# scomup/EasyGaussianSplatting

Measured on AMD Instinct MI355X. Metric: rendered Mpix/s fwd+bwd at 1920x1080, 1M Gaussians, higher is better.
Workload: dtype f32; 1 GPU; 1 MI355X per view: 1000000 synthetic Gaussians, 1920x1080, SH degree 3, forward+backward (GSFunction, mode=fused); gaussians=1000000, width=1920, height=1080, sh_dim=48, views_per_rank=1, view_streams=1, policy=gsplatcu, mode=fused, validation=deferred (commit per step), preconditioning=400 untimed steps before the warm-up steps (clock ramp), lists=footprint-culled (fused path)

## Files before the change

### easygaussiansplatting_amd/_ahead.py

```python
from __future__ import annotations

import collections
import ctypes as C
import threading

import torch

from . import _lib
from ._host import _ptr

MAILBOX_SLOTS = 64
HINT_SLOTS = 16
SIZE_TABLE_MAX = 1024


class _Ticket:
    __slots__ = ("ctx", "slot", "key", "cap", "hint", "state", "status", "patches", "need", "collected")
    PENDING, OK, FAILED = 0, 1, 2


class _DeviceCtx:

    def __init__(self, lib, index):
        self.index = index
        self.lib = lib
        self.mb = lib.egs_mailbox_create(MAILBOX_SLOTS)
        if not self.mb:
            raise RuntimeError("egs_mailbox_create failed (page-locked host memory)")
        self.free = list(range(MAILBOX_SLOTS))
        self.pending = collections.deque()
        self.failed = []
        self.capacity = {}
        self.tile_work = {}
        self.seg_hint = {}
        self.walk_word = {}
        self.long_walks_expected = 0
        self.lock = threading.RLock()


_contexts = {}
_tls = threading.local()


def _ctx(dev) -> _DeviceCtx:
    c = _contexts.get(dev.index)
    if c is None:
        c = _contexts.setdefault(dev.index, _DeviceCtx(_lib.load(), dev.index))
    return c


def _grow(p):
    return p + p // 16 + 4096


def _learn_capacity(ctx, key, patches):
    cap = ctx.capacity
    val = max(cap.pop(key, 0), _grow(min(patches, 2**31 - 1)))
    cap[key] = val
    while len(cap) > SIZE_TABLE_MAX:
        cap.pop(next(iter(cap)), None)


_key_bits = {}
_key_low = {}
KEY_BITS_DECAY = 32


def _get_key_bits(dev_index, key=None) -> int:
    return _key_bits.get((dev_index, key), 32)


def _set_key_bits(dev_index, key, bits) -> None:
    _key_bits[(dev_index, key)] = int(bits)
    _key_low.pop((dev_index, key), None)


def _learn_key_bits(dev_index, key, need, missed=False) -> None:
    k = (dev_index, key)
    target = min(32, int(need) + 1)
    while len(_key_bits) > 1024:
        old = next(iter(_key_bits))
        _key_bits.pop(old, None)
        _key_low.pop(old, None)
    if missed:
        _key_bits[k] = 32
        _key_low.pop(k, None)
        return
    hint = _key_bits.get(k, 32)
    if hint >= 32 or target >= hint:
        _key_bits[k] = target
        _key_low.pop(k, None)
        return
    low = _key_low.setdefault(k, [0, 0])
    low[0] += 1
    low[1] = max(low[1], target)
    if low[0] >= KEY_BITS_DECAY:
        _key_bits[k] = low[1]
        _key_low.pop(k, None)


def _bin_stage(enqueue, device, key=None):
    total = torch.empty(2, dtype=torch.int32, device=device)
    hint = _get_key_bits(device.index, key)
    enqueue(hint, total, None)
    p, mk = (int(v) & 0xFFFFFFFF for v in total.tolist())
    need = mk.bit_length()
    if hint < 32 and need > hint:
        enqueue(32, total, None)
        p, mk = (int(v) & 0xFFFFFFFF for v in total.tolist())
    _learn_key_bits(device.index, key, need)
    if p >= 2**31:
        raise RuntimeError("splat: %d tile patches overflow int32 indexing" % p)
    return p


def _settle(t: _Ticket, blocking: bool) -> bool:
    ctx = t.ctx
    with ctx.lock:
        if t.status != _Ticket.PENDING:
            return True
        out = (C.c_uint32 * 2)()
    rc = ctx.lib.egs_mailbox_fetch(ctx.mb, t.slot, 1 if blocking else 0, out)
    if rc == 0:
        return False
    if rc < 0:
        with ctx.lock:
            if t.status == _Ticket.PENDING:
                t.status, t.patches, t.need = _Ticket.FAILED, 0, 0
                ctx.free.append(t.slot)
                try:
                    ctx.pending.remove(t)
                except ValueError:
                    pass
                if t.state is not None:
                    t.state.ticket = None
                    t.state._patches = 0
        _lib.check(-rc)
    with ctx.lock:
        if t.status != _Ticket.PENDING:
            return True
        t.patches, mk = int(out[0]), int(out[1])
        t.need = mk.bit_length()
        ctx.free.append(t.slot)
        try:
            ctx.pending.remove(t)
        except ValueError:
            pass
        ok = t.patches <= t.cap and not (t.hint < 32 and t.need > t.hint) and t.patches < 2**31
        _learn_key_bits(ctx.index, t.key, t.need, missed=(t.hint < 32 and t.need > t.hint))
        _learn_capacity(ctx, t.key, t.patches)
        t.status = _Ticket.OK if ok else _Ticket.FAILED
        S = t.state
        if S is not None:
            S._patches = t.patches
            S.ticket = None
            if ok:
                S.gsid = S.gsid[:t.patches]
        if not ok and not t.collected:
            ctx.failed.append(t)
    return True


class deferred:

    def __enter__(self):
        self._prev = getattr(_tls, "deferred", False)
        _tls.deferred = True
        return self

    def commit(self):
        return commit()

    def __exit__(self, et, ev, tb):
        _tls.deferred = self._prev
        if et is None and not self._prev:
            bad = commit()
            if bad:
                raise RuntimeError("%d enqueue-ahead render(s) were incomplete (patch capacity or depth-key hint "
                                   "exceeded) and nobody collected them with commit(): their results must not be used"
                                   % len(bad))
        return False


def commit(device=None):
    index = torch.cuda.current_device() if device is None else torch.device(device).index
    ctx = _contexts.get(index)
    if ctx is None:
        return []
    while True:
        with ctx.lock:
            t = ctx.pending[0] if ctx.pending else None
        if t is None:
            break
        _settle(t, True)
    with ctx.lock:
        bad, ctx.failed = ctx.failed, []
    for t in bad:
        t.collected = True
    return [t.state for t in bad]


def expect_long_walks(device=None, renders=4):
    index = torch.cuda.current_device() if device is None else torch.device(device).index
    if index is None:
        return
    ctx = _contexts.get(index)
    if ctx is None:
        ctx = _ctx(torch.device("cuda", index))
    with ctx.lock:
        ctx.long_walks_expected = max(ctx.long_walks_expected, int(renders))


def _seg_decision(ctx, lib, key, pol_, segments, speculate):
    if segments == "0" or pol_.footprint != 0 or not (pol_.alpha_skip > 0) or not (pol_.tau_stop > 0):
        return False, None, speculate == "1"
    with ctx.lock:
        slot = ctx.seg_hint.pop(key, None)
        if slot is None:
            if len(ctx.seg_hint) >= HINT_SLOTS:
                slot = ctx.seg_hint.pop(next(iter(ctx.seg_hint)))
            elif len(ctx.free) > MAILBOX_SLOTS // 2:
                slot = ctx.free.pop()
            else:
                return segments == "1", None, speculate == "1"
            _lib.check(lib.egs_mailbox_clear(ctx.mb, slot))
        ctx.seg_hint[key] = slot
    out = (C.c_uint32 * 4)()
    _lib.check(lib.egs_mailbox_peek(ctx.mb, slot, out))
    cfg = (C.c_int * 2)()
    _lib.check(lib.egs_seg_config(0, 0, cfg))
    longest, walk = int(out[0]), int(out[1])
    known = walk != 0xFFFFFFFF and longest != 0xFFFFFFFF
    unknown = walk == 0xFFFFFFFF and (longest == 0xFFFFFFFF or longest > cfg[1])
    use = segments == "1" or unknown or (walk != 0xFFFFFFFF and walk > cfg[1])
    with ctx.lock:
        announced = ctx.long_walks_expected > 0
        if announced:
            ctx.long_walks_expected -= 1
    hint = C.c_void_p(lib.egs_mailbox_slot(ctx.mb, slot))
    if announced and segments != "0":
        return True, hint, speculate != "0"
    return use, hint, speculate == "1" or (speculate == "auto" and known and 2 * walk >= longest)


def _walk_word(ctx, key, dev, st, have_hint):
    if not have_hint:
        return None
    k = (key, int(st.value or 0))
    with ctx.lock:
        w = ctx.walk_word.get(k)
        if w is None:
# ... 96 lines not shown
```

### easygaussiansplatting_amd/csrc/egs_bin.hip

```cpp
#include "egs_raster.h"

#include <stdlib.h>

#include <algorithm>

namespace egs {

__global__ __launch_bounds__(256) void k_bin_count(int n, BinParams p, const float* __restrict__ us,
                                                   int32_t* __restrict__ areas, float* __restrict__ depths,
                                                   uint4* __restrict__ cr,
                                                   uint32_t* __restrict__ dkeys, uint32_t* __restrict__ ids,
                                                   uint32_t* __restrict__ maxkey, uint32_t* __restrict__ sort_sup,
                                                   uint32_t sort_sup_words) {
  const int i = blockIdx.x * 256 + threadIdx.x;
  for (uint32_t z = (uint32_t)i; z < sort_sup_words; z += gridDim.x * 256u) sort_sup[z] = 0u;
  uint32_t key = 0u;
  if (i < n) {
    uint4 rect;
    bool cull;
    const uint32_t cnt = bin_count_one(p, us[2 * (size_t)i], us[2 * (size_t)i + 1], (float)areas[2 * (size_t)i],
                                       (float)areas[2 * (size_t)i + 1], depths[i], rect, key, cull);
    if (cull) {
      depths[i] = EGS_BAD_MARKER;
      areas[2 * (size_t)i] = 0;
      areas[2 * (size_t)i + 1] = 0;
    }
    ids[i] = (uint32_t)i;
    uint4 c = make_uint4(0u, 0u, 0u, 0u);
    if (cnt) {
      const uint32_t w = rect.z - rect.x, h = rect.w - rect.y;
      c.x = rect.x | (rect.y << 16);
      c.y = w | (h << 16);
      if (w <= 4u && h <= 4u) {
        const unsigned long long row = (1ull << (2 * w)) - 1ull;
        unsigned long long bits = 0ull;
        for (uint32_t r = 0; r < 2 * h; ++r) bits |= row << (8 * r);
        c.z = (uint32_t)bits; c.w = (uint32_t)(bits >> 32);
      } else {
        c.y |= EGS_CR_BIG; c.z = cnt; c.w = 0u;
      }
    }
    cr[i] = c;
    dkeys[i] = key;
  }
  __shared__ uint32_t wm[4];
  block_max_key(key, maxkey, wm);
}

__device__ __forceinline__ uint32_t row_stamp(float ux, float uy, float c0, float c1, float c2, float al) {
  uint32_t h = __float_as_uint(ux) * 0x9E3779B1u;
  h = (h ^ (h >> 15)) + __float_as_uint(uy) * 0x85EBCA77u;
  h = (h ^ (h >> 13)) + __float_as_uint(c0) * 0xC2B2AE3Du;
  h = (h ^ (h >> 16)) + __float_as_uint(c1) * 0x27D4EB2Fu;
  h = (h ^ (h >> 15)) + __float_as_uint(c2) * 0x165667B1u;
  h = (h ^ (h >> 13)) + __float_as_uint(al) * 0x9E3779B1u;
  return h ^ (h >> 16);
}
__device__ __forceinline__ void block_stamp(uint32_t h, uint32_t* __restrict__ stamp, uint32_t* red,
                                            const uint32_t* __restrict__ ref = nullptr,
                                            uint8_t* __restrict__ same = nullptr) {
  uint32_t s1 = h, s2 = h * (2u * threadIdx.x + 1u);
#pragma unroll
  for (int d = 32; d >= 1; d >>= 1) { s1 += (uint32_t)__shfl_xor((int)s1, d, 64); s2 += (uint32_t)__shfl_xor((int)s2, d, 64); }
  if ((threadIdx.x & 63) == 0) { red[threadIdx.x >> 6] = s1; red[4 + (threadIdx.x >> 6)] = s2; }
  __syncthreads();
  if (threadIdx.x == 0) {
    const uint32_t a = red[0] + red[1] + red[2] + red[3], b = red[4] + 3u * red[5] + 5u * red[6] + 7u * red[7];
    stamp[2 * (size_t)blockIdx.x] = a;
    stamp[2 * (size_t)blockIdx.x + 1] = b;
    if (ref && same) same[blockIdx.x] = (ref[2 * (size_t)blockIdx.x] == a && ref[2 * (size_t)blockIdx.x + 1] == b) ? 1 : 0;
  }
}
__global__ __launch_bounds__(256) void k_pack_bin(int n, BinParams p, float alpha_skip, const float* __restrict__ us,
                                                  const float* __restrict__ cinv, const float* __restrict__ alphas,
                                                  const float* __restrict__ colors, int32_t* __restrict__ areas,
                                                  float* __restrict__ depths, float4* __restrict__ rec,
                                                  uint4* __restrict__ cr, BinRec* __restrict__ br,
                                                  uint32_t* __restrict__ dkeys, uint32_t* __restrict__ ids,
                                                  uint32_t* __restrict__ maxkey, uint32_t* __restrict__ sort_sup,
                                                  uint32_t sort_sup_words, uint32_t* __restrict__ stamp,
                                                  uint8_t* __restrict__ visible) {
  const int i = blockIdx.x * 256 + threadIdx.x;
  for (uint32_t z = (uint32_t)i; z < sort_sup_words; z += gridDim.x * 256u) sort_sup[z] = 0u;
  uint32_t key = 0u, hst = 0u;
  __shared__ float4 st[256 * 5];
  float4 r3[3] = {make_float4(0.f, 0.f, 0.f, 0.f), make_float4(0.f, 0.f, 0.f, 0.f), make_float4(0.f, 0.f, 0.f, 0.f)};
  if (i < n) {
    const float ux = us[2 * (size_t)i], uy = us[2 * (size_t)i + 1];
    const float c0 = cinv[3 * (size_t)i], c1 = cinv[3 * (size_t)i + 1], c2 = cinv[3 * (size_t)i + 2];
    const float al = alphas[i];
    make_record(ux, uy, c0, c1, c2, al, colors[3 * (size_t)i], colors[3 * (size_t)i + 1], colors[3 * (size_t)i + 2],
                0, 0, p.W, p.H, 0, alpha_skip, r3);
    hst = row_stamp(ux, uy, c0, c1, c2, al);
    uint4 rect;
    bool cull;
    const uint32_t cnt = bin_count_one(p, ux, uy, (float)areas[2 * (size_t)i], (float)areas[2 * (size_t)i + 1],
                                       depths[i], rect, key, cull);
    const float depth_in = depths[i];
    if (cull) {
      depths[i] = EGS_BAD_MARKER;
      areas[2 * (size_t)i] = 0;
      areas[2 * (size_t)i + 1] = 0;
    }
    if (visible) visible[i] = (cull ? EGS_BAD_MARKER : depth_in) > 0.2f;
    ids[i] = (uint32_t)i;
    uint4 c = make_uint4(0u, 0u, 0u, 0u);
    if (cnt) {
      const BinRec b = make_binrec(ux, uy, c0, c1, c2, al, alpha_skip, true, rect, cnt);
      const uint32_t w = b.wh & 0xFFFFu, h = b.wh >> 16;
      if (w <= 4u && h <= 4u) {
        const unsigned long long bits = foot_bitmap(b);
        c = make_uint4(b.xy, b.wh | EGS_CR_ALLTILES, (uint32_t)bits, (uint32_t)(bits >> 32));
      } else {
        const bool walk = b.m < __int_as_float(0x7f800000);
        c = make_uint4(b.xy, b.wh | EGS_CR_BIG, cnt, walk ? 2u : 0u);
        if (walk) {
          float4* o = reinterpret_cast<float4*>(br + i);
          o[0] = make_float4(b.ux, b.uy, b.A, b.Bh);
          o[1] = make_float4(b.C, b.m, __uint_as_float(b.xy), __uint_as_float(b.wh));
        }
      }
    }
    cr[i] = c;
    dkeys[i] = key;
  }
#pragma unroll
  for (int j = 0; j < 3; ++j) st[threadIdx.x * 5 + j] = r3[j];
  __shared__ uint32_t wm[4];
  block_max_key(key, maxkey, wm);
  if (stamp) {
    __shared__ uint32_t red[8];
    block_stamp(hst, stamp, red);
  }
  {
    const int base = blockIdx.x * 256, rows = min(256, n - base);
    float4* __restrict__ d4 = rec + 3 * (size_t)base;
#pragma unroll
    for (int j = 0; j < 3; ++j) {
      const int f = (int)threadIdx.x + 256 * j;
      if (f < 3 * rows) { const int rr = f / 3; d4[f] = st[rr * 5 + (f - 3 * rr)]; }
    }
  }
}

__global__ __launch_bounds__(256) void k_bin_scan_partials(const uint32_t* __restrict__ cnt_sorted, int64_t n,
                                                           uint32_t* __restrict__ partials) {
  __shared__ uint32_t sm[4];
  const int64_t base = (int64_t)blockIdx.x * SC_TILE + (int64_t)threadIdx.x * SC_IPT;
  uint32_t s = 0;
  if (base + SC_IPT <= n) {
    const uint4 a = *reinterpret_cast<const uint4*>(cnt_sorted + base), b = *reinterpret_cast<const uint4*>(cnt_sorted + base + 4);
    s = a.x + a.y + a.z + a.w + b.x + b.y + b.z + b.w;
  } else {
#pragma unroll
    for (int k = 0; k < SC_IPT; ++k)
      if (base + k < n) s += cnt_sorted[base + k];
  }
  s = wave_inclusive_scan(s);
  if ((threadIdx.x & 63) == 63) sm[threadIdx.x >> 6] = s;
  __syncthreads();
  if (threadIdx.x == 0) partials[blockIdx.x] = sm[0] + sm[1] + sm[2] + sm[3];
}

__global__ __launch_bounds__(256) void k_bin_scan_apply(const uint32_t* __restrict__ cnt_sorted, int64_t n,
                                                        const uint32_t* __restrict__ partials,
                                                        uint32_t* __restrict__ out, uint32_t* __restrict__ total,
                                                        uint32_t* __restrict__ total_host) {
  __shared__ uint32_t sm[4];
  __shared__ uint32_t s_prefix;
  uint32_t pre = 0;
  for (int i = threadIdx.x; i < (int)blockIdx.x; i += 256) pre += partials[i];
  pre = wave_inclusive_scan(pre);
  if ((threadIdx.x & 63) == 63) sm[threadIdx.x >> 6] = pre;
  __syncthreads();
  if (threadIdx.x == 0) s_prefix = sm[0] + sm[1] + sm[2] + sm[3];
  __syncthreads();
  const uint32_t prefix = s_prefix;
  const int64_t base = (int64_t)blockIdx.x * SC_TILE + (int64_t)threadIdx.x * SC_IPT;
  uint32_t v[SC_IPT];
  uint32_t s = 0;
  if (base + SC_IPT <= n) {
    const uint4 a = *reinterpret_cast<const uint4*>(cnt_sorted + base), b = *reinterpret_cast<const uint4*>(cnt_sorted + base + 4);
    v[0] = a.x; v[1] = a.y; v[2] = a.z; v[3] = a.w; v[4] = b.x; v[5] = b.y; v[6] = b.z; v[7] = b.w;
  } else {
#pragma unroll
    for (int k = 0; k < SC_IPT; ++k) v[k] = (base + k < n) ? cnt_sorted[base + k] : 0u;
  }
#pragma unroll
  for (int k = 0; k < SC_IPT; ++k) s += v[k];
  uint32_t blocksum;
  uint32_t ex = block256_exclusive_scan(s, sm, &blocksum) + prefix;
  if (total && blockIdx.x == gridDim.x - 1 && threadIdx.x == 0) {
    *total = prefix + blocksum;
    if (total_host) *total_host = prefix + blocksum;
  }
  if (base + SC_IPT <= n) {
    uint4 a, b;
    a.x = ex; a.y = a.x + v[0]; a.z = a.y + v[1]; a.w = a.z + v[2];
    b.x = a.w + v[3]; b.y = b.x + v[4]; b.z = b.y + v[5]; b.w = b.z + v[6];
    *reinterpret_cast<uint4*>(out + base) = a;
    *reinterpret_cast<uint4*>(out + base + 4) = b;
  } else {
#pragma unroll
    for (int k = 0; k < SC_IPT; ++k) {
      const int64_t i = base + k;
      if (i < n) out[i] = ex;
      ex += v[k];
    }
  }
}

__global__ __launch_bounds__(256) void k_bin_emit(int n, int gx, const uint32_t* __restrict__ ids,
                                                  const uint32_t* __restrict__ offsets,
                                                  const uint4* __restrict__ cr_sorted,
                                                  const BinRec* __restrict__ br,
                                                  uint32_t* __restrict__ tkeys, uint32_t* __restrict__ gsid,
                                                  uint32_t cap, int32_t* __restrict__ ranges, int n_ranges,
                                                  int with_masks, uint32_t* __restrict__ sort_sup,
                                                  uint32_t sort_sup_words) {
  __shared__ uint32_t s_off[257];
  __shared__ uint32_t s_g[256];
  __shared__ uint4 s_cr[256];
  const int tid = threadIdx.x;
  const int j = blockIdx.x * 256 + tid;
  for (int i = j; i < n_ranges; i += gridDim.x * 256) ranges[i] = 0;
  for (uint32_t z = (uint32_t)j; z < sort_sup_words; z += gridDim.x * 256u) sort_sup[z] = 0u;
  uint32_t off = 0, g = 0;
  uint4 c = make_uint4(0u, 0u, 0u, 0u);
  if (j < n) {
    g = ids[j];
    c = cr_sorted[j];
    off = offsets[j];
  }
  __shared__ uint32_t s_first, s_last;
  if (tid == 0) s_first = off;
  const int last = min(255, n - 1 - blockIdx.x * 256);
  if (tid == last) s_last = off + cr_count(c);
  __syncthreads();
  const uint32_t first = s_first;
  s_off[tid] = (j < n) ? off - first : 0xFFFFFFFFu;
  s_g[tid] = g;
  s_cr[tid] = c;
  const uint32_t span = s_last - first;
  __syncthreads();
  for (uint32_t s0 = tid; s0 < span; s0 += 256) {
    int lo = 0;
#pragma unroll
    for (int step = 128; step >= 1; step >>= 1)
      if (s_off[lo + step] <= s0) lo += step;
    uint32_t r = s0 - s_off[lo];
    const uint4 cc = s_cr[lo];
    const int x0 = (int)(cc.x & 0xFFFFu), y0 = (int)(cc.x >> 16);
    const int w = (int)(cc.y & 0xFFFFu);
    uint32_t tile = 0u, mask = 0xFu;
    if (cc.y & EGS_CR_TILEMAP) {
      const unsigned long long tb = ((unsigned long long)cc.w << 32) | cc.z;
      int ty = 0, tx = 0;
      uint32_t rb = 0u;
      bool found = false;
#pragma unroll
      for (int q = 0; q < 8; ++q) {
        const uint32_t bq = (uint32_t)(tb >> (8 * q)) & 0xFFu;
        const uint32_t pc = (uint32_t)__popc(bq);
        if (!found) {
          if (r < pc) { rb = bq; ty = q; found = true; }
          else r -= pc;
        }
      }
      found = false;
#pragma unroll
      for (int q = 0; q < 8; ++q) {
        if (((rb >> q) & 1u) && !found) {
          if (r == 0u) { tx = q; found = true; }
          else --r;
        }
      }
      tile = (uint32_t)(y0 + ty) * (uint32_t)gx + (uint32_t)(x0 + tx);
      const BinRec b = br[s_g[lo]];
      const Foot f = foot_setup(b);
      const SlabPx sa = foot_slab(f, (y0 + ty) * EGS_TILE), sb = foot_slab(f, (y0 + ty) * EGS_TILE + 8);
      mask = foot_mask(sa, sb, x0 + tx);
    } else if (!(cc.y & EGS_CR_BIG)) {
      const unsigned long long blocks = ((unsigned long long)cc.w << 32) | cc.z;
      int ty = 0, tx = 0;
      if (cc.y & EGS_CR_ALLTILES) {
        ty = (int)(r / (uint32_t)w);
        tx = (int)(r - (uint32_t)ty * (uint32_t)w);
      } else {
      const unsigned long long tb = cr_tile_bits(blocks);
      uint32_t rb = 0u;
      bool found = false;
#pragma unroll
      for (int q = 0; q < 4; ++q) {
        const uint32_t bq = (uint32_t)(tb >> (16 * q)) & 0x55u;
        const uint32_t pc = (uint32_t)__popc(bq);
        if (!found) {
          if (r < pc) { rb = bq; ty = q; found = true; }
          else r -= pc;
        }
      }
      found = false;
#pragma unroll
      for (int q = 0; q < 4; ++q) {
        if (((rb >> (2 * q)) & 1u) && !found) {
          if (r == 0u) { tx = q; found = true; }
          else --r;
        }
      }
      }
      tile = (uint32_t)(y0 + ty) * (uint32_t)gx + (uint32_t)(x0 + tx);
      mask = ((uint32_t)(blocks >> (16 * ty + 2 * tx)) & 3u) | (((uint32_t)(blocks >> (16 * ty + 8 + 2 * tx)) & 3u) << 2);
    } else if (cc.w == 0u) {
      const uint32_t ry = r / (uint32_t)w, rx = r - ry * (uint32_t)w;
      tile = (uint32_t)(y0 + (int)ry) * (uint32_t)gx + (uint32_t)x0 + rx;
    } else if (cc.w == 2u) {
      const uint32_t ry = r / (uint32_t)w, rx = r - ry * (uint32_t)w;
      tile = (uint32_t)(y0 + (int)ry) * (uint32_t)gx + (uint32_t)x0 + rx;
      const BinRec b = br[s_g[lo]];
      mask = 0u;
      if (!(b.m < 0.f)) {
        const Foot f = foot_setup(b);
        SlabPx sa, sb;
        int tlo, thi;
        foot_row(f, y0 + (int)ry, sa, sb, tlo, thi);
        const int tx = x0 + (int)rx;
        if (tx >= tlo && tx <= thi) mask = foot_mask(sa, sb, tx);
      }
    } else {
      continue;
    }
    if (first + s0 >= cap) break;
    tkeys[first + s0] = tile;
    gsid[first + s0] = with_masks ? (s_g[lo] | (mask << EGS_GSID_BITS)) : s_g[lo];
  }
  {
    const int lane = tid & 63, wbase = tid & ~63;
    unsigned long long bigs = __ballot(j < n && (c.y & EGS_CR_BIG) && c.w == 1u && c.z != 0u);
    while (bigs != 0ull) {
      const int t = wbase + (int)__builtin_ctzll(bigs);
      bigs &= bigs - 1ull;
      const uint4 cc = s_cr[t];
      const uint32_t gg = s_g[t];
      const uint32_t obase = first + s_off[t];
      const int y0 = (int)(cc.x >> 16), h = (int)((cc.y & EGS_CR_WH_MASK) >> 16);
      const BinRec b = br[gg];
      const Foot f = foot_setup(b);
      uint32_t run = 0u;
      for (int rb = 0; rb < h; rb += 64) {
        SlabPx sa, sb;
        sa.pl = sb.pl = 0x7fffffff; sa.pr = sb.pr = (int)0x80000000;
        int tlo = 1, thi = 0;
        if (rb + lane < h) foot_row(f, y0 + rb + lane, sa, sb, tlo, thi);
        const uint32_t wd = thi >= tlo ? (uint32_t)(thi - tlo + 1) : 0u;
        const uint32_t inc = wave_inclusive_scan(wd);
        const uint32_t ex = run + inc - wd;
        const int rows = min(64, h - rb);
        for (int q = 0; q < rows; ++q) {
          const int qlo = __shfl(tlo, q, 64), qhi = __shfl(thi, q, 64);
          const uint32_t qoff = (uint32_t)__shfl((int)ex, q, 64);
          SlabPx qa, qb;
          qa.pl = __shfl(sa.pl, q, 64); qa.pr = __shfl(sa.pr, q, 64);
          qb.pl = __shfl(sb.pl, q, 64); qb.pr = __shfl(sb.pr, q, 64);
          for (int tx = qlo + lane; tx <= qhi; tx += 64) {
            const uint32_t o = obase + qoff + (uint32_t)(tx - qlo);
            if (o < cap) {
              tkeys[o] = (uint32_t)(y0 + rb + q) * (uint32_t)gx + (uint32_t)tx;
              gsid[o] = with_masks ? (gg | (foot_mask(qa, qb, tx) << EGS_GSID_BITS)) : gg;
            }
          }
        }
        run += (uint32_t)__shfl((int)inc, 63, 64);
      }
    }
  }
}

__global__ __launch_bounds__(256) void k_tile_ranges(int64_t P, const uint32_t* __restrict__ tkeys,
                                                     int32_t* __restrict__ ranges,
                                                     const uint32_t* __restrict__ n_dev,
                                                     const uint32_t* __restrict__ masked, int32_t* __restrict__ plain,
                                                     int32_t* __restrict__ zero, int zero_words,
                                                     int32_t* __restrict__ walk_word, uint32_t* __restrict__ walk_host) {
  for (int z = blockIdx.x * 256 + threadIdx.x; z < zero_words; z += gridDim.x * 256) zero[z] = 0;
  if (walk_word && blockIdx.x == 0 && threadIdx.x == 0) {
    const int w = walk_word[0], l = walk_word[1];
    if (w >= 0 && l >= 0 && walk_host) { walk_host[0] = (uint32_t)l; walk_host[1] = (uint32_t)w; }
    walk_word[0] = -1; walk_word[1] = -1;
  }
  if (n_dev) P = min(P, (int64_t)*n_dev);
  const int64_t p0 = ((int64_t)blockIdx.x * 256 + threadIdx.x) * 4;
  if (p0 >= P) return;
  if (plain) {
    if (p0 + 4 <= P) {
      uint4 v = *reinterpret_cast<const uint4*>(masked + p0);
      v.x &= EGS_GSID_MASK; v.y &= EGS_GSID_MASK; v.z &= EGS_GSID_MASK; v.w &= EGS_GSID_MASK;
      *reinterpret_cast<uint4*>(plain + p0) = v;
    } else {
      for (int64_t q = p0; q < P; ++q) plain[q] = (int32_t)(masked[q] & EGS_GSID_MASK);
    }
  }
  uint32_t k[5];
  k[0] = p0 > 0 ? tkeys[p0 - 1] : 0u;
  if (p0 + 4 <= P) {
    const uint4 v = *reinterpret_cast<const uint4*>(tkeys + p0);
    k[1] = v.x; k[2] = v.y; k[3] = v.z; k[4] = v.w;
  } else {
#pragma unroll
    for (int i = 0; i < 4; ++i) k[1 + i] = (p0 + i < P) ? tkeys[p0 + i] : 0u;
  }
#pragma unroll
  for (int i = 0; i < 4; ++i) {
    const int64_t p = p0 + i;
    if (p < P) {
      const uint32_t cur = k[1 + i];
      if (p == 0) ranges[2 * (size_t)cur] = 0;
      else if (k[i] != cur) {
        ranges[2 * (size_t)k[i] + 1] = (int32_t)p;
        ranges[2 * (size_t)cur] = (int32_t)p;
      }
      if (p == P - 1) ranges[2 * (size_t)cur + 1] = (int32_t)P;
    }
  }
}

__global__ __launch_bounds__(256) void k_pair_fix(int64_t P, uint32_t* __restrict__ kept,
                                                  const int32_t* __restrict__ plain,
                                                  const uint8_t* __restrict__ same, uint32_t n) {
  const int64_t p0 = 4 * ((int64_t)blockIdx.x * 256 + threadIdx.x);
  if (p0 >= P) return;
  uint32_t k[4], q[4];
  if (p0 + 4 <= P) {
    const uint4 kv = *reinterpret_cast<const uint4*>(kept + p0);
    const uint4 qv = *reinterpret_cast<const uint4*>(plain + p0);
    k[0] = kv.x; k[1] = kv.y; k[2] = kv.z; k[3] = kv.w;
    q[0] = qv.x; q[1] = qv.y; q[2] = qv.z; q[3] = qv.w;
  } else {
#pragma unroll
    for (int t = 0; t < 4; ++t) { k[t] = (p0 + t < P) ? kept[p0 + t] : 0u; q[t] = (p0 + t < P) ? (uint32_t)plain[p0 + t] : 0u; }
  }
  bool changed = false;
#pragma unroll
  for (int t = 0; t < 4; ++t) {
    const uint32_t gid = q[t] & EGS_GSID_MASK;
    const bool good = (k[t] & EGS_GSID_MASK) == q[t] && gid < n && same[gid >> 8] != 0;
    if (!good) { k[t] = (q[t] & EGS_GSID_MASK) | (0xFu << EGS_GSID_BITS); changed = true; }
  }
  if (changed) {
#pragma unroll
    for (int t = 0; t < 4; ++t)
      if (p0 + t < P) kept[p0 + t] = k[t];
  }
}

__global__ __launch_bounds__(256) void k_pack_records(int n, int W, int H, int footprint, float alpha_skip,
                                                      const float* __restrict__ us,
                                                      const float* __restrict__ cinv,
                                                      const float* __restrict__ alphas,
                                                      const float* __restrict__ colors,
                                                      const int32_t* __restrict__ areas,
                                                      float4* __restrict__ rec, uint32_t* __restrict__ stamp,
                                                      const uint32_t* __restrict__ stamp_ref, uint8_t* __restrict__ same) {
  const int i = blockIdx.x * 256 + threadIdx.x;
  uint32_t h = 0u;
  if (i < n) {
    const float ux = us[2 * (size_t)i], uy = us[2 * (size_t)i + 1];
    const float c0 = cinv[3 * (size_t)i], c1 = cinv[3 * (size_t)i + 1], c2 = cinv[3 * (size_t)i + 2];
    const float al = alphas[i];
    make_record(ux, uy, c0, c1, c2, al, colors[3 * (size_t)i], colors[3 * (size_t)i + 1],
                colors[3 * (size_t)i + 2], footprint == 1 ? areas[2 * (size_t)i] : 0,
                footprint == 1 ? areas[2 * (size_t)i + 1] : 0, W, H, footprint, alpha_skip, rec + 3 * (size_t)i);
    h = row_stamp(ux, uy, c0, c1, c2, al);
  }
  if (stamp) {
    __shared__ uint32_t red[8];
    block_stamp(h, stamp, red, stamp_ref, same);
  }
}

size_t bin_ws_bytes(int n) {
  const size_t N = (size_t)(n > 0 ? n : 1);
  return 2 * align_up(N * 16, 256) + align_up(N * 32, 256) + 6 * align_up(N * 4, 256) + scan_ws_bytes(n) +
         sort_ws_bytes(n) + align_up((64 + N / 256 + 1) * 4, 256) + 4096;
}
bool bin_carve(void* ws, size_t bytes, int n, BinLayout* L) {
  Carver cv(ws, bytes);
  const size_t N = (size_t)(n > 0 ? n : 1);
  L->cr = cv.take<uint4>(N);
  L->cr_sorted = cv.take<uint4>(N);
  L->br = cv.take<BinRec>(N);
  L->cnt_sorted = cv.take<uint32_t>(N);
  L->dkeys = cv.take<uint32_t>(N);
  L->dkeys_alt = cv.take<uint32_t>(N);
  L->ids = cv.take<uint32_t>(N);
  L->ids_alt = cv.take<uint32_t>(N);
  L->offsets = cv.take<uint32_t>(N);
  L->scan_partials = cv.take<uint32_t>(scan_ws_bytes(n) / 4);
  L->maxkey = cv.take<uint32_t>(64 + div_up(N, 256));
  return sort_ws_carve(cv, n, &L->sort) && cv.ok();
}


int bin_emit(int n, int gx, const BinLayout& B, uint32_t* tkeys, uint32_t* gsid, uint32_t cap, int32_t* ranges,
             int n_ranges, int with_masks, uint32_t* sort_sup, uint32_t sort_sup_words, hipStream_t s) {
  EGS_LAUNCH("k_bin_emit", k_bin_emit, dim3(div_up(n, 256)), dim3(256), s, n, gx, B.ids, B.offsets, B.cr_sorted, B.br,
             tkeys, gsid, cap, ranges, n_ranges, with_masks, sort_sup, sort_sup_words);
  EGS_LAUNCH_OK();
  return 0;
}

int tile_ranges(int64_t P, const uint32_t* tkeys, int32_t* ranges, const uint32_t* n_dev, const uint32_t* masked,
                int32_t* plain, hipStream_t s, int32_t* zero, int zero_words, int32_t* walk_word, uint32_t* walk_host) {
  EGS_LAUNCH("k_tile_ranges", k_tile_ranges, dim3(div_up(P, 1024)), dim3(256), s, P, tkeys, ranges, n_dev, masked, plain,
             zero, zero_words, walk_word, walk_host);
  EGS_LAUNCH_OK();
  return 0;
}

int pack_records(int n, int width, int height, int footprint, float alpha_skip, const float* us, const float* cinv2ds,
                 const float* alphas, const float* colors, const int32_t* areas, float4* rec, uint32_t* stamp,
                 const uint32_t* stamp_ref, uint8_t* same, hipStream_t s) {
  EGS_LAUNCH("k_pack_records", k_pack_records, dim3(div_up(n, 256)), dim3(256), s, n, width, height, footprint,
             alpha_skip, us, cinv2ds, alphas, colors, areas, rec, stamp, stamp_ref, same);
  EGS_LAUNCH_OK();
  return 0;
}

}

using namespace egs;

extern "C" size_t egs_splat_bin_ws_bytes(int n) { return bin_ws_bytes(n); }
static int splat_bin_impl(int n, int width, int height, const float* us, int32_t* areas, float* depths,
                          const EgsPolicy* pol, int key_bits_hint, void* ws_bin, size_t ws_bin_bytes,
                          uint32_t* total_patches, uint32_t* host_totals, void* stream);

extern "C" int egs_splat_bin(int n, int width, int height, const float* us, int32_t* areas, float* depths,
                             const EgsPolicy* pol, int key_bits_hint, void* ws_bin, size_t ws_bin_bytes,
                             uint32_t* total_patches, void* stream) {
  return splat_bin_impl(n, width, height, us, areas, depths, pol, key_bits_hint, ws_bin, ws_bin_bytes, total_patches,
                        nullptr, stream);
}

extern "C" int egs_splat_bin_mb(int n, int width, int height, const float* us, int32_t* areas, float* depths,
                                const EgsPolicy* pol, int key_bits_hint, void* ws_bin, size_t ws_bin_bytes,
                                uint32_t* total_patches, uint32_t* host_totals, void* stream) {
  return splat_bin_impl(n, width, height, us, areas, depths, pol, key_bits_hint, ws_bin, ws_bin_bytes, total_patches,
                        host_totals, stream);
}

extern "C" int egs_splat_bin_pack(int n, int width, int height, const float* us, const float* cinv2ds,
                                  const float* alphas, const float* colors, int32_t* areas, float* depths,
                                  const EgsPolicy* pol, int key_bits_hint, void* ws_bin, size_t ws_bin_bytes,
                                  uint32_t* total_patches, uint32_t* host_totals, void* rec, uint32_t* stamp,
                                  uint8_t* visible, void* stream) {
  EGS_CHECK_ARG(n >= 0 && width > 0 && height > 0 && pol && total_patches);
  EGS_CHECK_ARG(width < 32768 && height < 32768);
  EGS_CHECK_ARG(pol->footprint == 0 && pol->alpha_skip > 0.f && n < (1 << EGS_GSID_BITS));
  hipStream_t s = (hipStream_t)stream;
  if (n == 0) {
    EGS_HIP(hipMemsetAsync(total_patches, 0, 8, s));
    if (host_totals) EGS_HIP(hipMemcpyAsync(host_totals, total_patches, 8, hipMemcpyDeviceToHost, s));
    return 0;
  }
  EGS_CHECK_ARG(us && cinv2ds && alphas && colors && areas && depths && ws_bin && rec);
  EGS_CHECK_ARG(((uintptr_t)rec & 15) == 0);
  BinLayout L;
  if (!bin_carve(ws_bin, ws_bin_bytes, n, &L)) {
    set_error(EGS_ERR_WORKSPACE, "bin workspace too small", __FILE__, __LINE__);
    return EGS_ERR_WORKSPACE;
  }
  const BinParams p = make_bin_params(width, height, pol);
  EGS_LAUNCH("k_pack_bin", k_pack_bin, dim3(div_up(n, 256)), dim3(256), s, n, p, pol->alpha_skip, us, cinv2ds, alphas,
             colors, areas, depths, (float4*)rec, L.cr, L.br, L.dkeys, L.ids, L.maxkey, L.sort.sup,
             (uint32_t)L.sort.sup_words, stamp, visible);
  EGS_LAUNCH_OK();
  return splat_bin_after_count(n, key_bits_hint, ws_bin, ws_bin_bytes, total_patches, stream, host_totals);
}

static int splat_bin_impl(int n, int width, int height, const float* us, int32_t* areas, float* depths,
                          const EgsPolicy* pol, int key_bits_hint, void* ws_bin, size_t ws_bin_bytes,
                          uint32_t* total_patches, uint32_t* host_totals, void* stream) {
  EGS_CHECK_ARG(n >= 0 && width > 0 && height > 0 && pol && total_patches);
  EGS_CHECK_ARG(width < 32768 && height < 32768);
  hipStream_t s = (hipStream_t)stream;
  if (n == 0) {
    EGS_HIP(hipMemsetAsync(total_patches, 0, 8, s));
    if (host_totals) EGS_HIP(hipMemcpyAsync(host_totals, total_patches, 8, hipMemcpyDeviceToHost, s));
    return 0;
  }
  EGS_CHECK_ARG(us && areas && depths && ws_bin);
  BinLayout L;
  if (!bin_carve(ws_bin, ws_bin_bytes, n, &L)) {
    set_error(EGS_ERR_WORKSPACE, "bin workspace too small", __FILE__, __LINE__);
    return EGS_ERR_WORKSPACE;
  }
  const BinParams p = make_bin_params(width, height, pol);
  EGS_LAUNCH("k_bin_count", k_bin_count, dim3(div_up(n, 256)), dim3(256), s, n, p, us, areas, depths, L.cr,
             L.dkeys, L.ids, L.maxkey, L.sort.sup, (uint32_t)L.sort.sup_words);
  EGS_LAUNCH_OK();
  return splat_bin_after_count(n, key_bits_hint, ws_bin, ws_bin_bytes, total_patches, stream, host_totals);
}

namespace egs {
BinParams make_bin_params(int width, int height, const EgsPolicy* pol, bool cull_lists) {
  BinParams p;
  p.W = width; p.H = height;
  p.gx = div_up(width, EGS_TILE); p.gy = div_up(height, EGS_TILE);
  p.footprint = pol->footprint; p.far_cull = pol->far_cull; p.depth_key = pol->depth_key;
  p.mutate = (pol->footprint == 0);
  p.cull_lists = cull_lists && pol->footprint == 0 && pol->alpha_skip > 0.f;
  return p;
}

bool bin_count_outputs(void* ws_bin, size_t ws_bin_bytes, int n, BinCountOut* out) {
  BinLayout L;
  if (!bin_carve(ws_bin, ws_bin_bytes, n, &L)) return false;
  out->cr = L.cr; out->br = L.br; out->dkeys = L.dkeys; out->ids = L.ids; out->maxkey = L.maxkey;
  out->sort_sup = L.sort.sup; out->sort_sup_words = (uint32_t)L.sort.sup_words;
  return true;
}

int splat_bin_after_count(int n, int key_bits_hint, void* ws_bin, size_t ws_bin_bytes, uint32_t* total_patches,
                          void* stream, uint32_t* host_totals) {
  hipStream_t s = (hipStream_t)stream;
  BinLayout L;
  if (!bin_carve(ws_bin, ws_bin_bytes, n, &L)) {
    set_error(EGS_ERR_WORKSPACE, "bin workspace too small", __FILE__, __LINE__);
    return EGS_ERR_WORKSPACE;
  }
  const int end_bit = (key_bits_hint <= 0 || key_bits_hint > 32) ? 32 : key_bits_hint;
  int rc = radix_sort(n, L.dkeys, L.ids, L.dkeys_alt, L.ids_alt, 0, end_bit, L.sort, s, L.maxkey, nullptr, L.maxkey,
                      div_up(n, 256), total_patches + 1, host_totals ? host_totals + 1 : nullptr, L.cr, L.cr_sorted,
                      L.cnt_sorted);
  if (rc) return rc;
  if (sort_passes(0, end_bit) & 1) {
    EGS_HIP(hipMemcpyAsync(L.dkeys, L.dkeys_alt, (size_t)n * 4, hipMemcpyDeviceToDevice, s));
    EGS_HIP(hipMemcpyAsync(L.ids, L.ids_alt, (size_t)n * 4, hipMemcpyDeviceToDevice, s));
  }
  const int nb = div_up(n, SC_TILE);
  EGS_LAUNCH("k_bin_scan_partials", k_bin_scan_partials, dim3(nb), dim3(256), s, L.cnt_sorted, (int64_t)n,
             L.scan_partials);
  EGS_LAUNCH("k_bin_scan_apply", k_bin_scan_apply, dim3(nb), dim3(256), s, L.cnt_sorted, (int64_t)n, L.scan_partials,
             L.offsets, total_patches, host_totals);
  EGS_LAUNCH_OK();
  return 0;
}
}

extern "C" int egs_pack_records(int n, int width, int height, const float* us, const float* cinv2ds,
                                const float* alphas, const float* colors, const int32_t* areas, const EgsPolicy* pol,
                                void* rec, void* stream) {
  EGS_CHECK_ARG(n >= 0 && width > 0 && height > 0 && pol);
  if (n == 0) return 0;
  EGS_CHECK_ARG(us && cinv2ds && alphas && colors && rec && (areas || pol->footprint != 1));
  EGS_CHECK_ARG(((uintptr_t)rec & 15) == 0);
  return pack_records(n, width, height, pol->footprint, pol->alpha_skip, us, cinv2ds, alphas, colors, areas, (float4*)rec,
                      nullptr, nullptr, nullptr, (hipStream_t)stream);
}

extern "C" size_t egs_pair_stamp_words(int n) {
  const size_t nwg = (size_t)div_up(n > 0 ? n : 1, 256);
  return 2 * nwg + (nwg + 3) / 4 + 4;
}

extern "C" int egs_pack_records_validate(int n, int width, int height, const float* us, const float* cinv2ds,
                                         const float* alphas, const float* colors, const EgsPolicy* pol, void* rec,
                                         const uint32_t* stamp_a, uint32_t* stamp_b, int64_t patches, void* kept,
                                         const int32_t* plain, void* stream) {
  EGS_CHECK_ARG(n > 0 && width > 0 && height > 0 && pol && pol->footprint == 0 && n < (1 << EGS_GSID_BITS));
  EGS_CHECK_ARG(us && cinv2ds && alphas && colors && rec && stamp_a && stamp_b && patches >= 0);
  EGS_CHECK_ARG(patches == 0 || (kept && plain && (((uintptr_t)kept | (uintptr_t)plain) & 15) == 0));
  EGS_CHECK_ARG(((uintptr_t)rec & 15) == 0 && (((uintptr_t)stamp_a | (uintptr_t)stamp_b) & 7) == 0);
  hipStream_t s = (hipStream_t)stream;
  uint8_t* same = (uint8_t*)(stamp_b + 2 * (size_t)div_up(n, 256));
  EGS_LAUNCH("k_pack_records", k_pack_records, dim3(div_up(n, 256)), dim3(256), s, n, width, height, 0,
             pol->alpha_skip, us, cinv2ds, alphas, colors, (const int32_t*)nullptr, (float4*)rec, stamp_b, stamp_a, same);
  if (patches > 0)
    EGS_LAUNCH("k_pair_fix", k_pair_fix, dim3(div_up(patches, 1024)), dim3(256), s, patches, (uint32_t*)kept, plain,
               (const uint8_t*)same, (uint32_t)n);
  EGS_LAUNCH_OK();
  return 0;
}
```

### easygaussiansplatting_amd/csrc/egs_common.h

```cpp
#pragma once

#include <hip/hip_runtime.h>
#include <stdint.h>
#include <stddef.h>
#include <type_traits>

#include "../../include/egs_hip.h"

#define EGS_MIN_DEPTH 0.2f
#define EGS_BAD_MARKER (-1.f)
#define EGS_TILE 16
#define EGS_WAVE 64

namespace egs {

void set_error(int code, const char* what, const char* file, int line);

#define EGS_CHECK_ARG(cond)                                                      \
  do {                                                                           \
    if (!(cond)) {                                                               \
      ::egs::set_error(EGS_ERR_BAD_ARG, "bad argument: " #cond, __FILE__, __LINE__); \
      return EGS_ERR_BAD_ARG;                                                    \
    }                                                                            \
  } while (0)

#define EGS_HIP(expr)                                                            \
  do {                                                                           \
    hipError_t e__ = (expr);                                                     \
    if (e__ != hipSuccess) {                                                     \
      ::egs::set_error((int)e__, hipGetErrorString(e__), __FILE__, __LINE__);    \
      return (int)e__;                                                           \
    }                                                                            \
  } while (0)

#define EGS_LAUNCH_OK() EGS_HIP(hipGetLastError())

bool prof_on(const char* name);
void prof_begin(const char* name, hipStream_t s);
void prof_end(hipStream_t s);
struct ProfScope {
  hipStream_t s;
  bool on;
  ProfScope(const char* name, hipStream_t st) : s(st), on(prof_on(name)) {
    if (on) prof_begin(name, s);
  }
  ~ProfScope() {
    if (on) prof_end(s);
  }
};
#define EGS_LAUNCH(name, kern, grid, block, stream, ...)                 \
  do {                                                                   \
    ::egs::ProfScope ps__(name, stream);                                 \
    hipLaunchKernelGGL(kern, grid, block, 0, stream, __VA_ARGS__);       \
  } while (0)

template <typename F>
inline void with_bools(F&& f) { f(); }
template <typename F, typename... B>
inline void with_bools(F&& f, bool b0, B... rest) {
  if (b0) with_bools([&](auto... c) { f(std::true_type{}, c...); }, rest...);
  else with_bools([&](auto... c) { f(std::false_type{}, c...); }, rest...);
}
template <typename F>
inline void with_sh_dim(int sh_dim, F&& f) {
  switch (sh_dim) {
    case 3: f(std::integral_constant<int, 1>{}); break;
    case 12: f(std::integral_constant<int, 4>{}); break;
    case 27: f(std::integral_constant<int, 9>{}); break;
    default: f(std::integral_constant<int, 16>{}); break;
  }
}

static inline int div_up(int64_t a, int64_t b) { return (int)((a + b - 1) / b); }
static inline size_t align_up(size_t v, size_t a) { return (v + a - 1) / a * a; }

struct Carver {
  char* base;
  size_t off;
  size_t cap;
  Carver(void* p, size_t bytes) : base((char*)p), off(0), cap(bytes) {}
  template <typename T>
  T* take(size_t count) {
    size_t start = align_up(off, 256);
    off = start + count * sizeof(T);
    return (T*)(base + start);
  }
  bool ok() const { return off <= cap; }
};

struct BinParams {
  int W, H, gx, gy;
  int footprint, far_cull, depth_key, mutate;
  int cull_lists;
};
struct BinRec {
  float ux, uy, A, Bh;
  float C, m;
  uint32_t xy;
  uint32_t wh;
};
static_assert(sizeof(BinRec) == 32, "BinRec is two dwordx4");
#define EGS_CR_BIG 0x80000000u
#define EGS_CR_TILEMAP 0x40000000u
#define EGS_CR_ALLTILES 0x20000000u
#define EGS_CR_WH_MASK 0x1FFFFFFFu
struct BinCountOut {
  uint4* cr;
  BinRec* br;
  uint32_t *dkeys, *ids, *maxkey;
  uint32_t* sort_sup;
  uint32_t sort_sup_words;
};
#define EGS_GSID_BITS 28
#define EGS_GSID_MASK 0x0FFFFFFFu
BinParams make_bin_params(int width, int height, const EgsPolicy* pol, bool cull_lists = false);
bool bin_count_outputs(void* ws_bin, size_t ws_bin_bytes, int n, BinCountOut* out);
int splat_bin_after_count(int n, int key_bits_hint, void* ws_bin, size_t ws_bin_bytes, uint32_t* total_patches,
                          void* stream, uint32_t* host_totals);

struct SplatSource {
  const void* rec;
  const float *us, *cinv2ds, *alphas, *colors;
  const int32_t* areas;
};
struct SplatForward {
  const int32_t* contrib;
  const float* final_tau;
  const int32_t* ranges;
  const int32_t* gsid;
};
struct SplatCarry {
  const int32_t* tile_order;
  float* grad_records;
  bool keep_forward_order;
  bool masked_lists;
  void* seg_ws;
  size_t seg_ws_bytes;
  int rebuild;
  uint32_t* seg_hint;
  const EgsExtras* extras;
  bool absgrad;
};
int splat_bwd_packed(int n, int64_t patches, int width, int height, const EgsPolicy* pol, const SplatSource& src,
                     const SplatForward& fwd, const float* dloss_dgammas, void* ws, const SplatCarry& carry,
                     float** gpack, void* stream);

#ifdef __HIPCC__
__device__ __forceinline__ int lane_id() { return (int)(threadIdx.x & 63u); }

__device__ __forceinline__ uint32_t wave_inclusive_scan(uint32_t v) {
  const int lane = lane_id();
#pragma unroll
  for (int d = 1; d < 64; d <<= 1) {
    uint32_t t = __shfl_up(v, d, 64);
    if (lane >= d) v += t;
  }
  return v;
}

__device__ __forceinline__ uint32_t block256_exclusive_scan(uint32_t v, uint32_t* smem, uint32_t* total) {
  const int wave = threadIdx.x >> 6, lane = threadIdx.x & 63;
  uint32_t inc = wave_inclusive_scan(v);
  if (lane == 63) smem[wave] = inc;
  __syncthreads();
  uint32_t s0 = smem[0], s1 = smem[1], s2 = smem[2], s3 = smem[3];
  uint32_t off = (wave > 0 ? s0 : 0u) + (wave > 1 ? s1 : 0u) + (wave > 2 ? s2 : 0u);
  if (total) *total = s0 + s1 + s2 + s3;
  __syncthreads();
  return off + inc - v;
}

__device__ __forceinline__ float wave_sum(float v) {
#pragma unroll
  for (int d = 32; d >= 1; d >>= 1) v += __shfl_xor(v, d, 64);
  return v;
}
#endif

}
```

### easygaussiansplatting_amd/csrc/egs_gaussian_math.h

```cpp
#pragma once
#include "egs_common.h"

namespace egs {

struct f3 { float x, y, z; };
struct q4 { float w, x, y, z; };
__device__ __forceinline__ f3 ld3(const float* p) { return {p[0], p[1], p[2]}; }
__device__ __forceinline__ void st3(float* p, f3 v) { p[0] = v.x; p[1] = v.y; p[2] = v.z; }
__device__ __forceinline__ f3 operator*(float s, f3 a) { return {s * a.x, s * a.y, s * a.z}; }
__device__ __forceinline__ f3 operator+(f3 a, f3 b) { return {a.x + b.x, a.y + b.y, a.z + b.z}; }
__device__ __forceinline__ float dot(f3 a, f3 b) { return a.x * b.x + a.y * b.y + a.z * b.z; }
__device__ __forceinline__ f3 had(f3 a, f3 b) { return {a.x * b.x, a.y * b.y, a.z * b.z}; }
__device__ __forceinline__ q4 vm(f3 v, q4 r0, q4 r1, q4 r2) {
  return {v.x * r0.w + v.y * r1.w + v.z * r2.w, v.x * r0.x + v.y * r1.x + v.z * r2.x,
          v.x * r0.y + v.y * r1.y + v.z * r2.y, v.x * r0.z + v.y * r1.z + v.z * r2.z};
}
__device__ __forceinline__ q4 operator+(q4 a, q4 b) { return {a.w + b.w, a.x + b.x, a.y + b.y, a.z + b.z}; }
__device__ __forceinline__ q4 operator*(float s, q4 a) { return {s * a.w, s * a.x, s * a.y, s * a.z}; }
__device__ __forceinline__ void st4(float* p, q4 v) { p[0] = v.w; p[1] = v.x; p[2] = v.y; p[3] = v.z; }

struct Proj {
  f3 pc;
  float u0, u1, z_inv;
};
// ... 433 lines not shown
  }
  if (cnt != 0) key = (p.depth_key == 0) ? (uint32_t)(depth * 1000.f) : __float_as_uint(depth);
  return cnt;
}

struct Foot {
  float ux, uy, A, Bh, C, m;
  float det, rA, ymax, k, eps;
  int px_lo, px_hi;
  bool cull;
};
struct SlabPx { int pl, pr; };
#pragma clang fp contract(off)
__device__ __forceinline__ Foot foot_setup(const BinRec& b) {
  Foot f;
  f.ux = b.ux; f.uy = b.uy; f.A = b.A; f.Bh = b.Bh; f.C = b.C; f.m = b.m;
  f.cull = b.m < __int_as_float(0x7f800000);
  const int x0 = (int)(b.xy & 0xFFFFu), w = (int)(b.wh & 0xFFFFu);
  f.px_lo = x0 * EGS_TILE;
  f.px_hi = (x0 + w) * EGS_TILE - 1;
  f.det = f.A * f.C - f.Bh * f.Bh;
  const float rdet = __builtin_amdgcn_rcpf(f.det);
  f.rA = __builtin_amdgcn_rcpf(f.A);
  const float xext = __builtin_amdgcn_sqrtf(f.m * f.C * rdet);
  f.ymax = __builtin_amdgcn_sqrtf(f.m * f.A * rdet);
  f.k = f.Bh * __builtin_amdgcn_rcpf(f.C) * xext;
  f.eps = 0.05f + 0.01f * fmaxf(xext, f.ymax);
  return f;
}
__device__ __forceinline__ SlabPx foot_slab(const Foot& f, int Y0) {
  SlabPx o;
  o.pl = 0x7fffffff; o.pr = (int)0x80000000;
  const float ya = fmaxf((float)Y0 - f.uy - f.eps, -f.ymax);
  const float yb = fminf((float)(Y0 + 7) - f.uy + f.eps, f.ymax);
  if (!(ya <= yb)) return o;
  const float yr = fminf(fmaxf(-f.k, ya), yb), yl = fminf(fmaxf(f.k, ya), yb);
  const float Am = f.A * f.m;
  const float sr = __builtin_amdgcn_sqrtf(fmaxf(Am - f.det * yr * yr, 0.f));
  const float sl = __builtin_amdgcn_sqrtf(fmaxf(Am - f.det * yl * yl, 0.f));
  const float xr = f.ux + ((sr - f.Bh * yr) * f.rA + f.eps);
  const float xl = f.ux + ((-sl - f.Bh * yl) * f.rA - f.eps);
  if (!(xl <= xr)) return o;
  o.pl = max(f.px_lo, (int)ceilf(fmaxf(xl, -1.0e9f)));
  o.pr = min(f.px_hi, (int)floorf(fminf(xr, 1.0e9f)));
  if (o.pl > o.pr) { o.pl = 0x7fffffff; o.pr = (int)0x80000000; }
  return o;
}
__device__ __forceinline__ void foot_row(const Foot& f, int ty, SlabPx& s0, SlabPx& s1, int& lo, int& hi) {
  s0 = foot_slab(f, ty * EGS_TILE);
  s1 = foot_slab(f, ty * EGS_TILE + 8);
  lo = min(s0.pl, s1.pl) >> 4;
  hi = max(s0.pr, s1.pr) >> 4;
  if (s0.pl > s0.pr && s1.pl > s1.pr) { lo = 1; hi = 0; }
}
__device__ __forceinline__ uint32_t foot_mask(const SlabPx& s0, const SlabPx& s1, int tx) {
  const int X = tx * EGS_TILE;
  uint32_t m = 0u;
  if (s0.pl <= X + 7 && s0.pr >= X) m |= 1u;
  if (s0.pl <= X + 15 && s0.pr >= X + 8) m |= 2u;
  if (s1.pl <= X + 7 && s1.pr >= X) m |= 4u;
  if (s1.pl <= X + 15 && s1.pr >= X + 8) m |= 8u;
  return m;
}
__device__ __forceinline__ uint32_t foot_count(const BinRec& b) {
  const int w = (int)(b.wh & 0xFFFFu), h = (int)(b.wh >> 16), y0 = (int)(b.xy >> 16);
  if (b.m < 0.f) return 0u;
  const Foot f = foot_setup(b);
  if (!f.cull) return (uint32_t)(w * h);
  uint32_t c = 0u;
  for (int ry = 0; ry < h; ++ry) {
    SlabPx s0, s1;
    int lo, hi;
    foot_row(f, y0 + ry, s0, s1, lo, hi);
    if (hi >= lo) c += (uint32_t)(hi - lo + 1);
  }
  return c;
}
__device__ __forceinline__ unsigned long long foot_bitmap(const BinRec& b) {
  const int x0 = (int)(b.xy & 0xFFFFu), y0 = (int)(b.xy >> 16), w = (int)(b.wh & 0xFFFFu), h = (int)(b.wh >> 16);
  const uint32_t rowfull = (1u << (2 * w)) - 1u;
  unsigned long long bits = 0ull;
  if (b.m < 0.f) return 0ull;
  const Foot f = foot_setup(b);
  for (int s = 0; s < 2 * h; ++s) {
    uint32_t row = rowfull;
    if (f.cull) {
      const SlabPx sp = foot_slab(f, y0 * EGS_TILE + 8 * s);
      row = 0u;
      if (sp.pl <= sp.pr) {
        const int bl = (sp.pl >> 3) - 2 * x0, br = (sp.pr >> 3) - 2 * x0;
        row = ((2u << br) - 1u) & ~((1u << bl) - 1u);
      }
    }
    bits |= (unsigned long long)row << (8 * s);
  }
  return bits;
}
__device__ __forceinline__ unsigned long long foot_tilemap(const BinRec& b) {
  const int x0 = (int)(b.xy & 0xFFFFu), y0 = (int)(b.xy >> 16), h = (int)(b.wh >> 16);
  if (b.m < 0.f) return 0ull;
  const Foot f = foot_setup(b);
  unsigned long long bits = 0ull;
  for (int ry = 0; ry < h; ++ry) {
    SlabPx s0, s1;
    int lo, hi;
    foot_row(f, y0 + ry, s0, s1, lo, hi);
    if (hi >= lo) bits |= (unsigned long long)(((2u << (hi - x0)) - 1u) & ~((1u << (lo - x0)) - 1u)) << (8 * ry);
  }
  return bits;
}
#pragma clang fp contract(fast)
__device__ __forceinline__ unsigned long long cr_tile_bits(unsigned long long blocks) {
  unsigned long long t = blocks | (blocks >> 1);
  t |= t >> 8;
  return t & 0x0055005500550055ull;
}
__device__ __forceinline__ uint32_t cr_count(const uint4& c) {
  if (c.y & EGS_CR_BIG) return c.z;
  if (c.y & EGS_CR_ALLTILES) return (c.y & 0xFFFFu) * ((c.y & EGS_CR_WH_MASK) >> 16);
  const unsigned long long b = ((unsigned long long)c.w << 32) | c.z;
  return (uint32_t)__popcll((c.y & EGS_CR_TILEMAP) ? b : cr_tile_bits(b));
}
__device__ __forceinline__ BinRec make_binrec(float ux, float uy, float c0, float c1, float c2, float alpha,
                                              float alpha_skip, bool cull, const uint4& rect, uint32_t cnt_rect) {
  BinRec b;
  const float inf = __int_as_float(0x7f800000);
  b.ux = ux; b.uy = uy;
  b.A = -EGS_NHL2E * c0; b.Bh = -EGS_NHL2E * c1; b.C = -EGS_NHL2E * c2;
  b.m = inf;
  b.xy = cnt_rect ? (rect.x | (rect.y << 16)) : 0u;
  b.wh = cnt_rect ? ((rect.z - rect.x) | ((rect.w - rect.y) << 16)) : 0u;
  if (cull && alpha_skip > 0.f) {
    const float det = c0 * c2 - c1 * c1;
    if (det > 1e-4f * c0 * c2 && c0 > 0.f && c2 > 0.f && alpha == alpha) {
      if (alpha >= alpha_skip) {
        const float m = log2f(alpha / alpha_skip);
        if (m == m && m < inf) b.m = m;
      } else {
        b.m = -1.f;
      }
    }
  }
  return b;
}

__device__ __forceinline__ void block_max_key(uint32_t key, uint32_t* __restrict__ maxkey, uint32_t* wm) {
  uint32_t mk = key;
#pragma unroll
  for (int d = 32; d >= 1; d >>= 1) mk = max(mk, (uint32_t)__shfl_xor((int)mk, d, 64));
  if ((threadIdx.x & 63) == 0) wm[threadIdx.x >> 6] = mk;
  __syncthreads();
  if (threadIdx.x == 0) maxkey[1 + blockIdx.x] = max(max(wm[0], wm[1]), max(wm[2], wm[3]));
}

__device__ __forceinline__ void make_record(float ux, float uy, float c0, float c1, float c2, float alpha,
                                            float r, float g, float b, int area_x, int area_y, int W, int H,
                                            int footprint, float alpha_skip, float4* __restrict__ out) {
  const float inf = __int_as_float(0x7f800000);
  float e1, e2;
  if (footprint == 1) {
    int x0, x1, y0, y1;
    pixel_box(ux, uy, (float)area_x, (float)area_y, W, H, x0, x1, y0, y1);
    e1 = __uint_as_float((uint32_t)x0 | ((uint32_t)x1 << 16));
    e2 = __uint_as_float((uint32_t)y0 | ((uint32_t)y1 << 16));
  } else {
    e1 = inf; e2 = inf;
    const float det = c0 * c2 - c1 * c1;
    if (alpha_skip > 0.f && det > 1e-4f * c0 * c2 && c0 > 0.f && c2 > 0.f) {
      if (alpha > alpha_skip) {
        const float mstar = 2.f * logf(alpha / alpha_skip);
        const float sxx = c2 / det, syy = c0 / det;
        e1 = sqrtf(mstar * sxx) * 1.01f + 0.05f;
        e2 = sqrtf(mstar * syy) * 1.01f + 0.05f;
      } else if (alpha <= alpha_skip * 0.999f) {
        e1 = -inf; e2 = -inf;
      }
    }
    if (!(e1 == e1) || !(e2 == e2)) { e1 = inf; e2 = inf; }
  }
  float thr;
  if (alpha_skip > 0.f) thr = (alpha >= alpha_skip) ? log2f(alpha_skip / alpha) : inf;
  else thr = (alpha < 0.f) ? inf : -inf;
  out[0] = make_float4(ux, uy, EGS_NHL2E * c0, (2.f * EGS_NHL2E) * c1);
  out[1] = make_float4(EGS_NHL2E * c2, alpha, r, g);
  out[2] = make_float4(b, e1, e2, thr);
}

}
```

### easygaussiansplatting_amd/csrc/egs_preprocess.hip

```cpp
#include "egs_gaussian_math.h"

namespace egs {

template <int K>
struct RowStage {
  static constexpr bool V4 = (K % 4 == 0);
  static constexpr int Q = K / 4;
  static constexpr int STRIDE = V4 ? 4 * ((Q + 1) | 1) : (K | 1);
  static constexpr int LDS_FLOATS = 256 * STRIDE;
  static constexpr bool DIRECT = (K <= 2);
  static constexpr int OUT_LDS_FLOATS = DIRECT ? 1 : LDS_FLOATS;
};
constexpr int cmax(int a, int b) { return a > b ? a : b; }

template <int K>
__device__ __forceinline__ void rows_out(const float* row, float* __restrict__ dst, int n, int base, float* lds) {
  using RO = RowStage<K>;
  const int tid = threadIdx.x;
  const int rows = min(256, n - base);
  if constexpr (RO::DIRECT) {
    if (tid < rows) {
      if constexpr (K == 2) reinterpret_cast<float2*>(dst)[base + tid] = make_float2(row[0], row[1]);
      else dst[base + tid] = row[0];
    }
// ... 796 lines not shown
  if (i < n) sh_grad_row<NC>(ld3(pws + 3 * (size_t)i), rows, stride, views, n, i, scale, gsh);
  if constexpr (RAW) {
    if (i < n) {
#pragma unroll
      for (int k = 0; k < 3; ++k) dL_dsh[3 * (size_t)i + k] = gsh[k] + (accum ? dL_dsh[3 * (size_t)i + k] : 0.f);
    }
    if constexpr (KH > 0) {
      if constexpr (KH % 2 == 1) stage_span_out<KH>(gsh + 3, dL_dsh_high, n, blockIdx.x * 256, stage, accum != 0);
      else stage_rows_out<KH>(gsh + 3, dL_dsh_high, n, blockIdx.x * 256, stage, accum != 0);
    }
  } else {
    stage_rows_out<K>(gsh, dL_dsh, n, blockIdx.x * 256, stage, accum != 0);
  }
}

}

using namespace egs;

static void fov_limits(const EgsPolicy* pol, float fx, float fy, float width, float height, float* limx,
                       float* limy) {
  *limx = 0.f; *limy = 0.f;
  if (pol->fov_mode == 0) {
    *limx = 1.3f * (width / (2 * fx));
    *limy = 1.3f * (height / (2 * fy));
  } else if (pol->fov_mode == 1) {
    *limx = (float)(1.3 * (2 * atan((double)width / (2 * (double)fx))));
    *limy = (float)(1.3 * (2 * atan((double)height / (2 * (double)fy))));
  }
}

extern "C" int egs_project(int n, const float* pws, const float* Rcw, const float* tcw, float fx, float fy,
                           float cx, float cy, const EgsPolicy* pol, float* us, float* pcs, float* depths,
                           float* du_dpcs, void* stream) {
  EGS_CHECK_ARG(n >= 0 && pol);
  if (n == 0) return 0;
  EGS_CHECK_ARG(pws && Rcw && tcw && us && pcs && depths);
  EGS_CHECK_ARG((((uintptr_t)us | (uintptr_t)du_dpcs) & 7) == 0);
  EGS_LAUNCH("k_project", k_project, dim3(div_up(n, 256)), dim3(256), (hipStream_t)stream, n, pws, Rcw, tcw, fx,
                     fy, cx, cy, pol->near_cull, us, pcs, depths, du_dpcs);
  EGS_LAUNCH_OK();
  return 0;
}

extern "C" int egs_cov3d(int n, const float* rots, const float* scales, const float* depths,
                         const EgsPolicy* pol, float* cov3ds, float* dcov3d_drots, float* dcov3d_dscales,
                         void* stream) {
  EGS_CHECK_ARG(n >= 0 && pol);
  if (n == 0) return 0;
  EGS_CHECK_ARG(rots && scales && depths && cov3ds);
  EGS_CHECK_ARG((dcov3d_drots == nullptr) == (dcov3d_dscales == nullptr));
  EGS_CHECK_ARG(((uintptr_t)rots & 15) == 0);
  EGS_CHECK_ARG((((uintptr_t)cov3ds | (uintptr_t)dcov3d_drots | (uintptr_t)dcov3d_dscales) & 15) == 0);
  EGS_LAUNCH("k_cov3d", k_cov3d, dim3(div_up(n, 256)), dim3(256), (hipStream_t)stream, n, rots, scales, depths,
                     pol->near_cull, cov3ds, dcov3d_drots, dcov3d_dscales);
  EGS_LAUNCH_OK();
  return 0;
}

extern "C" int egs_cov2d(int n, const float* cov3ds, const float* pcs, const float* Rcw, const float* depths,
                         float fx, float fy, float width, float height, const EgsPolicy* pol, float* cov2ds,
                         float* dcov2d_dcov3ds, float* dcov2d_dpcs, void* stream) {
  EGS_CHECK_ARG(n >= 0 && pol);
  if (n == 0) return 0;
  EGS_CHECK_ARG(cov3ds && pcs && Rcw && depths && cov2ds);
  EGS_CHECK_ARG((dcov2d_dcov3ds == nullptr) == (dcov2d_dpcs == nullptr));
  EGS_CHECK_ARG((((uintptr_t)cov3ds & 7) | (((uintptr_t)cov2ds | (uintptr_t)dcov2d_dcov3ds | (uintptr_t)dcov2d_dpcs) & 15)) == 0);
  float limx, limy;
  fov_limits(pol, fx, fy, width, height, &limx, &limy);
  EGS_LAUNCH("k_cov2d", k_cov2d, dim3(div_up(n, 256)), dim3(256), (hipStream_t)stream, n, cov3ds, pcs, Rcw,
                     depths, fx, fy, limx, limy, pol->fov_mode != 2, pol->near_cull, cov2ds, dcov2d_dcov3ds,
                     dcov2d_dpcs);
  EGS_LAUNCH_OK();
  return 0;
}

extern "C" int egs_sh2color(int n, int sh_dim, const float* shs, const float* pws, const float* twc,
                            float* colors, float* dcolor_dshs, float* dcolor_dpws, void* stream) {
  EGS_CHECK_ARG(n >= 0);
  EGS_CHECK_ARG(sh_dim == 3 || sh_dim == 12 || sh_dim == 27 || sh_dim == 48);
  if (n == 0) return 0;
  EGS_CHECK_ARG(shs && pws && twc && colors);
  EGS_CHECK_ARG((dcolor_dshs == nullptr) == (dcolor_dpws == nullptr));
  EGS_CHECK_ARG(sh_dim % 4 != 0 || ((uintptr_t)shs & 15) == 0);
  EGS_CHECK_ARG((((uintptr_t)colors | (uintptr_t)dcolor_dshs | (uintptr_t)dcolor_dpws) & 15) == 0);
  dim3 g(div_up(n, 256)), b(256);
  hipStream_t s = (hipStream_t)stream;
  decltype(&k_sh2color<1>) kern = nullptr;
  with_sh_dim(sh_dim, [&](auto nc) { kern = k_sh2color<nc.value>; });
  EGS_LAUNCH("k_sh2color", kern, g, b, s, n, shs, pws, twc, colors, dcolor_dshs, dcolor_dpws);
  EGS_LAUNCH_OK();
  return 0;
}

extern "C" int egs_inv_cov2d(int n, const float* cov2ds, float* depths, const EgsPolicy* pol, float* cinv2ds,
                             int32_t* areas, float* dcinv2d_dcov2ds, void* stream) {
  EGS_CHECK_ARG(n >= 0 && pol);
  if (n == 0) return 0;
  EGS_CHECK_ARG(cov2ds && depths && cinv2ds && areas);
  EGS_CHECK_ARG((((uintptr_t)cinv2ds | (uintptr_t)areas | (uintptr_t)dcinv2d_dcov2ds) & 15) == 0);
  EGS_LAUNCH("k_inv_cov2d", k_inv_cov2d, dim3(div_up(n, 256)), dim3(256), (hipStream_t)stream, n, cov2ds, depths,
                     pol->det_eps, pol->near_cull, pol->nan_cull, pol->radius_mode, cinv2ds, areas,
                     dcinv2d_dcov2ds);
  EGS_LAUNCH_OK();
  return 0;
}

extern "C" int egs_chain_rule(int n, int sh_dim, const float* dloss_dus, const float* dloss_dcinv2ds,
                              const float* dloss_dcolors, const float* Rcw, const float* dcinv2d_dcov2ds,
                              const float* dcov2d_dcov3ds, const float* dcov3d_drots,
                              const float* dcov3d_dscales, const float* dcolor_dshs, const float* du_dpcs,
                              const float* dcov2d_dpcs, const float* dcolor_dpws, float* dloss_dpws,
                              float* dloss_dshs, float* dloss_dscales, float* dloss_drots, void* stream) {
  EGS_CHECK_ARG(n >= 0);
  EGS_CHECK_ARG(sh_dim == 3 || sh_dim == 12 || sh_dim == 27 || sh_dim == 48);
  if (n == 0) return 0;
  EGS_CHECK_ARG(dloss_dus && dloss_dcinv2ds && dloss_dcolors && Rcw && dcinv2d_dcov2ds && dcov2d_dcov3ds &&
                dcov3d_drots && dcov3d_dscales && dcolor_dshs && du_dpcs && dcov2d_dpcs && dcolor_dpws &&
                dloss_dpws && dloss_dshs && dloss_dscales && dloss_drots);
  EGS_CHECK_ARG((((uintptr_t)dloss_dpws | (uintptr_t)dloss_dshs | (uintptr_t)dloss_dscales | (uintptr_t)dloss_drots |
                  (uintptr_t)dcov3d_drots | (sh_dim % 12 == 0 ? (uintptr_t)dcolor_dshs : 0)) & 15) == 0);
  EGS_CHECK_ARG((((uintptr_t)dloss_dus | (uintptr_t)dcov2d_dcov3ds | (uintptr_t)dcov3d_dscales | (uintptr_t)du_dpcs) & 7) == 0);
  dim3 g(div_up(n, 256)), b(256);
  hipStream_t s = (hipStream_t)stream;
  decltype(&k_chain_rule<1>) kern = nullptr;
  with_sh_dim(sh_dim, [&](auto nc) { kern = k_chain_rule<nc.value>; });
  EGS_LAUNCH("k_chain_rule", kern, g, b, s, n, dloss_dus, dloss_dcinv2ds, dloss_dcolors, Rcw, dcinv2d_dcov2ds,
             dcov2d_dcov3ds, dcov3d_drots, dcov3d_dscales, dcolor_dshs, du_dpcs, dcov2d_dpcs, dcolor_dpws, dloss_dpws,
             dloss_dshs, dloss_dscales, dloss_drots);
  EGS_LAUNCH_OK();
  return 0;
}

static PreParams make_pre_params(const EgsPolicy* pol, float fx, float fy, float cx, float cy, int width,
                                 int height) {
  PreParams pp;
  pp.fx = fx; pp.fy = fy; pp.cx = cx; pp.cy = cy;
  fov_limits(pol, fx, fy, (float)width, (float)height, &pp.limx, &pp.limy);
  pp.det_eps = pol->det_eps; pp.alpha_skip = pol->alpha_skip;
  pp.footprint = pol->footprint; pp.W = width; pp.H = height;
  pp.clamp_fov = pol->fov_mode != 2; pp.near_cull = pol->near_cull; pp.nan_cull = pol->nan_cull;
  pp.radius_mode = pol->radius_mode;
  pp.stage_in = 0;
  return pp;
}

extern "C" int egs_fused_forward(int n, int sh_dim, const float* pws, const float* rots, const float* scales,
                                 const float* shs, const float* shs_high, const float* alphas, const float* Rcw,
                                 const float* tcw, const float* twc, float fx, float fy, float cx, float cy, int width,
                                 int height, const EgsPolicy* pol, float* us, float* depths, float* cinv2ds,
                                 float* colors, int32_t* areas, void* rec, uint8_t* visible, float* dcolor_dpws,
                                 int flags, int key_bits_hint, void* ws_bin, size_t ws_bin_bytes,
                                 uint32_t* total_patches, uint32_t* host_totals, void* stream) {
  EGS_CHECK_ARG((flags & ~(EGS_FUSED_CULLED_LISTS | EGS_FUSED_ANTIALIASED | EGS_FUSED_RAW)) == 0);
  const bool cull_lists = (flags & EGS_FUSED_CULLED_LISTS) != 0;
  const bool aa = (flags & EGS_FUSED_ANTIALIASED) != 0;
  const bool raw = (flags & EGS_FUSED_RAW) != 0;
  EGS_CHECK_ARG(!aa || rec);
  EGS_CHECK_ARG(!raw || n == 0 || (rec && alphas));
  EGS_CHECK_ARG(raw || !shs_high);
  EGS_CHECK_ARG(n >= 0 && pol && width > 0 && height > 0 && total_patches);
  EGS_CHECK_ARG(!cull_lists || (rec && n < (1 << EGS_GSID_BITS)));
  EGS_CHECK_ARG(((uintptr_t)dcolor_dpws & 15) == 0);
  EGS_CHECK_ARG(width < 32768 && height < 32768);
  EGS_CHECK_ARG(sh_dim == 3 || sh_dim == 12 || sh_dim == 27 || sh_dim == 48);
  hipStream_t s = (hipStream_t)stream;
  if (n == 0) {
    EGS_HIP(hipMemsetAsync(total_patches, 0, 8, s));
    if (host_totals) EGS_HIP(hipMemcpyAsync(host_totals, total_patches, 8, hipMemcpyDeviceToHost, s));
    return 0;
  }
  EGS_CHECK_ARG(pws && rots && scales && shs && Rcw && tcw && twc && depths);
  EGS_CHECK_ARG(rec || (us && cinv2ds && colors && areas));
  EGS_CHECK_ARG(!rec || alphas);
  EGS_CHECK_ARG(ws_bin);
  EGS_CHECK_ARG(((uintptr_t)rots & 15) == 0);
  if (raw) EGS_CHECK_ARG(sh_dim == 3 || (shs_high && ((uintptr_t)shs_high & 15) == 0));
  else EGS_CHECK_ARG(sh_dim % 4 != 0 || ((uintptr_t)shs & 15) == 0);
  BinCountOut bo;
  if (!bin_count_outputs(ws_bin, ws_bin_bytes, n, &bo)) {
    set_error(EGS_ERR_WORKSPACE, "bin workspace too small", __FILE__, __LINE__);
    return EGS_ERR_WORKSPACE;
  }
  const BinParams bp = make_bin_params(width, height, pol, cull_lists);
  const PreParams pp = make_pre_params(pol, fx, fy, cx, cy, width, height);
  dim3 g(div_up(n, 256)), b(256);
  decltype(&k_preprocess_fwd<1, false, false, false>) kern = nullptr;
  with_sh_dim(sh_dim, [&](auto nc) {
    with_bools([&](auto raw_c, auto jw, auto aa_c) { kern = k_preprocess_fwd<nc.value, raw_c.value, jw.value, aa_c.value>; },
               raw, dcolor_dpws != nullptr, aa);
  });
  EGS_LAUNCH(aa ? "k_preprocess_fwd_aa" : "k_preprocess_fwd", kern, g, b, s, n, pp, pws, rots, scales, shs, shs_high,
             alphas, Rcw, tcw, twc, us, depths, cinv2ds, colors, areas, (float4*)rec, bp, bo, visible, dcolor_dpws);
  EGS_LAUNCH_OK();
  return splat_bin_after_count(n, key_bits_hint, ws_bin, ws_bin_bytes, total_patches, stream, host_totals);
}

extern "C" size_t egs_fused_backward_ws_bytes(int n) { return egs_splat_bwd_ws_bytes(n); }

extern "C" size_t egs_pose_ws_bytes(int n) { return align_up((size_t)div_up(n > 0 ? n : 1, 256) * 16 * sizeof(float), 256); }

extern "C" int egs_fused_backward(int n, int sh_dim, int64_t patches, int width, int height, const float* pws,
                                  const float* rots, const float* scales, const float* shs, const float* shs_high,
                                  const float* alphas, const float* Rcw, const float* tcw, const float* twc, float fx,
                                  float fy, float cx, float cy, const EgsPolicy* pol, const float* us,
                                  const float* cinv2ds, const float* colors, const int32_t* areas, const void* rec,
                                  const float* depths, const int32_t* contrib, const float* final_tau,
                                  const int32_t* patch_range_per_tile, const int32_t* gsid_per_patch,
                                  const float* dloss_dgammas, void* ws, size_t ws_bytes, float* dloss_dpws,
                                  float* dloss_dshs, float* dloss_dshs_high, float* dloss_dalphas,
                                  float* dloss_dscales, float* dloss_drots, float* dloss_dus,
                                  const int32_t* tile_order, float* grad_records, const float* dcolor_dpws, int phase,
                                  int row_begin, int row_count, void* seg_ws, size_t seg_ws_bytes, void* stream,
                                  const EgsExtras* extras, const EgsPoseGrad* pose) {
  EGS_CHECK_ARG(n >= 0 && pol && width > 0 && height > 0 && patches >= 0);
  const bool keep_order = (phase & EGS_BWD_KEEP_FORWARD_ORDER) != 0;
  const bool masked = (phase & EGS_FUSED_CULLED_LISTS) != 0;
  const int accum = ((phase & EGS_BWD_ACCUMULATE) ? 1 : 0) | ((phase & EGS_BWD_FACTORED_SH) ? 2 : 0);
  const bool factored = (phase & EGS_BWD_FACTORED_SH) != 0;
  const bool aa = (phase & EGS_FUSED_ANTIALIASED) != 0;
  const bool raw = (phase & EGS_FUSED_RAW) != 0;
  const bool absgrad = (phase & EGS_BWD_ABSGRAD) != 0;
  const bool pose_only = (phase & EGS_BWD_POSE_ONLY) != 0;
  phase &= ~(EGS_BWD_KEEP_FORWARD_ORDER | EGS_BWD_ACCUMULATE | EGS_BWD_FACTORED_SH | EGS_FUSED_CULLED_LISTS |
             EGS_FUSED_ANTIALIASED | EGS_FUSED_RAW | EGS_BWD_ABSGRAD | EGS_BWD_POSE_ONLY);
  EGS_CHECK_ARG(phase >= 0 && phase <= 2);
  EGS_CHECK_ARG(!pose_only || (pose && phase == 0 && !accum && !absgrad));
  EGS_CHECK_ARG(!absgrad || ((grad_records || n == 0) && !extras));
  EGS_CHECK_ARG(raw || (!shs_high && !dloss_dshs_high));
  if (pose) {
    EGS_CHECK_ARG(phase == 0 && pose->dloss_dRcw && pose->dloss_dtcw);
    if (pose->ws_bytes < egs_pose_ws_bytes(n) || !pose->ws) {
      set_error(EGS_ERR_WORKSPACE, "fused_backward pose workspace too small", __FILE__, __LINE__);
      return EGS_ERR_WORKSPACE;
    }
    if (n == 0) {
      EGS_HIP(hipMemsetAsync(pose->dloss_dRcw, 0, 9 * sizeof(float), (hipStream_t)stream));
      EGS_HIP(hipMemsetAsync(pose->dloss_dtcw, 0, 3 * sizeof(float), (hipStream_t)stream));
    }
  }
  if (phase != 2) { row_begin = 0; row_count = n; }
  EGS_CHECK_ARG(row_begin >= 0 && row_count >= 0 && row_begin + (int64_t)row_count <= n && row_begin % 256 == 0);
  EGS_CHECK_ARG(sh_dim == 3 || sh_dim == 12 || sh_dim == 27 || sh_dim == 48);
  if (n == 0) return 0;
  EGS_CHECK_ARG(pws && rots && scales && shs && alphas && Rcw && tcw && twc && depths && ws &&
                (pose_only || (dloss_dpws && dloss_dshs && dloss_dalphas && dloss_dscales && dloss_drots && dloss_dus)));
  if (raw) EGS_CHECK_ARG(rec && (sh_dim == 3 || (shs_high && (dloss_dshs_high || factored || pose_only))));
  if (ws_bytes < egs_splat_bwd_ws_bytes(n)) {
    set_error(EGS_ERR_WORKSPACE, "fused_backward workspace too small", __FILE__, __LINE__);
    return EGS_ERR_WORKSPACE;
  }
  float* gpack = grad_records ? grad_records : (float*)((char*)ws + align_up((size_t)n * 48, 256));
  if (phase != 2) {
    int rc = splat_bwd_packed(
        n, patches, width, height, pol,
        {.rec = rec, .us = us, .cinv2ds = cinv2ds, .alphas = alphas, .colors = colors, .areas = areas},
        {.contrib = contrib, .final_tau = final_tau, .ranges = patch_range_per_tile, .gsid = gsid_per_patch},
        dloss_dgammas, ws,
        {.tile_order = tile_order, .grad_records = grad_records, .keep_forward_order = keep_order, .masked_lists = masked,
         .seg_ws = seg_ws, .seg_ws_bytes = seg_ws_bytes, .extras = extras, .absgrad = absgrad},
        &gpack, stream);
    if (rc) return rc;
    if (phase == 1) return 0;
  }
  if (row_count == 0) return 0;
  const PreParams pp = make_pre_params(pol, fx, fy, cx, cy, width, height);
  const int kh = sh_dim - 3;
  const size_t r0 = (size_t)row_begin;
  dim3 g(div_up(row_count, 256)), b(256);
  hipStream_t s = (hipStream_t)stream;
  float* pose_ws = pose ? (float*)pose->ws : nullptr;
  const char* label = pose_only ? "k_preprocess_bwd_pose_only"
                      : aa      ? "k_preprocess_bwd_aa"
                      : pose    ? "k_preprocess_bwd_pose"
                      : extras  ? "k_preprocess_bwd_extra"
                                : "k_preprocess_bwd";
  const int sh_in = raw ? 3 : sh_dim, sh_out = (factored || raw) ? 3 : sh_dim;
  decltype(&k_preprocess_bwd<1, false, false, false, false, false, false>) kern = nullptr;
  with_sh_dim(sh_dim, [&](auto nc) {
    if (pose_only)
      with_bools(
          [&](auto raw_c, auto jw, auto extra, auto aa_c) {
            kern = k_preprocess_bwd<nc.value, raw_c.value, jw.value, extra.value, true, aa_c.value, true>;
          },
          raw, dcolor_dpws != nullptr, extras != nullptr, aa);
    else
      with_bools(
          [&](auto raw_c, auto jw, auto extra, auto pose_c, auto aa_c) {
            kern = k_preprocess_bwd<nc.value, raw_c.value, jw.value, extra.value, pose_c.value, aa_c.value, false>;
          },
          raw, dcolor_dpws != nullptr, extras != nullptr, pose != nullptr, aa);
  });
  EGS_LAUNCH(label, kern, g, b, s, row_count, pp, pws + 3 * r0, rots + 4 * r0, scales + 3 * r0, shs + sh_in * r0,
             (raw && shs_high) ? shs_high + kh * r0 : shs_high, alphas + r0, Rcw, tcw, twc, depths + r0,
             (const float4*)gpack + 3 * r0, dloss_dpws + 3 * r0, dloss_dshs + sh_out * r0,
             factored ? (row_begin == 0 ? dloss_dshs + 3 * (size_t)n : nullptr)
                      : ((raw && dloss_dshs_high) ? dloss_dshs_high + kh * r0 : dloss_dshs_high),
             dloss_dalphas + r0, dloss_dscales + 3 * r0, dloss_drots + 4 * r0, dloss_dus + 2 * r0,
             dcolor_dpws ? dcolor_dpws + 9 * r0 : dcolor_dpws, accum, pose_ws);
  EGS_LAUNCH_OK();
  if (pose) {
    EGS_LAUNCH("k_pose_reduce", k_pose_reduce, dim3(1), dim3(1024), s, (int)g.x, pose_ws, Rcw, tcw, pose->dloss_dRcw,
               pose->dloss_dtcw);
    EGS_LAUNCH_OK();
  }
  return 0;
}

extern "C" int egs_sh_grad_views(int n, int sh_dim, int views, const float* pws, const float* rows,
                                 int64_t row_stride, float scale, float* dloss_dshs, float* dloss_dhigh_shs,
                                 int accumulate, void* stream) {
  EGS_CHECK_ARG(n >= 0 && views >= 0);
  EGS_CHECK_ARG(sh_dim == 3 || sh_dim == 12 || sh_dim == 27 || sh_dim == 48);
  if (n == 0) return 0;
  EGS_CHECK_ARG(pws && dloss_dshs && (views == 0 || rows) && row_stride >= 3 * (int64_t)n + 3);
  const bool raw = dloss_dhigh_shs != nullptr;
  EGS_CHECK_ARG((((uintptr_t)dloss_dshs | (uintptr_t)dloss_dhigh_shs) & 15) == 0);
  dim3 g(div_up(n, 256)), b(256);
  hipStream_t s = (hipStream_t)stream;
  decltype(&k_sh_grad_views<1, false>) kern = nullptr;
  with_sh_dim(sh_dim, [&](auto nc) {
    with_bools([&](auto raw_c) { kern = k_sh_grad_views<nc.value, raw_c.value && nc.value != 1>; }, raw);
  });
  EGS_LAUNCH("k_sh_grad_views", kern, g, b, s, n, views, pws, rows, row_stride, scale, dloss_dshs, dloss_dhigh_shs,
             accumulate ? 1 : 0);
  EGS_LAUNCH_OK();
  return 0;
}
```

### easygaussiansplatting_amd/csrc/egs_raster.h

```cpp
#pragma once
#include "egs_gaussian_math.h"

namespace egs {

struct SortWs {
  uint32_t* hist;
  uint32_t* sup;
  size_t sup_words;
  int nblocks;
};
size_t sort_ws_bytes(int64_t n);
bool sort_ws_carve(Carver& cv, int64_t n, SortWs* w);
int sort_passes(int begin_bit, int end_bit);
int radix_sort(int64_t n, uint32_t* keys, uint32_t* vals, uint32_t* keys_alt, uint32_t* vals_alt, int begin_bit,
               int end_bit, const SortWs& w, hipStream_t s, const uint32_t* maxkey = nullptr,
               const uint32_t* n_dev = nullptr, uint32_t* mk_parts = nullptr, int nparts = 0,
               uint32_t* mk_out = nullptr, uint32_t* mk_host = nullptr, const uint4* gsrc = nullptr,
               uint4* gdst = nullptr, uint32_t* cdst = nullptr);
constexpr int SC_IPT = 8;
constexpr int SC_TILE = 256 * SC_IPT;
size_t scan_ws_bytes(int64_t n);

struct BinLayout {
  uint4 *cr, *cr_sorted;
  uint32_t* cnt_sorted;
  BinRec* br;
  uint32_t *dkeys, *dkeys_alt, *ids, *ids_alt, *offsets, *scan_partials, *maxkey;
  SortWs sort;
};
size_t bin_ws_bytes(int n);
bool bin_carve(void* ws, size_t bytes, int n, BinLayout* L);
int bin_emit(int n, int gx, const BinLayout& B, uint32_t* tkeys, uint32_t* gsid, uint32_t cap, int32_t* ranges,
             int n_ranges, int with_masks, uint32_t* sort_sup, uint32_t sort_sup_words, hipStream_t s);
int tile_ranges(int64_t P, const uint32_t* tkeys, int32_t* ranges, const uint32_t* n_dev, const uint32_t* masked,
                int32_t* plain, hipStream_t s, int32_t* zero = nullptr, int zero_words = 0, int32_t* walk_word = nullptr,
                uint32_t* walk_host = nullptr);
int pack_records(int n, int width, int height, int footprint, float alpha_skip, const float* us, const float* cinv2ds,
                 const float* alphas, const float* colors, const int32_t* areas, float4* rec, uint32_t* stamp,
                 const uint32_t* stamp_ref, uint8_t* same, hipStream_t s);

struct DrawParams {
  int W, H, gx, gy, T;
  float alpha_skip, tau_stop;
  float lskip;
  int maha_floor, alpha_clamp;
  int nan_blend;
  int map_mode;
  const int32_t* order;
  int ngrid;
  float4* zero_buf;
  uint32_t zero_n4, zero_per;
  int32_t* work_out;
  int32_t* walk_out;
  int32_t* walk_max;
  int masked;
};
DrawParams make_draw_params(int W, int H, const EgsPolicy* pol, bool backward = false);
struct DrawExtras {
  const float* depths;
  float* depth_out;
  float* alpha_out;
  const float* dl_depth;
  const float* dl_alpha;
  float bg[3];
};
int draw_grid(const DrawParams& p);
constexpr int TILE_ORDER_MAX_T = (16 + 24) * 1024;
int tile_order_enqueue(DrawParams& p, int32_t* buf, size_t buf_len, const int32_t* ranges, hipStream_t s,
                       const int32_t* work = nullptr, const int32_t* walk = nullptr, uint32_t* hint = nullptr);
int tile_work_from_contrib(const DrawParams& p, const int32_t* contrib, int32_t* work, int32_t* walk, hipStream_t s);
int launch_draw(const DrawParams& dp, const EgsPolicy* pol, int32_t* ranges, const int32_t* gsid, const float4* rec,
                float* image, int32_t* contrib, float* final_tau, const DrawExtras* ex, hipStream_t s);

constexpr int SEG_HDR = 16;
constexpr int SEG_SLOT_FLOATS = 256 * 6;
constexpr uint32_t SEG_TILE_MASK = 0x7FFFFu, SEG_SEG_MASK = 0x7FFu;
constexpr int SEG_SPEC = 1, SEG_COMPOSE = 2;
enum { SH_ITEMS1 = 0, SH_ITEMS3 = 1, SH_SLOTS = 2, SH_MAXLEN = 3, SH_SPLIT = 4, SH_L = 6, SH_MIN = 7,
       SH_MAXWALK = 8 ,
       SH_P_SLOTS = 10, SH_P_N3 = 11 ,
       SH_P_MAXLEN = 12, SH_P_MAXWALK = 13 };
constexpr int SEG_PLAN_BINS = 4096;
constexpr int SEG_PLAN_WORDS = SEG_HDR + 48 + SEG_PLAN_BINS;
struct SegArgs {
  int32_t* hdr;
  int32_t* seg_base;
  int32_t* walk;
  int32_t* items1;
  int32_t* items3;
  int32_t* tmp;
  int32_t* tmp2;
  float4* st4;
  float* st1;
  float* st2;
  int slot_cap, item_cap;
  int32_t* hist_walk;
  int rebuild;
  int32_t* walk_max;
};
struct SegConfig { int L, split_min; };
SegConfig seg_config();
size_t seg_ws_bytes_for(int64_t slots, int T);
bool seg_carve(void* ws, size_t bytes, int T, SegArgs* a);
int64_t seg_item_bound(int T, int64_t patches, const SegConfig& c);
int draw_segments_forward(DrawParams& dp, const EgsPolicy* pol, SegArgs& sga, const SegConfig& cfg, int64_t patches,
                          const int32_t* hist, int speculate, bool fix_pass, int32_t* walk_word, uint32_t* seg_hint,
                          bool plan_zeroed,
                          int32_t* ranges, const int32_t* gsid, const float4* rec, float* image, int32_t* contrib,
                          float* final_tau, hipStream_t s);
template <bool EXTRA> struct DrawBwdFlavour { SegArgs sg; };
template <> struct DrawBwdFlavour<true> { DrawExtras ex; };
int launch_draw_bwd(const DrawParams& dp, const EgsPolicy* pol, const int32_t* ranges, const int32_t* gsid,
                    const float4* rec, const float* final_tau, const int32_t* contrib, const float* dLdg, float* gpack,
                    const DrawExtras* ex, hipStream_t s, bool absgrad = false);
int launch_draw_bwd_seg(const DrawParams& dp, const EgsPolicy* pol, const int32_t* ranges, const int32_t* gsid,
                        const float4* rec, const float* final_tau, const int32_t* contrib, const float* dLdg,
                        float* gpack, const SegArgs& sga, int grid, hipStream_t s, bool absgrad = false);
int unpack_grads(int n, const float* gpack, float* dus, float* dcinv, float* dalpha, float* dcolor, hipStream_t s);

}
```

### easygaussiansplatting_amd/csrc/egs_sort.hip

```cpp
#include "egs_raster.h"

#include <algorithm>

namespace egs {

constexpr int RS_THREADS = 256;
constexpr int64_t RS_SHORT = 5 << 19;
static int rs_ipt(int64_t n) { return n <= RS_SHORT ? 8 : 16; }

constexpr int RS_SB = 32;
template <int RS_IPT>
__global__ __launch_bounds__(RS_THREADS) void k_radix_hist(const uint32_t* __restrict__ keys, int64_t n,
                                                           int shift, uint32_t dmask, int nblocks,
                                                           uint32_t* __restrict__ hist, uint32_t* __restrict__ sup,
                                                           const uint32_t* __restrict__ maxkey,
                                                           const uint32_t* __restrict__ n_dev,
                                                           uint32_t* __restrict__ mk_parts, int nparts,
                                                           uint32_t* __restrict__ mk_out,
                                                           uint32_t* __restrict__ mk_host) {
  constexpr int RS_TILE = RS_THREADS * RS_IPT;
  __shared__ uint32_t h[256];
  __shared__ uint32_t sm[4];
  const int tid = threadIdx.x;
  const int blk = mk_parts ? (int)blockIdx.x - 1 : (int)blockIdx.x;
  if (mk_parts && blockIdx.x == 0) {
    uint32_t mk = 0u;
    for (int i = tid; i < nparts; i += 256) mk = max(mk, mk_parts[1 + i]);
#pragma unroll
    for (int d = 32; d >= 1; d >>= 1) mk = max(mk, (uint32_t)__shfl_xor((int)mk, d, 64));
    if ((tid & 63) == 0) sm[tid >> 6] = mk;
    __syncthreads();
    if (tid == 0) {
      const uint32_t m = max(max(sm[0], sm[1]), max(sm[2], sm[3]));
      mk_parts[0] = m;
      if (mk_out) *mk_out = m;
      if (mk_host) *mk_host = m;
    }
    return;
  }
  if (!mk_parts && maxkey && ((*maxkey >> shift) == 0u)) return;
  if (n_dev) n = min(n, (int64_t)*n_dev);
  h[tid] = 0;
  __syncthreads();
  const int64_t base = (int64_t)blk * RS_TILE;
  if (base < n) {
    const uint32_t* kb = keys + base;
    const uint32_t rlast = (uint32_t)min(n - base, (int64_t)RS_TILE) - 1u;
    uint32_t k[RS_IPT];
#pragma unroll
    for (int r = 0; r < RS_IPT; ++r) k[r] = kb[min((uint32_t)(r * RS_THREADS + tid), rlast)];
#pragma unroll
    for (int r = 0; r < RS_IPT; ++r)
      if ((uint32_t)(r * RS_THREADS + tid) <= rlast) atomicAdd(&h[(k[r] >> shift) & dmask], 1u);
  }
  __syncthreads();
  const uint32_t c = h[tid];
  hist[(size_t)blk * 256 + tid] = c;
  if (c) atomicAdd(&sup[(size_t)(blk / RS_SB) * 256 + tid], c);
}

template <int RS_IPT, int EXTRA>
__global__ __launch_bounds__(RS_THREADS) __attribute__((amdgpu_waves_per_eu(4, 8))) void k_radix_scatter(
    const uint32_t* __restrict__ keys_in, const uint32_t* __restrict__ vals_in,
    uint32_t* __restrict__ keys_out, uint32_t* __restrict__ vals_out, int64_t n, int shift, uint32_t dmask,
    int nblocks, const uint32_t* __restrict__ hist, const uint32_t* __restrict__ sup,
    const uint32_t* __restrict__ maxkey, const uint32_t* __restrict__ n_dev,
    const uint4* __restrict__ gsrc, uint4* __restrict__ gdst, uint32_t* __restrict__ cdst) {
  if (n_dev) n = min(n, (int64_t)*n_dev);
  constexpr int RS_TILE = RS_THREADS * RS_IPT;
  constexpr int RS_WAVE_ITEMS = EGS_WAVE * RS_IPT;
  const int tid = threadIdx.x, wave = __builtin_amdgcn_readfirstlane(tid >> 6), lane = tid & 63;
  const int64_t blockbase = (int64_t)blockIdx.x * RS_TILE;
  if (blockbase >= n) return;
  if (maxkey && ((*maxkey >> shift) == 0u)) {
#pragma unroll
    for (int r = 0; r < RS_IPT; ++r) {
      const int64_t idx = blockbase + r * RS_THREADS + tid;
      if (idx < n) {
        const uint32_t v = vals_in[idx];
        keys_out[idx] = keys_in[idx];
        vals_out[idx] = v;
        if constexpr (EXTRA == 1) { const uint4 c = gsrc[v]; gdst[idx] = c; cdst[idx] = cr_count(c); }
      }
    }
    return;
  }
  __shared__ uint32_t wcount[4][256];
  __shared__ uint32_t dstart[256];
  __shared__ uint32_t gadj[256];
  __shared__ uint32_t sm[4];
  __shared__ uint32_t skey[RS_TILE], sval[RS_TILE];
#pragma unroll
  for (int w = 0; w < 4; ++w) wcount[w][tid] = 0;
  const int64_t base = blockbase + (int64_t)wave * RS_WAVE_ITEMS;
  uint32_t key[RS_IPT], val[RS_IPT], rank[RS_IPT];
  uint4 tot = make_uint4(0u, 0u, 0u, 0u), bef = tot;
  {
    const int sb = blockIdx.x / RS_SB, nsb = (nblocks + RS_SB - 1) / RS_SB;
    const uint4* sup4 = reinterpret_cast<const uint4*>(sup) + lane;
    const uint4* hist4 = reinterpret_cast<const uint4*>(hist) + lane;
    uint4 v[8], w[8];
    __builtin_amdgcn_sched_barrier(0);
#pragma unroll
    for (int r = 0; r < 8; ++r) v[r] = sup4[(size_t)min(wave + 4 * r, nsb - 1) * 64];
#pragma unroll
    for (int r = 0; r < 8; ++r) w[r] = hist4[(size_t)min(sb * RS_SB + wave + 4 * r, (int)blockIdx.x) * 64];
    const uint32_t* kb = keys_in + blockbase;
    const uint32_t* vb = vals_in + blockbase;
    const uint32_t rlast = (uint32_t)min(n - blockbase, (int64_t)RS_TILE) - 1u;
    uint32_t off[RS_IPT];
#pragma unroll
    for (int r = 0; r < RS_IPT; ++r) off[r] = min((uint32_t)(wave * RS_WAVE_ITEMS + r * EGS_WAVE + lane), rlast);
#pragma unroll
    for (int r = 0; r < RS_IPT; ++r) key[r] = kb[off[r]];
#pragma unroll
    for (int r = 0; r < RS_IPT; ++r) val[r] = vb[off[r]];
    __builtin_amdgcn_sched_barrier(0);
#pragma unroll
    for (int r = 0; r < 8; ++r) {
      const int q = wave + 4 * r;
      const uint32_t mt = q < nsb ? ~0u : 0u, mb = q < sb ? ~0u : 0u;
      tot.x += v[r].x & mt; tot.y += v[r].y & mt; tot.z += v[r].z & mt; tot.w += v[r].w & mt;
      bef.x += v[r].x & mb; bef.y += v[r].y & mb; bef.z += v[r].z & mb; bef.w += v[r].w & mb;
    }
#pragma unroll
    for (int r = 0; r < 8; ++r) {
      const uint32_t mb = (sb * RS_SB + wave + 4 * r < (int)blockIdx.x) ? ~0u : 0u;
      bef.x += w[r].x & mb; bef.y += w[r].y & mb; bef.z += w[r].z & mb; bef.w += w[r].w & mb;
    }
    for (int q0 = wave + 32; q0 < nsb; q0 += 32) {
#pragma unroll
      for (int r = 0; r < 8; ++r) v[r] = sup4[(size_t)min(q0 + 4 * r, nsb - 1) * 64];
#pragma unroll
      for (int r = 0; r < 8; ++r) {
        const int q = q0 + 4 * r;
        const uint32_t mt = q < nsb ? ~0u : 0u, mb = q < sb ? ~0u : 0u;
        tot.x += v[r].x & mt; tot.y += v[r].y & mt; tot.z += v[r].z & mt; tot.w += v[r].w & mt;
        bef.x += v[r].x & mb; bef.y += v[r].y & mb; bef.z += v[r].z & mb; bef.w += v[r].w & mb;
      }
    }
  }
  reinterpret_cast<uint4*>(skey)[wave * 64 + lane] = tot;
  reinterpret_cast<uint4*>(sval)[wave * 64 + lane] = bef;
  __syncthreads();
  const uint32_t dtotal = skey[tid] + skey[256 + tid] + skey[512 + tid] + skey[768 + tid];
  const uint32_t before = sval[tid] + sval[256 + tid] + sval[512 + tid] + sval[768 + tid];
  const uint32_t dig_ex = block256_exclusive_scan(dtotal, sm, nullptr);
  const uint32_t gbase = dig_ex + before;

  uint32_t* wc = wcount[wave];
  const int nbits = __popc(dmask);
#pragma unroll
  for (int r = 0; r < RS_IPT; ++r) {
    const int64_t idx = base + r * EGS_WAVE + lane;
    const bool valid = idx < n;
    const uint32_t d = (key[r] >> shift) & dmask;
    const uint64_t vb = __ballot(valid);
    uint32_t plo = (uint32_t)vb, phi = (uint32_t)(vb >> 32);
#pragma unroll
    for (int b = 0; b < 8; ++b) {
      if (b >= nbits) break;
      const uint32_t m = (uint32_t)((int32_t)(d << (31 - b)) >> 31);
      const uint64_t bal = __ballot(m != 0u);
      plo &= ~((uint32_t)bal ^ m);
      phi &= ~((uint32_t)(bal >> 32) ^ m);
    }
    const uint32_t below = __builtin_amdgcn_mbcnt_hi(phi, __builtin_amdgcn_mbcnt_lo(plo, 0u));
    uint32_t prev = 0;
    if (valid) prev = __hip_atomic_load(&wc[d], __ATOMIC_RELAXED, __HIP_MEMORY_SCOPE_WAVEFRONT);
    if (valid && below == 0)
      __hip_atomic_store(&wc[d], prev + (uint32_t)(__popc(plo) + __popc(phi)), __ATOMIC_RELAXED, __HIP_MEMORY_SCOPE_WAVEFRONT);
    __builtin_amdgcn_fence(__ATOMIC_ACQ_REL, "wavefront");
    rank[r] = prev + below;
  }
  __syncthreads();
  uint32_t cnt = 0;
  {
#pragma unroll
    for (int w = 0; w < 4; ++w) {
      const uint32_t c = wcount[w][tid];
      wcount[w][tid] = cnt;
      cnt += c;
    }
  }
  const uint32_t ds = block256_exclusive_scan(cnt, sm, nullptr);
  dstart[tid] = ds;
  gadj[tid] = gbase - ds;
  __syncthreads();
#pragma unroll
  for (int r = 0; r < RS_IPT; ++r) {
    const int64_t idx = base + r * EGS_WAVE + lane;
    if (idx < n) {
      const uint32_t d = (key[r] >> shift) & dmask;
      const uint32_t slot = dstart[d] + wcount[wave][d] + rank[r];
      skey[slot] = key[r];
      sval[slot] = val[r];
    }
  }
  __syncthreads();
  const int64_t rem = n - blockbase;
  const int nvalid = rem < RS_TILE ? (int)rem : RS_TILE;
  if constexpr (EXTRA == 1) {
    constexpr int G = 8;
#pragma unroll
    for (int r0 = 0; r0 < RS_IPT; r0 += G) {
      uint32_t ok[G], ov[G], op[G];
      uint4 oc[G];
#pragma unroll
      for (int r = 0; r < G; ++r) {
        const int slot = (r0 + r) * RS_THREADS + tid;
        ok[r] = 0u; ov[r] = 0u; op[r] = 0u; oc[r] = make_uint4(0u, 0u, 0u, 0u);
        if (slot < nvalid) {
          ok[r] = skey[slot];
          op[r] = gadj[(ok[r] >> shift) & dmask] + (uint32_t)slot;
          ov[r] = sval[slot];
          oc[r] = gsrc[ov[r]];
        }
      }
#pragma unroll
      for (int r = 0; r < G; ++r) asm volatile("" ::"v"(oc[r].x), "v"(oc[r].y), "v"(oc[r].z), "v"(oc[r].w));
#pragma unroll
      for (int r = 0; r < G; ++r) {
        const int slot = (r0 + r) * RS_THREADS + tid;
        if (slot < nvalid) {
          keys_out[op[r]] = ok[r];
          vals_out[op[r]] = ov[r];
          gdst[op[r]] = oc[r];
          cdst[op[r]] = cr_count(oc[r]);
        }
      }
    }
  } else {
#pragma unroll
    for (int r = 0; r < RS_IPT; ++r) {
      const int slot = r * RS_THREADS + tid;
      if (slot < nvalid) {
        const uint32_t k = skey[slot];
        const uint32_t pos = gadj[(k >> shift) & dmask] + (uint32_t)slot;
        keys_out[pos] = k;
        vals_out[pos] = sval[slot];
      }
    }
  }
}

static size_t sort_sup_words(int64_t n) {
  const int nb = n > 0 ? div_up(n, RS_THREADS * 8) : 1;
  return (size_t)4 * div_up(nb, RS_SB) * 256;
}
size_t sort_ws_bytes(int64_t n) {
  const int nb = n > 0 ? div_up(n, RS_THREADS * 8) : 1;
  return align_up((size_t)256 * nb * 4, 256) + align_up(sort_sup_words(n) * 4, 256) + 512;
}
bool sort_ws_carve(Carver& cv, int64_t n, SortWs* w) {
  w->nblocks = n > 0 ? div_up(n, RS_THREADS * rs_ipt(n)) : 1;
  w->hist = cv.take<uint32_t>((size_t)256 * w->nblocks);
  w->sup_words = sort_sup_words(n);
  w->sup = cv.take<uint32_t>(w->sup_words);
  return cv.ok();
}
int sort_passes(int begin_bit, int end_bit) { return (end_bit - begin_bit + 7) / 8; }

int radix_sort(int64_t n, uint32_t* keys, uint32_t* vals, uint32_t* keys_alt, uint32_t* vals_alt, int begin_bit,
               int end_bit, const SortWs& w, hipStream_t s, const uint32_t* maxkey, const uint32_t* n_dev,
               uint32_t* mk_parts, int nparts, uint32_t* mk_out, uint32_t* mk_host, const uint4* gsrc, uint4* gdst,
               uint32_t* cdst) {
  if (n <= 0) return 0;
  uint32_t *ki = keys, *vi = vals, *ko = keys_alt, *vo = vals_alt;
  const int passes = sort_passes(begin_bit, end_bit);
  const int width = (end_bit - begin_bit + passes - 1) / passes;
  int pass = 0;
  for (int shift = begin_bit; shift < end_bit; shift += width) {
    const int nb = end_bit - shift < width ? end_bit - shift : width;
    const uint32_t dmask = (1u << nb) - 1u;
    const bool first = shift == begin_bit && mk_parts != nullptr;
    const uint32_t* mk = first ? nullptr : maxkey;
    const bool last = shift + width >= end_bit;
    const uint4* gs = last ? gsrc : nullptr;
    uint32_t* sup = w.sup + (size_t)pass * div_up(w.nblocks, RS_SB) * 256;
    uint32_t* mkp = first ? mk_parts : (uint32_t*)nullptr;
    if (rs_ipt(n) == 8)
      EGS_LAUNCH("k_radix_hist", k_radix_hist<8>, dim3(w.nblocks + (mkp ? 1 : 0)), dim3(RS_THREADS), s, ki, n, shift, dmask,
                 w.nblocks, w.hist, sup, mk, n_dev, mkp, nparts, mk_out, mk_host);
    else
      EGS_LAUNCH("k_radix_hist", k_radix_hist<16>, dim3(w.nblocks + (mkp ? 1 : 0)), dim3(RS_THREADS), s, ki, n, shift, dmask,
                 w.nblocks, w.hist, sup, mk, n_dev, mkp, nparts, mk_out, mk_host);
    ++pass;
#define EGS_SCATTER(IPT, EXTRA)                                                                                     \
  EGS_LAUNCH("k_radix_scatter", (k_radix_scatter<IPT, EXTRA>), dim3(w.nblocks), dim3(RS_THREADS), s, ki, vi, ko, vo, n, \
             shift, dmask, w.nblocks, w.hist, sup, mk, n_dev, gs, gdst, cdst)
    if (rs_ipt(n) == 8) {
      if (gs) EGS_SCATTER(8, 1); else EGS_SCATTER(8, 0);
    } else {
      if (gs) EGS_SCATTER(16, 1); else EGS_SCATTER(16, 0);
    }
#undef EGS_SCATTER
    uint32_t* t = ki; ki = ko; ko = t;
    t = vi; vi = vo; vo = t;
  }
  EGS_LAUNCH_OK();
  return 0;
}


__global__ __launch_bounds__(256) void k_scan_partials(const uint32_t* __restrict__ in,
                                                       const uint32_t* __restrict__ gather, int64_t n,
                                                       uint32_t* __restrict__ partials) {
  __shared__ uint32_t sm[4];
  const int64_t base = (int64_t)blockIdx.x * SC_TILE + (int64_t)threadIdx.x * SC_IPT;
  uint32_t s = 0;
#pragma unroll
  for (int k = 0; k < SC_IPT; ++k) {
    const int64_t i = base + k;
    if (i < n) s += in[gather ? gather[i] : i];
  }
  s = wave_inclusive_scan(s);
  if ((threadIdx.x & 63) == 63) sm[threadIdx.x >> 6] = s;
  __syncthreads();
  if (threadIdx.x == 0) partials[blockIdx.x] = sm[0] + sm[1] + sm[2] + sm[3];
}

__global__ __launch_bounds__(256) void k_scan_apply(const uint32_t* __restrict__ in,
                                                    const uint32_t* __restrict__ gather, int64_t n,
                                                    const uint32_t* __restrict__ partials,
                                                    uint32_t* __restrict__ out, uint32_t* __restrict__ total) {
  __shared__ uint32_t sm[4];
  __shared__ uint32_t s_prefix;
  uint32_t pre = 0;
  for (int i = threadIdx.x; i < (int)blockIdx.x; i += 256) pre += partials[i];
  pre = wave_inclusive_scan(pre);
  if ((threadIdx.x & 63) == 63) sm[threadIdx.x >> 6] = pre;
  __syncthreads();
  if (threadIdx.x == 0) s_prefix = sm[0] + sm[1] + sm[2] + sm[3];
  __syncthreads();
  const uint32_t prefix = s_prefix;
  const int64_t base = (int64_t)blockIdx.x * SC_TILE + (int64_t)threadIdx.x * SC_IPT;
  uint32_t v[SC_IPT];
  uint32_t s = 0;
#pragma unroll
  for (int k = 0; k < SC_IPT; ++k) {
    const int64_t i = base + k;
    v[k] = (i < n) ? in[gather ? gather[i] : i] : 0u;
    s += v[k];
  }
  uint32_t blocksum;
  uint32_t ex = block256_exclusive_scan(s, sm, &blocksum) + prefix;
  if (total && blockIdx.x == gridDim.x - 1 && threadIdx.x == 0) *total = prefix + blocksum;
#pragma unroll
  for (int k = 0; k < SC_IPT; ++k) {
    const int64_t i = base + k;
    if (i < n) out[i] = ex;
    ex += v[k];
  }
}

size_t scan_ws_bytes(int64_t n) { return align_up((size_t)(n > 0 ? div_up(n, SC_TILE) : 1) * 4, 256) + 256; }

static int exclusive_scan(int64_t n, const uint32_t* in, const uint32_t* gather, uint32_t* out, uint32_t* total,
                          uint32_t* partials, hipStream_t s) {
  if (n <= 0) {
    if (total) EGS_HIP(hipMemsetAsync(total, 0, 4, s));
    return 0;
  }
  const int nb = div_up(n, SC_TILE);
  EGS_LAUNCH("k_scan_partials", k_scan_partials, dim3(nb), dim3(256), s, in, gather, n, partials);
  EGS_LAUNCH("k_scan_apply", k_scan_apply, dim3(nb), dim3(256), s, in, gather, n, partials, out, total);
  EGS_LAUNCH_OK();
  return 0;
}

}

using namespace egs;

extern "C" size_t egs_sort_pairs_ws_bytes(int64_t n) { return sort_ws_bytes(n); }

extern "C" int egs_sort_pairs(int64_t n, uint32_t* keys, uint32_t* vals, uint32_t* keys_alt, uint32_t* vals_alt,
                              int begin_bit, int end_bit, void* ws, size_t ws_bytes, int* result_in_alt_host,
                              void* stream) {
  EGS_CHECK_ARG(n >= 0 && begin_bit >= 0 && end_bit <= 32 && begin_bit <= end_bit);
  if (result_in_alt_host) *result_in_alt_host = (n > 0) ? (sort_passes(begin_bit, end_bit) & 1) : 0;
  if (n == 0 || begin_bit == end_bit) {
    if (result_in_alt_host) *result_in_alt_host = 0;
    return 0;
  }
  EGS_CHECK_ARG(keys && vals && keys_alt && vals_alt && ws);
  Carver cv(ws, ws_bytes);
  SortWs w;
  if (!sort_ws_carve(cv, n, &w)) {
    set_error(EGS_ERR_WORKSPACE, "sort workspace too small", __FILE__, __LINE__);
    return EGS_ERR_WORKSPACE;
  }
  EGS_HIP(hipMemsetAsync(w.sup, 0, w.sup_words * 4, (hipStream_t)stream));
  return radix_sort(n, keys, vals, keys_alt, vals_alt, begin_bit, end_bit, w, (hipStream_t)stream);
}

extern "C" size_t egs_scan_ws_bytes(int64_t n) { return scan_ws_bytes(n); }

extern "C" int egs_exclusive_scan_u32(int64_t n, const uint32_t* in, const uint32_t* gather, uint32_t* out,
                                      uint32_t* total, void* ws, size_t ws_bytes, void* stream) {
  EGS_CHECK_ARG(n >= 0);
  EGS_CHECK_ARG(n == 0 || (in && out && ws));
  if (ws_bytes < scan_ws_bytes(n)) {
    set_error(EGS_ERR_WORKSPACE, "scan workspace too small", __FILE__, __LINE__);
    return EGS_ERR_WORKSPACE;
  }
  return exclusive_scan(n, in, gather, out, total, (uint32_t*)ws, (hipStream_t)stream);
}
```

### easygaussiansplatting_amd/csrc/egs_splat.hip

```cpp
#include "egs_raster.h"

#include <algorithm>
#include <cstring>

namespace egs {

static int tile_bits(int T) {
  int b = 1;
  while ((1 << b) < T) ++b;
  return b;
}

struct DrawLayout {
  uint32_t *tkeys, *tkeys_alt, *gsid_alt;
  float4* rec;
  int32_t* order;
  SortWs sort;
};
static size_t draw_ws_bytes(int n, int64_t P, int width, int height) {
  const size_t N = (size_t)(n > 0 ? n : 1), PP = (size_t)(P > 0 ? P : 1);
  const size_t ord = (size_t)div_up(width, EGS_TILE) * div_up(height, EGS_TILE);
  return 3 * align_up(PP * 4, 256) + align_up(N * 48, 256) + align_up(ord * 4, 256) + sort_ws_bytes(P) + 4096;
}
static bool draw_carve(void* ws, size_t bytes, int n, int64_t P, int width, int height, DrawLayout* L) {
// ... 21 lines not shown
  return ex;
}

int splat_bwd_packed(int n, int64_t patches, int width, int height, const EgsPolicy* pol, const SplatSource& src,
                     const SplatForward& fwd, const float* dloss_dgammas, void* ws, const SplatCarry& carry,
                     float** gpack_out, void* stream) {
  hipStream_t s = (hipStream_t)stream;
  const float4* rec = src.rec ? (const float4*)src.rec : (const float4*)ws;
  float* gpack = carry.grad_records ? carry.grad_records : (float*)((char*)ws + align_up((size_t)n * 48, 256));
  *gpack_out = gpack;
  if (!carry.grad_records) EGS_HIP(hipMemsetAsync(gpack, 0, (size_t)n * 48, s));
  if (patches == 0) return 0;
  EGS_CHECK_ARG(fwd.contrib && fwd.final_tau && fwd.ranges && fwd.gsid && dloss_dgammas);
  EGS_CHECK_ARG(!carry.extras || (carry.extras->depths && !carry.seg_ws));
  EGS_CHECK_ARG(!(carry.absgrad && carry.extras));
  EGS_CHECK_ARG(src.rec || (src.us && src.cinv2ds && src.alphas && src.colors && (src.areas || pol->footprint == 0)));
  DrawParams dp = make_draw_params(width, height, pol, true);
  dp.masked = (carry.masked_lists && pol->footprint == 0 && pol->alpha_skip > 0.f) ? 1 : 0;
  if (!src.rec) {
    const int rc = pack_records(n, width, height, pol->footprint, pol->alpha_skip, src.us, src.cinv2ds, src.alphas,
                                src.colors, src.areas, (float4*)ws, nullptr, nullptr, nullptr, s);
    if (rc) return rc;
  }
  if (carry.seg_ws) {
    SegArgs sga;
    const size_t hw = (size_t)width * height;
    const size_t scratch = carry.rebuild ? align_up(20 * hw, 256) + 256 : 0;
    if (pol->footprint != 0 || !(pol->alpha_skip > 0.f) || !(pol->tau_stop > 0.f) || carry.seg_ws_bytes <= scratch ||
        !seg_carve(carry.seg_ws, carry.seg_ws_bytes - scratch, dp.T, &sga)) {
      set_error(EGS_ERR_WORKSPACE, "segment workspace too small (or a policy without a skip / stop threshold)", __FILE__, __LINE__);
      return EGS_ERR_WORKSPACE;
    }
    const int grid = sga.item_cap;
    if (carry.rebuild) {
      sga.rebuild = 1;
      char* sc = (char*)(((uintptr_t)carry.seg_ws + carry.seg_ws_bytes - scratch + 255) & ~(uintptr_t)255);
      float* simg = (float*)sc;
      int32_t* scont = (int32_t*)(sc + 12 * hw);
      float* stau = (float*)(sc + 16 * hw);
      DrawParams fp = make_draw_params(width, height, pol);
      fp.masked = dp.masked;
      int32_t* rg = const_cast<int32_t*>(fwd.ranges);
      int rc = tile_work_from_contrib(dp, fwd.contrib, nullptr, sga.walk, s);
      if (rc) return rc;
      rc = draw_segments_forward(fp, pol, sga, seg_config(), patches, (const int32_t*)sga.walk, 0, true, nullptr,
                                 carry.seg_hint, false, rg, fwd.gsid, rec, simg, scont, stau, s);
      if (rc) return rc;
    }
    return launch_draw_bwd_seg(dp, pol, fwd.ranges, fwd.gsid, rec, fwd.final_tau, fwd.contrib, dloss_dgammas,
                               gpack, sga, grid, s, carry.absgrad);
  }
  if (carry.tile_order && (carry.keep_forward_order || (size_t)dp.T > BWD_ORDER_CAP)) {
    dp.order = carry.tile_order;
    dp.ngrid = dp.T;
  } else if (carry.tile_order) {
    int32_t* order = (int32_t*)((char*)ws + 2 * align_up((size_t)n * 48, 256));
    const int32_t* wk = carry.tile_order + dp.T;
    const int rc = tile_order_enqueue(dp, order, BWD_ORDER_CAP, fwd.ranges, s, wk,
                                      carry.seg_hint ? wk + dp.T : nullptr, carry.seg_hint);
    if (rc) return rc;
  } else {
    int32_t* order = (int32_t*)((char*)ws + 2 * align_up((size_t)n * 48, 256));
    int32_t* work = nullptr;
    int32_t* walk = nullptr;
    if (2 * (size_t)dp.T <= BWD_ORDER_CAP) {
      work = order + dp.T;
      if (carry.seg_hint && 3 * (size_t)dp.T <= BWD_ORDER_CAP) walk = work + dp.T;
      const int rc = tile_work_from_contrib(dp, fwd.contrib, work, walk, s);
      if (rc) return rc;
    }
    const int rc = tile_order_enqueue(dp, order, BWD_ORDER_CAP, fwd.ranges, s, work, walk,
                                      walk ? carry.seg_hint : nullptr);
    if (rc) return rc;
  }
  const DrawExtras ex = draw_extras(carry.extras);
  return launch_draw_bwd(dp, pol, fwd.ranges, fwd.gsid, rec, fwd.final_tau, fwd.contrib, dloss_dgammas, gpack,
                         carry.extras ? &ex : nullptr, s, carry.absgrad);
}
}

using namespace egs;

extern "C" size_t egs_splat_draw_ws_bytes(int n, int64_t patches, int width, int height) {
  return draw_ws_bytes(n, patches, width, height);
}

struct DrawOptions {
  const uint32_t* patches_dev;
  int32_t* tile_order;
  float* grad_records;
  const int32_t* prev_tile_work;
  int order_ready;
  int flags;
  int32_t* gsid_plain;
  void* seg_ws;
  size_t seg_ws_bytes;
  uint32_t* seg_hint;
  int32_t* walk_word;
  const EgsExtras* extras;
};

static int splat_draw_impl(int n, int64_t patches, int width, int height, const EgsPolicy* pol, const SplatSource& src,
                           const void* ws_bin, void* ws_draw, size_t ws_draw_bytes, float* image, int32_t* contrib,
                           float* final_tau, int32_t* patch_range_per_tile, int32_t* gsid_per_patch,
                           const DrawOptions& o, void* stream) {
  EGS_CHECK_ARG(n >= 0 && patches >= 0 && patches < (int64_t)0x7FFFFFFF && width > 0 && height > 0 && pol);
  EGS_CHECK_ARG(image && contrib && final_tau && patch_range_per_tile);
  EGS_CHECK_ARG(!o.extras || ((o.extras->depths || n == 0) && !o.seg_ws));
  hipStream_t s = (hipStream_t)stream;
  DrawParams dp = make_draw_params(width, height, pol);
  const bool masked = (o.flags & (EGS_DRAW_CULLED_LISTS | EGS_DRAW_MASKED_LISTS)) && pol->footprint == 0 &&
                      pol->alpha_skip > 0.f;
  EGS_CHECK_ARG(!masked || n < (1 << EGS_GSID_BITS));
  dp.masked = masked ? 1 : 0;
  if (o.grad_records && n > 0 && (patches == 0)) EGS_HIP(hipMemsetAsync(o.grad_records, 0, (size_t)n * 48, s));
  if (n == 0 || patches == 0) {
    const size_t hw = (size_t)width * height;
    EGS_HIP(hipMemsetAsync(patch_range_per_tile, 0, (size_t)dp.T * 8, s));
    EGS_HIP(hipMemsetAsync(image, 0, 12 * hw, s));
    EGS_HIP(hipMemsetAsync(contrib, 0, 4 * hw, s));
    EGS_HIP(hipMemsetAsync(final_tau, 0, 4 * hw, s));
    if (o.extras) {
      for (int c = 0; c < 3; ++c) {
        uint32_t bits;
        memcpy(&bits, &o.extras->background[c], 4);
        EGS_HIP(hipMemsetD32Async((hipDeviceptr_t)(image + c * hw), (int)bits, hw, s));
      }
      if (o.extras->depth_out) EGS_HIP(hipMemsetAsync(o.extras->depth_out, 0, 4 * hw, s));
      if (o.extras->alpha_out) EGS_HIP(hipMemsetAsync(o.extras->alpha_out, 0, 4 * hw, s));
    }
    if (o.tile_order) {
      if (!o.order_ready) {
        const int rc = tile_order_enqueue(dp, o.tile_order, (size_t)dp.T, patch_range_per_tile, s, nullptr);
        if (rc) return rc;
      }
      EGS_HIP(hipMemsetAsync(o.tile_order + dp.T, 0, (size_t)dp.T * 8, s));
    }
    if (o.seg_ws) {
      SegArgs sa;
      if (seg_carve(o.seg_ws, o.seg_ws_bytes, dp.T, &sa)) EGS_HIP(hipMemsetAsync(sa.hdr, 0, SEG_HDR * 4, s));
    }
    return 0;
  }
  EGS_CHECK_ARG(ws_bin && ws_draw && gsid_per_patch);
  EGS_CHECK_ARG(src.rec || (src.us && src.cinv2ds && src.alphas && src.colors && src.areas));
  BinLayout B;
  if (!bin_carve(const_cast<void*>(ws_bin), bin_ws_bytes(n), n, &B)) return EGS_ERR_WORKSPACE;
  DrawLayout D;
  if (!draw_carve(ws_draw, ws_draw_bytes, n, patches, width, height, &D)) {
    set_error(EGS_ERR_WORKSPACE, "draw workspace too small", __FILE__, __LINE__);
    return EGS_ERR_WORKSPACE;
  }
  const int tb = tile_bits(dp.T);
  const int passes = sort_passes(0, tb);
  uint32_t* gs_primary = (uint32_t*)gsid_per_patch;
  uint32_t* k0 = (passes & 1) ? D.tkeys_alt : D.tkeys;
  uint32_t* k1 = (passes & 1) ? D.tkeys : D.tkeys_alt;
  uint32_t* v0 = (passes & 1) ? D.gsid_alt : gs_primary;
  uint32_t* v1 = (passes & 1) ? gs_primary : D.gsid_alt;
  int rc = bin_emit(n, dp.gx, B, k0, v0, (uint32_t)patches, patch_range_per_tile, 2 * dp.T, dp.masked, D.sort.sup,
                    (uint32_t)D.sort.sup_words, s);
  if (rc) return rc;
  const float4* rec = src.rec ? (const float4*)src.rec : D.rec;
  if (!src.rec) {
    rc = pack_records(n, width, height, pol->footprint, pol->alpha_skip, src.us, src.cinv2ds, src.alphas, src.colors,
                      src.areas, D.rec, nullptr, nullptr, nullptr, s);
    if (rc) return rc;
  }
  rc = radix_sort(patches, k0, v0, k1, v1, 0, tb, D.sort, s, nullptr, o.patches_dev);
  if (rc) return rc;
  SegArgs sga;
  const bool seg = o.seg_ws && pol->footprint == 0 && pol->alpha_skip > 0.f && pol->tau_stop > 0.f &&
                   dp.T <= (int)SEG_TILE_MASK && seg_carve(o.seg_ws, o.seg_ws_bytes, dp.T, &sga);
  rc = tile_ranges(patches, D.tkeys, patch_range_per_tile, o.patches_dev,
                   (const uint32_t*)(o.gsid_plain ? gsid_per_patch : nullptr), o.gsid_plain, s, seg ? sga.hdr : nullptr,
                   seg ? SEG_PLAN_WORDS : 0, o.walk_word, o.seg_hint);
  if (rc) return rc;
  if (o.seg_ws && !seg) {
    set_error(EGS_ERR_WORKSPACE, "segment workspace too small (or a policy without a skip / stop threshold)", __FILE__, __LINE__);
    return EGS_ERR_WORKSPACE;
  }
  if (seg) {
    const SegConfig cfg = seg_config();
    const int32_t* hist = (o.tile_order && (o.flags & EGS_DRAW_SEG_HISTORY)) ? o.tile_order + 2 * dp.T : nullptr;
    sga.hist_walk = o.tile_order ? o.tile_order + 2 * dp.T : nullptr;
    const int speculate = (o.flags & EGS_DRAW_SEG_SPECULATE) ? 1 : 0;
    if (o.tile_order) dp.work_out = o.tile_order + dp.T;
    if (o.grad_records) {
      dp.zero_buf = (float4*)o.grad_records;
      dp.zero_n4 = (uint32_t)(3 * (size_t)n);
    }
    return draw_segments_forward(dp, pol, sga, cfg, patches, hist, speculate, hist || speculate, o.walk_word,
                                 o.seg_hint, true, patch_range_per_tile, gsid_per_patch, rec, image, contrib, final_tau, s);
  }
  if (o.order_ready && o.tile_order && dp.T <= TILE_ORDER_MAX_T) {
    dp.order = o.tile_order;
    dp.ngrid = dp.T;
  } else {
    rc = tile_order_enqueue(dp, o.tile_order ? o.tile_order : D.order, (size_t)dp.T, patch_range_per_tile, s,
                            o.prev_tile_work, nullptr, o.walk_word ? nullptr : o.seg_hint);
    if (rc) return rc;
  }
  if (o.tile_order) { dp.work_out = o.tile_order + dp.T; dp.walk_out = dp.work_out + dp.T; }
  if (o.tile_order) dp.walk_max = o.walk_word;
  if (o.grad_records) {
    dp.zero_buf = (float4*)o.grad_records;
    dp.zero_n4 = (uint32_t)(3 * (size_t)n);
    dp.zero_per = (dp.zero_n4 + (uint32_t)draw_grid(dp) - 1) / (uint32_t)draw_grid(dp);
  }
  const DrawExtras ex = draw_extras(o.extras);
  return launch_draw(dp, pol, patch_range_per_tile, gsid_per_patch, rec, image, contrib, final_tau,
                     o.extras ? &ex : nullptr, s);
}

extern "C" int egs_splat_draw(int n, int64_t patches, int width, int height, const float* us,
                              const float* cinv2ds, const float* alphas, const float* colors,
                              const int32_t* areas, const EgsPolicy* pol, const void* ws_bin, void* ws_draw,
                              size_t ws_draw_bytes, float* image, int32_t* contrib, float* final_tau,
                              int32_t* patch_range_per_tile, int32_t* gsid_per_patch, void* stream) {
  return splat_draw_impl(n, patches, width, height, pol,
                         {.us = us, .cinv2ds = cinv2ds, .alphas = alphas, .colors = colors, .areas = areas}, ws_bin,
                         ws_draw, ws_draw_bytes, image, contrib, final_tau, patch_range_per_tile, gsid_per_patch,
                         DrawOptions{}, stream);
}

extern "C" int egs_splat_draw_rec_seg(int n, int64_t patches, const uint32_t* total_patches, int width, int height,
                                      const void* rec, const EgsPolicy* pol, const void* ws_bin, void* ws_draw,
                                      size_t ws_draw_bytes, float* image, int32_t* contrib, float* final_tau,
                                      int32_t* patch_range_per_tile, int32_t* gsid_per_patch, int32_t* tile_order,
                                      float* grad_records, const int32_t* prev_tile_work, int order_ready, int flags,
                                      void* seg_ws, size_t seg_ws_bytes, uint32_t* seg_hint, int32_t* walk_word,
                                      int32_t* gsid_plain, void* stream, const EgsExtras* extras) {
  EGS_CHECK_ARG((rec || n == 0) && (!total_patches || patches > 0));
  EGS_CHECK_ARG(!gsid_plain || ((((uintptr_t)gsid_plain | (uintptr_t)gsid_per_patch) & 15) == 0));
  return splat_draw_impl(n, patches, width, height, pol, {.rec = rec}, ws_bin, ws_draw, ws_draw_bytes, image, contrib,
                         final_tau, patch_range_per_tile, gsid_per_patch,
                         {.patches_dev = total_patches, .tile_order = tile_order, .grad_records = grad_records,
                          .prev_tile_work = prev_tile_work, .order_ready = order_ready, .flags = flags,
                          .gsid_plain = gsid_plain, .seg_ws = seg_ws, .seg_ws_bytes = seg_ws_bytes, .seg_hint = seg_hint,
                          .walk_word = walk_word, .extras = extras},
                         stream);
}

extern "C" size_t egs_splat_bwd_ws_bytes(int n) {
  return 2 * align_up((size_t)(n > 0 ? n : 1) * 48, 256) + BWD_ORDER_CAP * 4 + 256;
}
extern "C" size_t egs_seg_rebuild_ws_bytes(int64_t patch_capacity, int width, int height) {
  return egs_seg_ws_bytes(patch_capacity, width, height) + align_up((size_t)20 * width * height, 256) + 512;
}

static int splat_bwd_unpacked(int n, int64_t patches, int width, int height, const EgsPolicy* pol,
                              const SplatSource& src, const SplatForward& fwd, const float* dloss_dgammas, void* ws,
                              size_t ws_bytes, const SplatCarry& carry, float* dloss_dus, float* dloss_dcinv2ds,
                              float* dloss_dalphas, float* dloss_dcolors, void* stream) {
  EGS_CHECK_ARG(n >= 0 && patches >= 0 && width > 0 && height > 0 && pol);
  if (n == 0) return 0;
  EGS_CHECK_ARG(ws && dloss_dus && dloss_dcinv2ds && dloss_dalphas && dloss_dcolors);
  if (ws_bytes < egs_splat_bwd_ws_bytes(n)) {
    set_error(EGS_ERR_WORKSPACE, "splat_bwd workspace too small", __FILE__, __LINE__);
    return EGS_ERR_WORKSPACE;
  }
  float* gpack = nullptr;
  const int rc = splat_bwd_packed(n, patches, width, height, pol, src, fwd, dloss_dgammas, ws, carry, &gpack, stream);
  if (rc) return rc;
  return unpack_grads(n, gpack, dloss_dus, dloss_dcinv2ds, dloss_dalphas, dloss_dcolors, (hipStream_t)stream);
}

extern "C" int egs_splat_bwd_seg(int n, int64_t patches, int width, int height, const float* us, const float* cinv2ds,
                                 const float* alphas, const float* colors, const void* rec, const EgsPolicy* pol,
                                 const int32_t* contrib, const float* final_tau, const int32_t* patch_range_per_tile,
                                 const int32_t* gsid_per_patch, const float* dloss_dgammas, void* ws, size_t ws_bytes,
                                 const int32_t* tile_order, float* grad_records, float* dloss_dus,
                                 float* dloss_dcinv2ds, float* dloss_dalphas, float* dloss_dcolors, int flags,
                                 void* seg_ws, size_t seg_ws_bytes, int rebuild, uint32_t* seg_hint, void* stream) {
  EGS_CHECK_ARG(n <= 0 || !pol || rec || (us && cinv2ds && alphas && colors && pol->footprint != 1));
  return splat_bwd_unpacked(n, patches, width, height, pol,
                            {.rec = rec, .us = us, .cinv2ds = cinv2ds, .alphas = alphas, .colors = colors},
                            {.contrib = contrib, .final_tau = final_tau, .ranges = patch_range_per_tile,
                             .gsid = gsid_per_patch},
                            dloss_dgammas, ws, ws_bytes,
                            {.tile_order = tile_order, .grad_records = grad_records,
                             .masked_lists = (flags & (EGS_DRAW_CULLED_LISTS | EGS_DRAW_MASKED_LISTS)) != 0,
                             .seg_ws = seg_ws, .seg_ws_bytes = seg_ws_bytes, .rebuild = rebuild, .seg_hint = seg_hint},
                            dloss_dus, dloss_dcinv2ds, dloss_dalphas, dloss_dcolors, stream);
}

extern "C" int egs_splat_bwd(int n, int64_t patches, int width, int height, const float* us,
                             const float* cinv2ds, const float* alphas, const float* colors,
                             const int32_t* areas, const EgsPolicy* pol, const int32_t* contrib,
                             const float* final_tau, const int32_t* patch_range_per_tile,
                             const int32_t* gsid_per_patch, const float* dloss_dgammas, void* ws, size_t ws_bytes,
                             float* dloss_dus, float* dloss_dcinv2ds, float* dloss_dalphas, float* dloss_dcolors,
                             void* stream) {
  return splat_bwd_unpacked(n, patches, width, height, pol,
                            {.us = us, .cinv2ds = cinv2ds, .alphas = alphas, .colors = colors, .areas = areas},
                            {.contrib = contrib, .final_tau = final_tau, .ranges = patch_range_per_tile,
                             .gsid = gsid_per_patch},
                            dloss_dgammas, ws, ws_bytes, SplatCarry{}, dloss_dus, dloss_dcinv2ds, dloss_dalphas,
                            dloss_dcolors, stream);
}
```

### easygaussiansplatting_amd/fused.py

```python
from __future__ import annotations

import collections
import ctypes as C
import os
import weakref

import torch

from . import _ahead, _lib
from ._ahead import (_ctx, _seg_decision, _settle, _tls, _walk_word,
                     commit, deferred, expect_long_walks, seg_hint)
from ._host import _alphas, _chk, _lib_on, _pol, _ptr, _stream, _tiles
from .dist_views import flat_grad_buffer


ENQUEUE_AHEAD = os.environ.get("EGS_ENQUEUE_AHEAD", "1") != "0"
MAILBOX_COPY = os.environ.get("EGS_MAILBOX_COPY", "0") == "1"
REUSE_ORDER = os.environ.get("EGS_BWD_REUSE_ORDER", "1") != "0"
KEEP_FORWARD_ORDER = 16
ORDER_REFRESH = max(2, int(os.environ.get("EGS_TILE_ORDER_REFRESH", "4")))
TILE_WORK_CACHE = os.environ.get("EGS_TILE_WORK_CACHE", "1") != "0"
SAVE_DCOLOR = os.environ.get("EGS_SAVE_DCOLOR", "1") != "0"
CULL_LISTS = os.environ.get("EGS_CULL_LISTS", "1") != "0"
SEGMENTS = os.environ.get("EGS_SEGMENTS", "auto")
DRAW_CULLED_LISTS = 1
DRAW_MASKED_LISTS = 2
SEG_HISTORY = 4
SEG_SPECULATE_FLAG = 8
SEG_SPECULATE = os.environ.get("EGS_SEG_SPECULATE", "auto")
ACCUMULATE = 64
FACTORED_SH = 128
ABSGRAD = 1024
POSE_ONLY = 2048
CULLED_LISTS = 32
ANTIALIASED = 256
RAW = 512
GSID_MASK = 0x0FFFFFFF


class FusedState:
    __slots__ = ("us", "depths", "cinv2ds", "colors", "areas", "rec", "contrib", "final_tau", "ranges", "gsid",
                 "order", "order_by_work", "gpack", "dcw", "flags", "width", "height", "ticket", "_patches", "_keep",
                 "seg", "extras")

    @property
    def culled(self):
        return bool(self.flags & CULLED_LISTS)

    @property
    def antialiased(self):
        return bool(self.flags & ANTIALIASED)

    def patch_count(self) -> int:
        if self.ticket is not None:
            _settle(self.ticket, True)
        return self._patches

    def gaussian_ids(self):
        g = self.gsid[:self.patch_count()]
        return (g & GSID_MASK) if self.culled else g

    def block_masks(self):
        g = self.gsid[:self.patch_count()]
        return ((g >> 28) & 15) if self.culled else torch.full_like(g, 15)


class Extras(collections.namedtuple("Extras", ("depth", "alpha", "background"))):
    __slots__ = ()

    def background_rgb(self):
        return (0.0, 0.0, 0.0) if self.background is None else tuple(float(v) for v in self.background)


def _egs_extras(depths, bg, depth_out=None, alpha_out=None, dloss_ddepth=None, dloss_dalpha=None):
    ex = _lib.EgsExtras()
    ex.depths = depths.data_ptr() if depths is not None else None
    ex.depth_out = depth_out.data_ptr() if depth_out is not None else None
    ex.alpha_out = alpha_out.data_ptr() if alpha_out is not None else None
    ex.background[:] = bg
    ex.dloss_ddepth = dloss_ddepth.data_ptr() if dloss_ddepth is not None else None
    ex.dloss_dalpha = dloss_dalpha.data_ptr() if dloss_dalpha is not None else None
    return ex


def pose_tensors(Rcw, tcw, like):
    pair = ((Rcw, "Rcw", (3, 3)), (tcw, "tcw", (3,)))
    for t, name, shape in pair:
        if not isinstance(t, torch.Tensor):
            raise ValueError("pose %s must be a torch.Tensor, got %s" % (name, type(t).__name__))
        if tuple(t.shape) != shape:
            raise ValueError("pose %s must have shape %s, got %s" % (name, list(shape), list(t.shape)))
        if t.dtype != torch.float32:
            raise ValueError("pose %s must be torch.float32, got %s" % (name, t.dtype))
    for t, name, _ in pair:
        if not t.is_cuda or t.device != like.device:
            raise ValueError("pose %s must live on the device of the Gaussians (%s), got %s" % (name, like.device,
                                                                                                 t.device))
    return Rcw.contiguous(), tcw.contiguous()


_exchange_hook = None
_sh_sink = None


def _split_sh(low_shs, high_shs, n):
    low = _chk(low_shs, "low_shs", torch.float32, (n, 3))
    high = _chk(high_shs, "high_shs", torch.float32, (n, None))
    K = 3 + high.shape[1]
    if K not in (3, 12, 27, 48):
        raise ValueError("low_shs + high_shs must have 3, 12, 27 or 48 columns, got %d" % K)
    return low, high, K


def forward(pws, shs, alphas, scales, rots, cam, high_shs=None, need_grad=False, extras=None, antialiased=False):
    raw = high_shs is not None
    pws = _chk(pws, "pws", torch.float32, (None, 3))
    n = pws.shape[0]
    if raw:
        shs, high_shs, K = _split_sh(shs, high_shs, n)
    else:
        shs = _chk(shs, "shs", torch.float32, (n, None))
        K = shs.shape[1]
        if K not in (3, 12, 27, 48):
            raise ValueError("shs must have 3, 12, 27 or 48 columns, got %d" % K)
    alphas = _alphas(alphas, n)
    scales = _chk(scales, "scales", torch.float32, (n, 3))
    rots = _chk(rots, "rots", torch.float32, (n, 4))
    Rcw = _chk(cam.Rcw, "cam.Rcw", torch.float32, (3, 3))
    tcw = _chk(cam.tcw, "cam.tcw", torch.float32, (3,))
    twc = _chk(cam.twc, "cam.twc", torch.float32, (3,))
    W, H = int(cam.width), int(cam.height)
    lib = _lib_on(pws)
    dev = pws.device
    pol = C.byref(_pol())
    st = _stream()
    f32, i32 = torch.float32, torch.int32
    S = FusedState()
    S.width, S.height = W, H
    S.ticket, S._patches, S._keep, S.seg, S.extras = None, None, None, None, None
    S.us = S.cinv2ds = S.colors = S.areas = None
    pol_ = _pol()
    culled = CULL_LISTS and pol_.footprint == 0 and pol_.alpha_skip > 0 and n < (1 << 28)
    S.flags = (CULLED_LISTS if culled else 0) | (ANTIALIASED if antialiased else 0) | (RAW if raw else 0)
    S.depths = torch.empty((n,), dtype=f32, device=dev)
    S.rec = torch.empty((max(n, 1), 12), dtype=f32, device=dev)
    mask = torch.empty((n,), dtype=torch.bool, device=dev)
    ws_bin_bytes = lib.egs_splat_bin_ws_bytes(n)
    ws_bin = torch.empty(ws_bin_bytes, dtype=torch.uint8, device=dev)
    enqueue_bin = lambda hint, total, host_slot: _lib.check(lib.egs_fused_forward(
        n, K, _ptr(pws), _ptr(rots), _ptr(scales), _ptr(shs), _ptr(high_shs), _ptr(alphas), _ptr(Rcw), _ptr(tcw),
        _ptr(twc), float(cam.fx), float(cam.fy), float(cam.cx), float(cam.cy), W, H, pol, _ptr(S.us), _ptr(S.depths),
        _ptr(S.cinv2ds), _ptr(S.colors), _ptr(S.areas), _ptr(S.rec), _ptr(mask), _ptr(S.dcw), S.flags, hint,
        _ptr(ws_bin), ws_bin_bytes, _ptr(total), host_slot, st))
    image = torch.empty((3, H, W), dtype=f32, device=dev)
    depth_map = alpha_map = None
    ex = None
    if extras is not None:
        S.extras = extras
        if extras.depth:
            depth_map = torch.empty((1, H, W), dtype=f32, device=dev)
        if extras.alpha:
            alpha_map = torch.empty((1, H, W), dtype=f32, device=dev)
        ex = _egs_extras(S.depths, extras.background_rgb(), depth_map, alpha_map)
    done = (lambda: (image, mask, S)) if extras is None else (lambda: (image, mask, S, depth_map, alpha_map))
    S.contrib = torch.empty((H, W), dtype=i32, device=dev)
    S.final_tau = torch.empty((H, W), dtype=f32, device=dev)
    S.ranges = torch.empty((_tiles(W, H), 2), dtype=i32, device=dev)
    S.order = None
    S.gpack = torch.empty((max(n, 1), 12), dtype=f32, device=dev) if (need_grad and n > 0) else None
    S.dcw = torch.empty((n, 9), dtype=f32, device=dev) if (need_grad and n > 0 and SAVE_DCOLOR) else None

    def draw(rows, total, redo):
        S.gsid = torch.empty(rows, dtype=i32, device=dev)
        ws_draw = torch.empty(lib.egs_splat_draw_ws_bytes(n, rows, W, H), dtype=torch.uint8, device=dev)
        if use_seg:
            S.seg = torch.empty(lib.egs_seg_ws_bytes(max(rows, 1), W, H), dtype=torch.uint8, device=dev)
        _lib.check(lib.egs_splat_draw_rec_seg(
            n, rows, _ptr(total), W, H, _ptr(S.rec), pol, _ptr(ws_bin), _ptr(ws_draw), ws_draw.numel(), _ptr(image),
            _ptr(S.contrib), _ptr(S.final_tau), _ptr(S.ranges), _ptr(S.gsid), _ptr(S.order), _ptr(S.gpack), prev_work,
            order_ready, draw_flags, _ptr(S.seg), S.seg.numel() if S.seg is not None else 0,
            None if (redo and walk_word is not None) else seg_hint, _ptr(walk_word), None, st,
            None if ex is None else C.byref(ex)))
        remember_order()

    ctx = _ctx(dev)
    key = (n, W, H)
    S.ticket = None
    prev_work, order_ready = None, 0
    cache_entry = None
    use_seg, seg_hint, speculate = _seg_decision(ctx, lib, key, pol_, SEGMENTS, SEG_SPECULATE) if n > 0 \
        else (False, None, False)
    if extras is not None:
        use_seg = False
    walk_word = _walk_word(ctx, key, dev, st, seg_hint is not None)
    walk_known = False
    if TILE_WORK_CACHE and n > 0:
        ck = (id(cam), int(st.value or 0))
        olen = lib.egs_tile_order_len(W, H)
        with ctx.lock:
            hit = ctx.tile_work.get(ck)
            if hit is not None and hit[0]() is cam and hit[1].numel() == olen and hit[3] == (n, W, H):
                S.order = hit[1]
                renders = hit[2] + (0 if use_seg else 1)
                walk_known = True
                if not use_seg:
                    if renders <= 2 or renders % ORDER_REFRESH == 0:
                        prev_work = C.c_void_p(S.order.data_ptr() + 4 * (olen - 2 * _tiles(W, H)))
                    else:
                        order_ready = 1
            else:
                S.order = torch.empty(olen, dtype=i32, device=dev)
                renders = 0 if use_seg else 1
        cache_entry = (ck, renders)
    if S.order is None:
        S.order = torch.empty(lib.egs_tile_order_len(W, H), dtype=i32, device=dev)

    def remember_order():
        if cache_entry is None:
            return
        ck, renders = cache_entry
        tw = ctx.tile_work

        def drop(_ref, ck=ck, tw=tw, lock=ctx.lock):
            with lock:
                ent = tw.get(ck)
                if ent is not None and ent[0] is _ref:
                    del tw[ck]
        try:
            ref = weakref.ref(cam, drop)
        except TypeError:
            return
        with ctx.lock:
            tw[ck] = (ref, S.order, renders, (n, W, H))
    S.order_by_work = prev_work is not None or order_ready == 1
    draw_flags = (DRAW_CULLED_LISTS if culled else 0) | (SEG_HISTORY if (use_seg and walk_known) else 0) | \
        (SEG_SPECULATE_FLAG if (use_seg and speculate) else 0)
    cap = ctx.capacity.get(key, 0) if (ENQUEUE_AHEAD and n > 0) else 0
    patches = _ahead.render(ctx, dev, key, st, cap, _ahead.wait_slot, enqueue_bin, draw, S,
                            getattr(_tls, "deferred", False), MAILBOX_COPY)
    if patches is not None:
        S._patches = patches
    return done()


_pad_index = {}


class accumulate_in_kernel:

    def __enter__(self):
        self._prev = getattr(_acc_flag, "on", False)
        _acc_flag.on = True
        return self

    def __exit__(self, et, ev, tb):
        _acc_flag.on = self._prev
        return False


class _AccFlag:
    on = False


_acc_flag = _AccFlag()


def _engine_accumulates_into(node_ctx, count):
    try:
        nodes = [fn for fn, _ in node_ctx.next_functions[:count]]
        return all(fn is not None and torch._C._will_engine_execute_node(fn) for fn in nodes)
    except Exception:
        return False


DEFAULT = object()


def sh_sink_for(node_ctx, count, sh_tensors, explicit=None):
    sink, hook = (_sh_sink, _exchange_hook) if explicit is None else explicit
    if sink is None or not all(t.is_leaf and t.requires_grad for t in sh_tensors) or \
            not _engine_accumulates_into(node_ctx, count):
        return None
    if hook is not None:
        raise RuntimeError("FactoredShGrad and ChunkedExchange cannot be attached together (the overlapped exchange "
                           "all-reduces the SH rows the factored form never writes)")
    return sink


def accumulation_targets(leaves, node_ctx=None, count=None, explicit=None):
    on, hook = (getattr(_acc_flag, "on", False), _exchange_hook) if explicit is None else explicit
    if not on or hook is not None:
        return None
    if node_ctx is not None and not _engine_accumulates_into(node_ctx, len(leaves) if count is None else count):
        return None
    grads = []
    for t in leaves:
        g = t.grad if (t.is_leaf and t.requires_grad) else None
        if g is None or g.dtype != torch.float32 or not g.is_contiguous() or g.shape != t.shape or \
                (g.data_ptr() & 15) or g.device != t.device:
            return None
        grads.append(g)
    if flat_grad_buffer(leaves) is None:
        return None
    return grads


def backward(pws, shs, alphas, scales, rots, cam, S: FusedState, dloss_dgammas, high_shs=None, accumulate=None,
             sh_sink=None, exchange=DEFAULT, dloss_ddepth=None, dloss_dalpha=None, pose=None, absgrad=False,
             pose_only=False):
    raw = high_shs is not None
    pws = _chk(pws, "pws", torch.float32, (None, 3))
    n = pws.shape[0]
    if raw:
        shs, high_shs, K = _split_sh(shs, high_shs, n)
    else:
        shs = _chk(shs, "shs", torch.float32, (n, None))
        K = shs.shape[1]
    alphas = _alphas(alphas, n)
    scales = _chk(scales, "scales", torch.float32, (n, 3))
    rots = _chk(rots, "rots", torch.float32, (n, 4))
    if raw != bool(S.flags & RAW):
        raise ValueError("fused.backward: the inputs must have the layout of the forward call (raw tensors with "
                         "high_shs, or activated ones without)")
    W, H = S.width, S.height
    dl = _chk(dloss_dgammas, "dloss_dgammas", torch.float32, (3, H, W))
    rx = getattr(S, "extras", None)
    ex = None
    if rx is not None:
        dd = _chk(dloss_ddepth, "dloss_ddepth", torch.float32, (1, H, W)) if dloss_ddepth is not None else None
        da = _chk(dloss_dalpha, "dloss_dalpha", torch.float32, (1, H, W)) if dloss_dalpha is not None else None
        ex = _egs_extras(S.depths, rx.background_rgb(), dloss_ddepth=dd, dloss_dalpha=da)
    elif dloss_ddepth is not None or dloss_dalpha is not None:
        raise ValueError("fused.backward: depth / alpha gradients for a render without extras")
    if absgrad and rx is not None:
        raise ValueError("fused.backward: absgrad is not available for a render with extras (depth / alpha / background)")
    lib = _lib_on(pws)
    dev = pws.device
    f32 = torch.float32
    pg = None
    hook = _exchange_hook if exchange is DEFAULT else exchange
    if pose_only:
        if pose is None:
            raise ValueError("fused.backward: pose_only needs pose=(Rcw, tcw)")
        for v, name in ((accumulate, "accumulate"), (sh_sink, "sh_sink"), (absgrad or None, "absgrad"),
                        (hook, "a ChunkedExchange")):
            if v is not None:
                raise ValueError("fused.backward: pose_only writes no per-Gaussian gradient and does not combine with "
# ... 100 lines not shown
```

### include/egs_hip.h

```cpp
#ifndef EGS_HIP_H_
#define EGS_HIP_H_

#include <stddef.h>
#include <stdint.h>

#ifdef __cplusplus
extern "C" {
#endif

#define EGS_ABI_VERSION 12

#define EGS_ERR_BAD_ARG 10001
#define EGS_ERR_WORKSPACE 10002

typedef struct EgsPolicy {
  int32_t near_cull;
  int32_t fov_mode;
  float det_eps;
  int32_t nan_cull;
  int32_t radius_mode;
  int32_t footprint;
  int32_t far_cull;
  int32_t maha_floor;
  int32_t alpha_clamp;
  float alpha_skip;
  float tau_stop;
  int32_t depth_key;
  int32_t nan_maha;
} EgsPolicy;

void egs_policy_gsplatcu(EgsPolicy* p);
void egs_policy_forward_cpu(EgsPolicy* p);

int egs_abi_version(void);
const char* egs_last_error_string(void);


int egs_project(int n, const float* pws, const float* Rcw, const float* tcw, float fx, float fy,
                float cx, float cy, const EgsPolicy* pol, float* us, float* pcs, float* depths,
                float* du_dpcs, void* stream);

int egs_cov3d(int n, const float* rots, const float* scales, const float* depths, const EgsPolicy* pol,
              float* cov3ds, float* dcov3d_drots, float* dcov3d_dscales, void* stream);

int egs_cov2d(int n, const float* cov3ds, const float* pcs, const float* Rcw, const float* depths,
              float fx, float fy, float width, float height, const EgsPolicy* pol, float* cov2ds,
              float* dcov2d_dcov3ds, float* dcov2d_dpcs, void* stream);

int egs_sh2color(int n, int sh_dim, const float* shs, const float* pws, const float* twc,
                 float* colors, float* dcolor_dshs, float* dcolor_dpws, void* stream);

int egs_inv_cov2d(int n, const float* cov2ds, float* depths, const EgsPolicy* pol, float* cinv2ds,
                  int32_t* areas, float* dcinv2d_dcov2ds, void* stream);

size_t egs_splat_bin_ws_bytes(int n);
size_t egs_splat_draw_ws_bytes(int n, int64_t patches, int width, int height);

int egs_splat_bin(int n, int width, int height, const float* us, int32_t* areas, float* depths,
                  const EgsPolicy* pol, int key_bits_hint, void* ws_bin, size_t ws_bin_bytes,
                  uint32_t* total_patches, void* stream);

int egs_splat_draw(int n, int64_t patches, int width, int height, const float* us,
                   const float* cinv2ds, const float* alphas, const float* colors, const int32_t* areas,
                   const EgsPolicy* pol, const void* ws_bin, void* ws_draw, size_t ws_draw_bytes,
                   float* image, int32_t* contrib, float* final_tau, int32_t* patch_range_per_tile,
                   int32_t* gsid_per_patch, void* stream);

size_t egs_splat_bwd_ws_bytes(int n);
int egs_splat_bwd(int n, int64_t patches, int width, int height, const float* us, const float* cinv2ds,
                  const float* alphas, const float* colors, const int32_t* areas, const EgsPolicy* pol,
                  const int32_t* contrib, const float* final_tau, const int32_t* patch_range_per_tile,
                  const int32_t* gsid_per_patch, const float* dloss_dgammas, void* ws, size_t ws_bytes,
                  float* dloss_dus, float* dloss_dcinv2ds, float* dloss_dalphas, float* dloss_dcolors,
                  void* stream);

int egs_splat_bin_mb(int n, int width, int height, const float* us, int32_t* areas, float* depths,
                     const EgsPolicy* pol, int key_bits_hint, void* ws_bin, size_t ws_bin_bytes,
                     uint32_t* total_patches, uint32_t* host_totals , void* stream);

int egs_pack_records(int n, int width, int height, const float* us, const float* cinv2ds, const float* alphas,
                     const float* colors, const int32_t* areas , const EgsPolicy* pol,
                     void* rec, void* stream);
int egs_splat_bin_pack(int n, int width, int height, const float* us, const float* cinv2ds, const float* alphas,
                       const float* colors, int32_t* areas, float* depths, const EgsPolicy* pol, int key_bits_hint,
                       void* ws_bin, size_t ws_bin_bytes, uint32_t* total_patches, uint32_t* host_totals, void* rec,
                       uint32_t* stamp ,
                       uint8_t* visible ,
                       void* stream);
size_t egs_pair_stamp_words(int n);
int egs_pack_records_validate(int n, int width, int height, const float* us, const float* cinv2ds,
                              const float* alphas, const float* colors, const EgsPolicy* pol, void* rec,
                              const uint32_t* stamp_a, uint32_t* stamp_b, int64_t patches, void* kept,
                              const int32_t* plain, void* stream);
int egs_words_differ(const void* a, const void* b, int64_t n_words, int32_t* flag, void* stream);

#define EGS_DRAW_CULLED_LISTS 1
#define EGS_DRAW_MASKED_LISTS 2
#define EGS_DRAW_SEG_HISTORY 4
#define EGS_DRAW_SEG_SPECULATE 8
size_t egs_tile_order_len(int width, int height);
size_t egs_seg_ws_bytes(int64_t patch_capacity, int width, int height);
int egs_seg_config(int segment_len, int split_min, int* out2);
typedef struct EgsExtras {
  const float* depths;
  float* depth_out;
  float* alpha_out;
  float background[3];
  const float* dloss_ddepth;
  const float* dloss_dalpha;
} EgsExtras;
int egs_splat_draw_rec_seg(int n, int64_t patches, const uint32_t* total_patches, int width, int height,
                           const void* rec, const EgsPolicy* pol, const void* ws_bin, void* ws_draw,
                           size_t ws_draw_bytes, float* image, int32_t* contrib, float* final_tau,
                           int32_t* patch_range_per_tile, int32_t* gsid_per_patch, int32_t* tile_order,
                           float* grad_records, const int32_t* prev_tile_work, int order_ready, int flags, void* seg_ws,
                           size_t seg_ws_bytes, uint32_t* seg_hint, int32_t* walk_word, int32_t* gsid_plain,
                           void* stream, const EgsExtras* extras);
size_t egs_seg_rebuild_ws_bytes(int64_t patch_capacity, int width, int height);
int egs_splat_bwd_seg(int n, int64_t patches, int width, int height, const float* us, const float* cinv2ds,
                      const float* alphas, const float* colors, const void* rec, const EgsPolicy* pol,
                      const int32_t* contrib, const float* final_tau, const int32_t* patch_range_per_tile,
                      const int32_t* gsid_per_patch, const float* dloss_dgammas, void* ws, size_t ws_bytes,
                      const int32_t* tile_order, float* grad_records, float* dloss_dus, float* dloss_dcinv2ds,
                      float* dloss_dalphas, float* dloss_dcolors, int flags, void* seg_ws, size_t seg_ws_bytes,
                      int rebuild, uint32_t* seg_hint, void* stream);


size_t egs_sort_pairs_ws_bytes(int64_t n);
int egs_sort_pairs(int64_t n, uint32_t* keys, uint32_t* vals, uint32_t* keys_alt, uint32_t* vals_alt,
                   int begin_bit, int end_bit, void* ws, size_t ws_bytes, int* result_in_alt_host,
                   void* stream);

size_t egs_scan_ws_bytes(int64_t n);
int egs_exclusive_scan_u32(int64_t n, const uint32_t* in, const uint32_t* gather, uint32_t* out,
                           uint32_t* total, void* ws, size_t ws_bytes, void* stream);

int egs_chain_rule(int n, int sh_dim, const float* dloss_dus, const float* dloss_dcinv2ds,
                   const float* dloss_dcolors, const float* Rcw, const float* dcinv2d_dcov2ds,
                   const float* dcov2d_dcov3ds, const float* dcov3d_drots, const float* dcov3d_dscales,
                   const float* dcolor_dshs, const float* du_dpcs, const float* dcov2d_dpcs,
                   const float* dcolor_dpws, float* dloss_dpws, float* dloss_dshs, float* dloss_dscales,
                   float* dloss_drots, void* stream);

#define EGS_FUSED_CULLED_LISTS 32
#define EGS_FUSED_ANTIALIASED 256
#define EGS_FUSED_RAW 512
int egs_fused_forward(int n, int sh_dim, const float* pws, const float* rots, const float* scales,
                      const float* shs, const float* high_shs , const float* alphas,
                      const float* Rcw, const float* tcw, const float* twc, float fx, float fy, float cx, float cy,
                      int width, int height, const EgsPolicy* pol, float* us, float* depths, float* cinv2ds,
                      float* colors, int32_t* areas, void* rec, uint8_t* visible, float* dcolor_dpws ,
                      int flags , int key_bits_hint, void* ws_bin, size_t ws_bin_bytes,
                      uint32_t* total_patches, uint32_t* host_totals, void* stream);
int egs_hbm_copy_probe(void* dst, const void* src, size_t bytes, void* stream);
int egs_clock_probe(void* out8, int iters, void* stream);
void* egs_mailbox_create(int slots);
void egs_mailbox_destroy(void* mailbox);
int egs_mailbox_post(void* mailbox, int slot, const uint32_t* total_patches, void* stream);
uint32_t* egs_mailbox_slot(void* mailbox, int slot);
int egs_mailbox_arm(void* mailbox, int slot, void* stream);
int egs_mailbox_fetch(void* mailbox, int slot, int blocking, uint32_t* out2);
int egs_mailbox_peek(void* mailbox, int slot, uint32_t* out4);
int egs_mailbox_clear(void* mailbox, int slot);
size_t egs_fused_backward_ws_bytes(int n);
#define EGS_BWD_KEEP_FORWARD_ORDER 16
#define EGS_BWD_ACCUMULATE 64
#define EGS_BWD_FACTORED_SH 128
#define EGS_BWD_ABSGRAD 1024
int egs_grad_records_absgrad(int n, const float* grad_records, float* dloss_dus_abs , void* stream);
#define EGS_BWD_POSE_ONLY 2048
typedef struct EgsPoseGrad {
  float* dloss_dRcw;
  float* dloss_dtcw;
  void* ws;
  size_t ws_bytes;
} EgsPoseGrad;
size_t egs_pose_ws_bytes(int n);
int egs_fused_backward(int n, int sh_dim, int64_t patches, int width, int height, const float* pws,
                       const float* rots, const float* scales, const float* shs, const float* shs_high,
                       const float* alphas, const float* Rcw, const float* tcw, const float* twc, float fx, float fy,
                       float cx, float cy, const EgsPolicy* pol, const float* us, const float* cinv2ds,
                       const float* colors, const int32_t* areas, const void* rec , const float* depths,
                       const int32_t* contrib, const float* final_tau, const int32_t* patch_range_per_tile,
                       const int32_t* gsid_per_patch, const float* dloss_dgammas, void* ws, size_t ws_bytes,
                       float* dloss_dpws, float* dloss_dshs, float* dloss_dhigh_shs, float* dloss_dalphas,
                       float* dloss_dscales, float* dloss_drots, float* dloss_dus,
                       const int32_t* tile_order ,
                       float* grad_records ,
                       const float* dcolor_dpws , int phase, int row_begin,
                       int row_count, void* seg_ws ,
                       size_t seg_ws_bytes, void* stream, const EgsExtras* extras ,
                       const EgsPoseGrad* pose );
int egs_sh_grad_views(int n, int sh_dim, int views, const float* pws, const float* rows, int64_t row_stride,
                      float scale, float* dloss_dshs, float* dloss_dhigh_shs , int accumulate,
                      void* stream);


size_t egs_gau_loss_ws_bytes(int height, int width);
int egs_gau_loss(int height, int width, const float* image, const float* gt_image, float loss_lambda,
                 float grad_scale, void* ws, size_t ws_bytes, float* loss_out, float* dloss_dimage,
                 void* stream);

typedef struct EgsGaussianParams {
  float* pws;
  float* low_shs;
  float* high_shs;
  float* alphas_raw;
  float* scales_raw;
  float* rots_raw;
} EgsGaussianParams;

int egs_density_accumulate(int n, const float* dloss_dus, const uint8_t* visible, int first, float* grad_accum,
                           int32_t* count, void* stream);

size_t egs_densify_ws_bytes(int n);
int egs_densify_plan(int n, const float* alphas_raw, const float* scales_raw, const float* grad_accum,
                     const int32_t* count, float alpha_thr_raw, float big_thr_raw, float grad_thr, float scale_thr,
                     uint8_t* cls, void* ws, size_t ws_bytes, int32_t* totals, void* stream);
int egs_densify_apply(int n, int n_keep, int n_clone, int n_split, int high_sh_width, const uint8_t* cls,
                      const void* ws, const EgsGaussianParams* in, const EgsGaussianParams* in_exp_avg,
                      const EgsGaussianParams* in_exp_avg_sq, const EgsGaussianParams* out,
                      const EgsGaussianParams* out_exp_avg, const EgsGaussianParams* out_exp_avg_sq,
                      const float* unit_noise, uint64_t seed, uint64_t round, void* stream);

int egs_reset_alpha(int n, float raw_val, float* alphas_raw, float* exp_avg, float* exp_avg_sq, void* stream);

typedef struct EgsAdamGroup {
  float* param;
  const float* grad;
  float* exp_avg;
  float* exp_avg_sq;
  int64_t count;
  float lr;
  int32_t step;
} EgsAdamGroup;
int egs_adam_step(int n_groups, const EgsAdamGroup* groups, double beta1, double beta2, double eps, void* stream);
int egs_adam_sh_factored(int n, int sh_dim, int views, const float* pws, const float* rows, int64_t row_stride,
                         float scale, const EgsAdamGroup* low, const EgsAdamGroup* high , double beta1,
                         double beta2, double eps, void* stream);

size_t egs_nn_sqdist_ws_bytes(int n);
int egs_nn_sqdist(int n, const float* points, void* ws, size_t ws_bytes, float* out_sqdist, void* stream);

int egs_viewer_prep(int n, int sh_dim, const float* gs_data, const float* view_matrix,
                    const float* projection_matrix, float focal_x, float focal_y, float* gs_prep, float* depth,
                    int flags , void* stream);

int egs_prof_enable(int on);
void egs_prof_set_filter(const char* kernel_name);
void egs_prof_reset(void);
int egs_prof_report(char* buf, size_t cap);

#ifdef __cplusplus
}
#endif
#endif
```

Before: 2470 Mpix/s.

## Replace global depth radix sort with per-tile depth sort via composite tile-depth keys

Adds a tile-depth-sort path that skips the global radix sort of Gaussians by depth. Instead it emits patch keys as (tile << dbits | depth bits) in unsorted Gaussian order, computes offsets directly from the count records, and sorts each tile's short list by depth in a new per-tile LDS sort kernel. The goal is to remove the full-size depth sort and its copies from the binning stage. The path is enabled by default but falls back when tile plus depth bits exceed 32 or when the longest list exceeds the 2048 cap. In exchange it adds a per-tile sort kernel, wider keys, and extra host-side gating logic.

```diff
diff --git a/easygaussiansplatting_amd/_ahead.py b/easygaussiansplatting_amd/_ahead.py
--- a/easygaussiansplatting_amd/_ahead.py
+++ b/easygaussiansplatting_amd/_ahead.py
@@ -97,6 +97,26 @@
     if low[0] >= KEY_BITS_DECAY:
         _key_bits[k] = low[1]
         _key_low.pop(k, None)
+
+
+def tile_bits(tiles) -> int:
+    b = 1
+    while (1 << b) < tiles:
+        b += 1
+    return b
+
+
+def tile_depth_bits(enabled, tiles, hint, longest, cap) -> int:
+    dbits = 32 if (hint <= 0 or hint > 32) else int(hint)
+    if not enabled or tile_bits(tiles) + dbits > 32:
+        return 0
+    if longest is not None and longest > cap:
+        return 0
+    return dbits
+
+
+def draw_depth_flags(dbits, flag, shift) -> int:
+    return (flag | (dbits << shift)) if dbits else 0
 
 
 def _bin_stage(enqueue, device, key=None):
diff --git a/easygaussiansplatting_amd/_tilesortlib.py b/easygaussiansplatting_amd/_tilesortlib.py
--- /dev/null
+++ b/easygaussiansplatting_amd/_tilesortlib.py
@@ -0,0 +1,36 @@
+from __future__ import annotations
+
+import ctypes as C
+import os
+
+from ._lib import load_library
+
+_HERE = os.path.dirname(os.path.abspath(__file__))
+LIB_PATH = os.path.join(_HERE, "libegs_tilesort.so")
+ABI_VERSION = 1
+CAP = 2048
+
+_P = C.c_void_p
+_i = C.c_int
+
+SIGNATURES = {
+    "egs_tilesort_abi_version": (_i, []),
+    "egs_tilesort_last_error_string": (C.c_char_p, []),
+    "egs_tile_depth_sort_cap": (_i, []),
+    "egs_tile_depth_sort": (_i, [_i, _P, _P, _P, _P, _P, C.c_int64, _i, _P]),
+}
+
+_lib = None
+
+
+def load():
+    global _lib
+    if _lib is None:
+        _lib = load_library(LIB_PATH, SIGNATURES, "egs_tilesort_abi_version", ABI_VERSION)
+    return _lib
+
+
+def check(rc: int):
+    if rc != 0:
+        msg = load().egs_tilesort_last_error_string().decode("utf-8", "replace")
+        raise RuntimeError(msg)
diff --git a/easygaussiansplatting_amd/csrc/egs_bin.hip b/easygaussiansplatting_amd/csrc/egs_bin.hip
--- a/easygaussiansplatting_amd/csrc/egs_bin.hip
+++ b/easygaussiansplatting_amd/csrc/egs_bin.hip
@@ -143,35 +143,69 @@
   }
 }
 
-__global__ __launch_bounds__(256) void k_bin_scan_partials(const uint32_t* __restrict__ cnt_sorted, int64_t n,
-                                                           uint32_t* __restrict__ partials) {
+template <bool CR>
+__global__ __launch_bounds__(256) void k_bin_scan_partials(const uint32_t* __restrict__ cnt_sorted,
+                                                           const uint4* __restrict__ cr, int64_t n,
+                                                           uint32_t* __restrict__ partials,
+                                                           uint32_t* __restrict__ mk_parts, int nparts,
+                                                           uint32_t* __restrict__ mk_out,
+                                                           uint32_t* __restrict__ mk_host) {
   __shared__ uint32_t sm[4];
-  const int64_t base = (int64_t)blockIdx.x * SC_TILE + (int64_t)threadIdx.x * SC_IPT;
   uint32_t s = 0;
-  if (base + SC_IPT <= n) {
-    const uint4 a = *reinterpret_cast<const uint4*>(cnt_sorted + base), b = *reinterpret_cast<const uint4*>(cnt_sorted + base + 4);
-    s = a.x + a.y + a.z + a.w + b.x + b.y + b.z + b.w;
+  int blk = blockIdx.x;
+  if constexpr (CR) {
+    if (blockIdx.x == 0) {
+      fold_max_key(mk_parts, nparts, mk_out, mk_host, sm);
+      return;
+    }
+    blk = (int)blockIdx.x - 1;
+    const int64_t tb = (int64_t)blk * SC_TILE + threadIdx.x;
+#pragma unroll
+    for (int k = 0; k < SC_IPT; ++k) {
+      const uint4 c = cr[min(tb + k * 256, n - 1)];
+      if (tb + k * 256 < n) s += cr_count(c);
+    }
   } else {
-#pragma unroll
-    for (int k = 0; k < SC_IPT; ++k)
-      if (base + k < n) s += cnt_sorted[base + k];
+    const int64_t base = (int64_t)blockIdx.x * SC_TILE + (int64_t)threadIdx.x * SC_IPT;
+    if (base + SC_IPT <= n) {
+      const uint4 a = *reinterpret_cast<const uint4*>(cnt_sorted + base), b = *reinterpret_cast<const uint4*>(cnt_sorted + base + 4);
+      s = a.x + a.y + a.z + a.w + b.x + b.y + b.z + b.w;
+    } else {
+#pragma unroll
+      for (int k = 0; k < SC_IPT; ++k)
+        if (base + k < n) s += cnt_sorted[base + k];
+    }
   }
   s = wave_inclusive_scan(s);
   if ((threadIdx.x & 63) == 63) sm[threadIdx.x >> 6] = s;
   __syncthreads();
-  if (threadIdx.x == 0) partials[blockIdx.x] = sm[0] + sm[1] + sm[2] + sm[3];
-}
-
-__global__ __launch_bounds__(256) void k_bin_scan_apply(const uint32_t* __restrict__ cnt_sorted, int64_t n,
+  if (threadIdx.x == 0) partials[blk] = sm[0] + sm[1] + sm[2] + sm[3];
+}
+
+template <bool CR>
+__global__ __launch_bounds__(256) void k_bin_scan_apply(const uint32_t* __restrict__ cnt_sorted,
+                                                        const uint4* __restrict__ cr, int64_t n,
                                                         const uint32_t* __restrict__ partials,
                                                         uint32_t* __restrict__ out, uint32_t* __restrict__ total,
                                                         uint32_t* __restrict__ total_host) {
   __shared__ uint32_t sm[4];
   __shared__ uint32_t s_prefix;
+  __shared__ uint32_t s_cnt[CR ? SC_TILE : 1];
+  uint4 c8[CR ? SC_IPT : 1];
+  if constexpr (CR) {
+    const int64_t tb = (int64_t)blockIdx.x * SC_TILE + threadIdx.x;
+#pragma unroll
+    for (int k = 0; k < SC_IPT; ++k) c8[k] = cr[min(tb + k * 256, n - 1)];
+  }
   uint32_t pre = 0;
   for (int i = threadIdx.x; i < (int)blockIdx.x; i += 256) pre += partials[i];
   pre = wave_inclusive_scan(pre);
   if ((threadIdx.x & 63) == 63) sm[threadIdx.x >> 6] = pre;
+  if constexpr (CR) {
+    const int64_t tb = (int64_t)blockIdx.x * SC_TILE + threadIdx.x;
+#pragma unroll
+    for (int k = 0; k < SC_IPT; ++k) s_cnt[k * 256 + threadIdx.x] = (tb + k * 256 < n) ? cr_count(c8[k]) : 0u;
+  }
   __syncthreads();
   if (threadIdx.x == 0) s_prefix = sm[0] + sm[1] + sm[2] + sm[3];
   __syncthreads();
@@ -179,7 +213,11 @@
   const int64_t base = (int64_t)blockIdx.x * SC_TILE + (int64_t)threadIdx.x * SC_IPT;
   uint32_t v[SC_IPT];
   uint32_t s = 0;
-  if (base + SC_IPT <= n) {
+  if constexpr (CR) {
+    const uint4 a = *reinterpret_cast<const uint4*>(s_cnt + threadIdx.x * SC_IPT);
+    const uint4 b = *reinterpret_cast<const uint4*>(s_cnt + threadIdx.x * SC_IPT + 4);
+    v[0] = a.x; v[1] = a.y; v[2] = a.z; v[3] = a.w; v[4] = b.x; v[5] = b.y; v[6] = b.z; v[7] = b.w;
+  } else if (base + SC_IPT <= n) {
     const uint4 a = *reinterpret_cast<const uint4*>(cnt_sorted + base), b = *reinterpret_cast<const uint4*>(cnt_sorted + base + 4);
     v[0] = a.x; v[1] = a.y; v[2] = a.z; v[3] = a.w; v[4] = b.x; v[5] = b.y; v[6] = b.z; v[7] = b.w;
   } else {
@@ -210,6 +248,7 @@
   }
 }
 
+template <bool TDS>
 __global__ __launch_bounds__(256) void k_bin_emit(int n, int gx, const uint32_t* __restrict__ ids,
                                                   const uint32_t* __restrict__ offsets,
                                                   const uint4* __restrict__ cr_sorted,
@@ -217,10 +256,12 @@
                                                   uint32_t* __restrict__ tkeys, uint32_t* __restrict__ gsid,
                                                   uint32_t cap, int32_t* __restrict__ ranges, int n_ranges,
                                                   int with_masks, uint32_t* __restrict__ sort_sup,
-                                                  uint32_t sort_sup_words) {
+                                                  uint32_t sort_sup_words, const uint32_t* __restrict__ dkeys,
+                                                  int dbits) {
   __shared__ uint32_t s_off[257];
   __shared__ uint32_t s_g[256];
   __shared__ uint4 s_cr[256];
+  __shared__ uint32_t s_dk[TDS ? 256 : 1];
   const int tid = threadIdx.x;
   const int j = blockIdx.x * 256 + tid;
   for (int i = j; i < n_ranges; i += gridDim.x * 256) ranges[i] = 0;
@@ -228,7 +269,8 @@
   uint32_t off = 0, g = 0;
   uint4 c = make_uint4(0u, 0u, 0u, 0u);
   if (j < n) {
-    g = ids[j];
+    if constexpr (TDS) { g = (uint32_t)j; s_dk[tid] = dkeys[j] & ((1u << dbits) - 1u); }
+    else g = ids[j];
     c = cr_sorted[j];
     off = offsets[j];
   }
@@ -330,6 +372,7 @@
       continue;
     }
     if (first + s0 >= cap) break;
+    if constexpr (TDS) tile = (tile << dbits) | s_dk[lo];
     tkeys[first + s0] = tile;
     gsid[first + s0] = with_masks ? (s_g[lo] | (mask << EGS_GSID_BITS)) : s_g[lo];
   }
@@ -364,7 +407,9 @@
           for (int tx = qlo + lane; tx <= qhi; tx += 64) {
             const uint32_t o = obase + qoff + (uint32_t)(tx - qlo);
             if (o < cap) {
-              tkeys[o] = (uint32_t)(y0 + rb + q) * (uint32_t)gx + (uint32_t)tx;
+              const uint32_t tl = (uint32_t)(y0 + rb + q) * (uint32_t)gx + (uint32_t)tx;
+              if constexpr (TDS) tkeys[o] = (tl << dbits) | s_dk[t];
+              else tkeys[o] = tl;
               gsid[o] = with_masks ? (gg | (foot_mask(qa, qb, tx) << EGS_GSID_BITS)) : gg;
             }
           }
@@ -380,7 +425,8 @@
                                                      const uint32_t* __restrict__ n_dev,
                                                      const uint32_t* __restrict__ masked, int32_t* __restrict__ plain,
                                                      int32_t* __restrict__ zero, int zero_words,
-                                                     int32_t* __restrict__ walk_word, uint32_t* __restrict__ walk_host) {
+                                                     int32_t* __restrict__ walk_word, uint32_t* __restrict__ walk_host,
+                                                     int key_shift) {
   for (int z = blockIdx.x * 256 + threadIdx.x; z < zero_words; z += gridDim.x * 256) zero[z] = 0;
   if (walk_word && blockIdx.x == 0 && threadIdx.x == 0) {
     const int w = walk_word[0], l = walk_word[1];
@@ -408,6 +454,8 @@
 #pragma unroll
     for (int i = 0; i < 4; ++i) k[1 + i] = (p0 + i < P) ? tkeys[p0 + i] : 0u;
   }
+#pragma unroll
+  for (int i = 0; i < 5; ++i) k[i] >>= key_shift;
 #pragma unroll
   for (int i = 0; i < 4; ++i) {
     const int64_t p = p0 + i;
@@ -501,17 +549,23 @@
 
 
 int bin_emit(int n, int gx, const BinLayout& B, uint32_t* tkeys, uint32_t* gsid, uint32_t cap, int32_t* ranges,
-             int n_ranges, int with_masks, uint32_t* sort_sup, uint32_t sort_sup_words, hipStream_t s) {
-  EGS_LAUNCH("k_bin_emit", k_bin_emit, dim3(div_up(n, 256)), dim3(256), s, n, gx, B.ids, B.offsets, B.cr_sorted, B.br,
-             tkeys, gsid, cap, ranges, n_ranges, with_masks, sort_sup, sort_sup_words);
+             int n_ranges, int with_masks, uint32_t* sort_sup, uint32_t sort_sup_words, hipStream_t s, int dbits) {
+  if (dbits > 0)
+    EGS_LAUNCH("k_bin_emit", k_bin_emit<true>, dim3(div_up(n, 256)), dim3(256), s, n, gx, (const uint32_t*)nullptr,
+               B.offsets, B.cr, B.br, tkeys, gsid, cap, ranges, n_ranges, with_masks, sort_sup, sort_sup_words, B.dkeys,
+               dbits);
+  else
+    EGS_LAUNCH("k_bin_emit", k_bin_emit<false>, dim3(div_up(n, 256)), dim3(256), s, n, gx, B.ids, B.offsets, B.cr_sorted,
+               B.br, tkeys, gsid, cap, ranges, n_ranges, with_masks, sort_sup, sort_sup_words, (const uint32_t*)nullptr, 0);
   EGS_LAUNCH_OK();
   return 0;
 }
 
 int tile_ranges(int64_t P, const uint32_t* tkeys, int32_t* ranges, const uint32_t* n_dev, const uint32_t* masked,
-                int32_t* plain, hipStream_t s, int32_t* zero, int zero_words, int32_t* walk_word, uint32_t* walk_host) {
+                int32_t* plain, hipStream_t s, int32_t* zero, int zero_words, int32_t* walk_word, uint32_t* walk_host,
+                int key_shift) {
   EGS_LAUNCH("k_tile_ranges", k_tile_ranges, dim3(div_up(P, 1024)), dim3(256), s, P, tkeys, ranges, n_dev, masked, plain,
-             zero, zero_words, walk_word, walk_host);
+             zero, zero_words, walk_word, walk_host, key_shift);
   EGS_LAUNCH_OK();
   return 0;
 }
@@ -621,12 +675,22 @@
 }
 
 int splat_bin_after_count(int n, int key_bits_hint, void* ws_bin, size_t ws_bin_bytes, uint32_t* total_patches,
-                          void* stream, uint32_t* host_totals) {
+                          void* stream, uint32_t* host_totals, bool tile_depth_sort) {
   hipStream_t s = (hipStream_t)stream;
   BinLayout L;
   if (!bin_carve(ws_bin, ws_bin_bytes, n, &L)) {
     set_error(EGS_ERR_WORKSPACE, "bin workspace too small", __FILE__, __LINE__);
     return EGS_ERR_WORKSPACE;
+  }
+  if (tile_depth_sort) {
+    const int nb = div_up(n, SC_TILE);
+    EGS_LAUNCH("k_bin_scan_partials", k_bin_scan_partials<true>, dim3(nb + 1), dim3(256), s, (const uint32_t*)nullptr,
+               L.cr, (int64_t)n, L.scan_partials, L.maxkey, div_up(n, 256), total_patches + 1,
+               host_totals ? host_totals + 1 : (uint32_t*)nullptr);
+    EGS_LAUNCH("k_bin_scan_apply", k_bin_scan_apply<true>, dim3(nb), dim3(256), s, (const uint32_t*)nullptr, L.cr,
+               (int64_t)n, L.scan_partials, L.offsets, total_patches, host_totals);
+    EGS_LAUNCH_OK();
+    return 0;
   }
   const int end_bit = (key_bits_hint <= 0 || key_bits_hint > 32) ? 32 : key_bits_hint;
   int rc = radix_sort(n, L.dkeys, L.ids, L.dkeys_alt, L.ids_alt, 0, end_bit, L.sort, s, L.maxkey, nullptr, L.maxkey,
@@ -638,10 +702,11 @@
     EGS_HIP(hipMemcpyAsync(L.ids, L.ids_alt, (size_t)n * 4, hipMemcpyDeviceToDevice, s));
   }
   const int nb = div_up(n, SC_TILE);
-  EGS_LAUNCH("k_bin_scan_partials", k_bin_scan_partials, dim3(nb), dim3(256), s, L.cnt_sorted, (int64_t)n,
-             L.scan_partials);
-  EGS_LAUNCH("k_bin_scan_apply", k_bin_scan_apply, dim3(nb), dim3(256), s, L.cnt_sorted, (int64_t)n, L.scan_partials,
-             L.offsets, total_patches, host_totals);
+  EGS_LAUNCH("k_bin_scan_partials", k_bin_scan_partials<false>, dim3(nb), dim3(256), s, L.cnt_sorted,
+             (const uint4*)nullptr, (int64_t)n, L.scan_partials, (uint32_t*)nullptr, 0, (uint32_t*)nullptr,
+             (uint32_t*)nullptr);
+  EGS_LAUNCH("k_bin_scan_apply", k_bin_scan_apply<false>, dim3(nb), dim3(256), s, L.cnt_sorted, (const uint4*)nullptr,
+             (int64_t)n, L.scan_partials, L.offsets, total_patches, host_totals);
   EGS_LAUNCH_OK();
   return 0;
 }
diff --git a/easygaussiansplatting_amd/csrc/egs_common.h b/easygaussiansplatting_amd/csrc/egs_common.h
--- a/easygaussiansplatting_amd/csrc/egs_common.h
+++ b/easygaussiansplatting_amd/csrc/egs_common.h
@@ -116,7 +116,7 @@
 BinParams make_bin_params(int width, int height, const EgsPolicy* pol, bool cull_lists = false);
 bool bin_count_outputs(void* ws_bin, size_t ws_bin_bytes, int n, BinCountOut* out);
 int splat_bin_after_count(int n, int key_bits_hint, void* ws_bin, size_t ws_bin_bytes, uint32_t* total_patches,
-                          void* stream, uint32_t* host_totals);
+                          void* stream, uint32_t* host_totals, bool tile_depth_sort = false);
 
 struct SplatSource {
   const void* rec;
diff --git a/easygaussiansplatting_amd/csrc/egs_gaussian_math.h b/easygaussiansplatting_amd/csrc/egs_gaussian_math.h
--- a/easygaussiansplatting_amd/csrc/egs_gaussian_math.h
+++ b/easygaussiansplatting_amd/csrc/egs_gaussian_math.h
@@ -609,6 +609,22 @@
   __syncthreads();
   if (threadIdx.x == 0) maxkey[1 + blockIdx.x] = max(max(wm[0], wm[1]), max(wm[2], wm[3]));
 }
+__device__ __forceinline__ void fold_max_key(uint32_t* __restrict__ mk_parts, int nparts, uint32_t* __restrict__ mk_out,
+                                             uint32_t* __restrict__ mk_host, uint32_t* sm) {
+  const int tid = threadIdx.x;
+  uint32_t mk = 0u;
+  for (int i = tid; i < nparts; i += 256) mk = max(mk, mk_parts[1 + i]);
+#pragma unroll
+  for (int d = 32; d >= 1; d >>= 1) mk = max(mk, (uint32_t)__shfl_xor((int)mk, d, 64));
+  if ((tid & 63) == 0) sm[tid >> 6] = mk;
+  __syncthreads();
+  if (tid == 0) {
+    const uint32_t m = max(max(sm[0], sm[1]), max(sm[2], sm[3]));
+    mk_parts[0] = m;
+    if (mk_out) *mk_out = m;
+    if (mk_host) *mk_host = m;
+  }
+}
 
 __device__ __forceinline__ void make_record(float ux, float uy, float c0, float c1, float c2, float alpha,
                                             float r, float g, float b, int area_x, int area_y, int W, int H,
diff --git a/easygaussiansplatting_amd/csrc/egs_preprocess.hip b/easygaussiansplatting_amd/csrc/egs_preprocess.hip
--- a/easygaussiansplatting_amd/csrc/egs_preprocess.hip
+++ b/easygaussiansplatting_amd/csrc/egs_preprocess.hip
@@ -972,7 +972,7 @@
                                  float* colors, int32_t* areas, void* rec, uint8_t* visible, float* dcolor_dpws,
                                  int flags, int key_bits_hint, void* ws_bin, size_t ws_bin_bytes,
                                  uint32_t* total_patches, uint32_t* host_totals, void* stream) {
-  EGS_CHECK_ARG((flags & ~(EGS_FUSED_CULLED_LISTS | EGS_FUSED_ANTIALIASED | EGS_FUSED_RAW)) == 0);
+  EGS_CHECK_ARG((flags & ~(EGS_FUSED_CULLED_LISTS | EGS_FUSED_ANTIALIASED | EGS_FUSED_RAW | EGS_FUSED_TILE_DEPTH_SORT)) == 0);
   const bool cull_lists = (flags & EGS_FUSED_CULLED_LISTS) != 0;
   const bool aa = (flags & EGS_FUSED_ANTIALIASED) != 0;
   const bool raw = (flags & EGS_FUSED_RAW) != 0;
@@ -1013,7 +1013,8 @@
   EGS_LAUNCH(aa ? "k_preprocess_fwd_aa" : "k_preprocess_fwd", kern, g, b, s, n, pp, pws, rots, scales, shs, shs_high,
              alphas, Rcw, tcw, twc, us, depths, cinv2ds, colors, areas, (float4*)rec, bp, bo, visible, dcolor_dpws);
   EGS_LAUNCH_OK();
-  return splat_bin_after_count(n, key_bits_hint, ws_bin, ws_bin_bytes, total_patches, stream, host_totals);
+  return splat_bin_after_count(n, key_bits_hint, ws_bin, ws_bin_bytes, total_patches, stream, host_totals,
+                               (flags & EGS_FUSED_TILE_DEPTH_SORT) != 0);
 }
 
 extern "C" size_t egs_fused_backward_ws_bytes(int n) { return egs_splat_bwd_ws_bytes(n); }
diff --git a/easygaussiansplatting_amd/csrc/egs_raster.h b/easygaussiansplatting_amd/csrc/egs_raster.h
--- a/easygaussiansplatting_amd/csrc/egs_raster.h
+++ b/easygaussiansplatting_amd/csrc/egs_raster.h
@@ -17,6 +17,8 @@
                const uint32_t* n_dev = nullptr, uint32_t* mk_parts = nullptr, int nparts = 0,
                uint32_t* mk_out = nullptr, uint32_t* mk_host = nullptr, const uint4* gsrc = nullptr,
                uint4* gdst = nullptr, uint32_t* cdst = nullptr);
+int tile_depth_sort(int T, const int32_t* ranges, uint32_t* tkeys, uint32_t* gsid, uint32_t* tkeys_alt,
+                    uint32_t* gsid_alt, int64_t capacity, int dbits, hipStream_t s);
 constexpr int SC_IPT = 8;
 constexpr int SC_TILE = 256 * SC_IPT;
 size_t scan_ws_bytes(int64_t n);
@@ -31,10 +33,10 @@
 size_t bin_ws_bytes(int n);
 bool bin_carve(void* ws, size_t bytes, int n, BinLayout* L);
 int bin_emit(int n, int gx, const BinLayout& B, uint32_t* tkeys, uint32_t* gsid, uint32_t cap, int32_t* ranges,
-             int n_ranges, int with_masks, uint32_t* sort_sup, uint32_t sort_sup_words, hipStream_t s);
+             int n_ranges, int with_masks, uint32_t* sort_sup, uint32_t sort_sup_words, hipStream_t s, int dbits = 0);
 int tile_ranges(int64_t P, const uint32_t* tkeys, int32_t* ranges, const uint32_t* n_dev, const uint32_t* masked,
                 int32_t* plain, hipStream_t s, int32_t* zero = nullptr, int zero_words = 0, int32_t* walk_word = nullptr,
-                uint32_t* walk_host = nullptr);
+                uint32_t* walk_host = nullptr, int key_shift = 0);
 int pack_records(int n, int width, int height, int footprint, float alpha_skip, const float* us, const float* cinv2ds,
                  const float* alphas, const float* colors, const int32_t* areas, float4* rec, uint32_t* stamp,
                  const uint32_t* stamp_ref, uint8_t* same, hipStream_t s);
diff --git a/easygaussiansplatting_amd/csrc/egs_sort.hip b/easygaussiansplatting_amd/csrc/egs_sort.hip
--- a/easygaussiansplatting_amd/csrc/egs_sort.hip
+++ b/easygaussiansplatting_amd/csrc/egs_sort.hip
@@ -1,4 +1,5 @@
 #include "egs_raster.h"
+#include "egs_tile_depth_sort.h"
 
 #include <algorithm>
 
@@ -24,18 +25,7 @@
   const int tid = threadIdx.x;
   const int blk = mk_parts ? (int)blockIdx.x - 1 : (int)blockIdx.x;
   if (mk_parts && blockIdx.x == 0) {
-    uint32_t mk = 0u;
-    for (int i = tid; i < nparts; i += 256) mk = max(mk, mk_parts[1 + i]);
-#pragma unroll
-    for (int d = 32; d >= 1; d >>= 1) mk = max(mk, (uint32_t)__shfl_xor((int)mk, d, 64));
-    if ((tid & 63) == 0) sm[tid >> 6] = mk;
-    __syncthreads();
-    if (tid == 0) {
-      const uint32_t m = max(max(sm[0], sm[1]), max(sm[2], sm[3]));
-      mk_parts[0] = m;
-      if (mk_out) *mk_out = m;
-      if (mk_host) *mk_host = m;
-    }
+    fold_max_key(mk_parts, nparts, mk_out, mk_host, sm);
     return;
   }
   if (!mk_parts && maxkey && ((*maxkey >> shift) == 0u)) return;
@@ -155,23 +145,7 @@
     const int64_t idx = base + r * EGS_WAVE + lane;
     const bool valid = idx < n;
     const uint32_t d = (key[r] >> shift) & dmask;
-    const uint64_t vb = __ballot(valid);
-    uint32_t plo = (uint32_t)vb, phi = (uint32_t)(vb >> 32);
-#pragma unroll
-    for (int b = 0; b < 8; ++b) {
-      if (b >= nbits) break;
-      const uint32_t m = (uint32_t)((int32_t)(d << (31 - b)) >> 31);
-      const uint64_t bal = __ballot(m != 0u);
-      plo &= ~((uint32_t)bal ^ m);
-      phi &= ~((uint32_t)(bal >> 32) ^ m);
-    }
-    const uint32_t below = __builtin_amdgcn_mbcnt_hi(phi, __builtin_amdgcn_mbcnt_lo(plo, 0u));
-    uint32_t prev = 0;
-    if (valid) prev = __hip_atomic_load(&wc[d], __ATOMIC_RELAXED, __HIP_MEMORY_SCOPE_WAVEFRONT);
-    if (valid && below == 0)
-      __hip_atomic_store(&wc[d], prev + (uint32_t)(__popc(plo) + __popc(phi)), __ATOMIC_RELAXED, __HIP_MEMORY_SCOPE_WAVEFRONT);
-    __builtin_amdgcn_fence(__ATOMIC_ACQ_REL, "wavefront");
-    rank[r] = prev + below;
+    EGS_WAVE_DIGIT_RANK(rank[r], d, valid, nbits, wc)
   }
   __syncthreads();
   uint32_t cnt = 0;
@@ -302,6 +276,16 @@
   return 0;
 }
 
+int tile_depth_sort(int T, const int32_t* ranges, uint32_t* tkeys, uint32_t* gsid, uint32_t* tkeys_alt,
+                    uint32_t* gsid_alt, int64_t capacity, int dbits, hipStream_t s) {
+  if (T <= 0 || dbits <= 0 || capacity <= 0) return 0;
+  const int width = tile_depth_sort_width(dbits);
+  EGS_LAUNCH("k_tile_depth_sort", k_tile_depth_sort, dim3(T), dim3(256), s, T, ranges, tkeys, gsid, tkeys_alt, gsid_alt,
+             capacity, dbits, width);
+  EGS_LAUNCH_OK();
+  return 0;
+}
+
 
 __global__ __launch_bounds__(256) void k_scan_partials(const uint32_t* __restrict__ in,
                                                        const uint32_t* __restrict__ gather, int64_t n,
diff --git a/easygaussiansplatting_amd/csrc/egs_splat.hip b/easygaussiansplatting_amd/csrc/egs_splat.hip
--- a/easygaussiansplatting_amd/csrc/egs_splat.hip
+++ b/easygaussiansplatting_amd/csrc/egs_splat.hip
@@ -197,6 +197,8 @@
     return EGS_ERR_WORKSPACE;
   }
   const int tb = tile_bits(dp.T);
+  const int dbits = (o.flags & EGS_DRAW_TILE_DEPTH_SORT) ? ((o.flags >> EGS_DRAW_DEPTH_BITS_SHIFT) & 63) : 0;
+  EGS_CHECK_ARG(!(o.flags & EGS_DRAW_TILE_DEPTH_SORT) || (dbits >= 1 && tb + dbits <= 32 && !o.gsid_plain));
   const int passes = sort_passes(0, tb);
   uint32_t* gs_primary = (uint32_t*)gsid_per_patch;
   uint32_t* k0 = (passes & 1) ? D.tkeys_alt : D.tkeys;
@@ -204,7 +206,7 @@
   uint32_t* v0 = (passes & 1) ? D.gsid_alt : gs_primary;
   uint32_t* v1 = (passes & 1) ? gs_primary : D.gsid_alt;
   int rc = bin_emit(n, dp.gx, B, k0, v0, (uint32_t)patches, patch_range_per_tile, 2 * dp.T, dp.masked, D.sort.sup,
-                    (uint32_t)D.sort.sup_words, s);
+                    (uint32_t)D.sort.sup_words, s, dbits);
   if (rc) return rc;
   const float4* rec = src.rec ? (const float4*)src.rec : D.rec;
   if (!src.rec) {
@@ -212,15 +214,19 @@
                       src.areas, D.rec, nullptr, nullptr, nullptr, s);
     if (rc) return rc;
   }
-  rc = radix_sort(patches, k0, v0, k1, v1, 0, tb, D.sort, s, nullptr, o.patches_dev);
+  rc = radix_sort(patches, k0, v0, k1, v1, dbits, dbits + tb, D.sort, s, nullptr, o.patches_dev);
   if (rc) return rc;
   SegArgs sga;
   const bool seg = o.seg_ws && pol->footprint == 0 && pol->alpha_skip > 0.f && pol->tau_stop > 0.f &&
                    dp.T <= (int)SEG_TILE_MASK && seg_carve(o.seg_ws, o.seg_ws_bytes, dp.T, &sga);
   rc = tile_ranges(patches, D.tkeys, patch_range_per_tile, o.patches_dev,
                    (const uint32_t*)(o.gsid_plain ? gsid_per_patch : nullptr), o.gsid_plain, s, seg ? sga.hdr : nullptr,
-                   seg ? SEG_PLAN_WORDS : 0, o.walk_word, o.seg_hint);
+                   seg ? SEG_PLAN_WORDS : 0, o.walk_word, o.seg_hint, dbits);
   if (rc) return rc;
+  if (dbits > 0) {
+    rc = tile_depth_sort(dp.T, patch_range_per_tile, D.tkeys, gs_primary, D.tkeys_alt, D.gsid_alt, patches, dbits, s);
+    if (rc) return rc;
+  }
   if (o.seg_ws && !seg) {
     set_error(EGS_ERR_WORKSPACE, "segment workspace too small (or a policy without a skip / stop threshold)", __FILE__, __LINE__);
     return EGS_ERR_WORKSPACE;
diff --git a/easygaussiansplatting_amd/csrc/egs_tile_depth_sort.h b/easygaussiansplatting_amd/csrc/egs_tile_depth_sort.h
--- /dev/null
+++ b/easygaussiansplatting_amd/csrc/egs_tile_depth_sort.h
@@ -0,0 +1,173 @@
+#pragma once
+#include "egs_common.h"
+
+namespace egs {
+
+#define EGS_WAVE_DIGIT_RANK(out, d, valid, nbits, wc)                                                                  \
+  {                                                                                                                    \
+    const uint64_t vb_ = __ballot(valid);                                                                              \
+    uint32_t plo_ = (uint32_t)vb_, phi_ = (uint32_t)(vb_ >> 32);                                                       \
+    _Pragma("unroll") for (int b_ = 0; b_ < 8; ++b_) {                                                                 \
+      if (b_ >= (nbits)) break;                                                 \
+      const uint32_t m_ = (uint32_t)((int32_t)((d) << (31 - b_)) >> 31);               \
+      const uint64_t bal_ = __ballot(m_ != 0u);                                                                        \
+      plo_ &= ~((uint32_t)bal_ ^ m_);                      \
+      phi_ &= ~((uint32_t)(bal_ >> 32) ^ m_);                                                                          \
+    }                                                                                                                  \
+    const uint32_t below_ = __builtin_amdgcn_mbcnt_hi(phi_, __builtin_amdgcn_mbcnt_lo(plo_, 0u));                      \
+    uint32_t prev_ = 0;                                                                                                \
+    if (valid) prev_ = __hip_atomic_load(&(wc)[d], __ATOMIC_RELAXED, __HIP_MEMORY_SCOPE_WAVEFRONT);                    \
+    if ((valid) && below_ == 0)                                                               \
+      __hip_atomic_store(&(wc)[d], prev_ + (uint32_t)(__popc(plo_) + __popc(phi_)), __ATOMIC_RELAXED,                  \
+                         __HIP_MEMORY_SCOPE_WAVEFRONT);                                                                \
+    __builtin_amdgcn_fence(__ATOMIC_ACQ_REL, "wavefront");                                                             \
+    (out) = prev_ + below_;                                                                                            \
+  }
+
+constexpr int TDS_CAP = 2048;
+constexpr int TDS_IPT = TDS_CAP / 256;
+
+__global__ __launch_bounds__(256) void k_tile_depth_sort(int T, const int32_t* __restrict__ ranges, uint32_t* tkeys,
+                                                         uint32_t* gsid, uint32_t* tkeys_alt, uint32_t* gsid_alt,
+                                                         int64_t capacity, int dbits, int width) {
+  __shared__ uint32_t wcount[4][256];
+  __shared__ uint32_t dstart[256];
+  __shared__ uint32_t sm[4];
+  __shared__ uint32_t skey[TDS_CAP], sval[TDS_CAP];
+  const int tid = threadIdx.x, wave = __builtin_amdgcn_readfirstlane(tid >> 6), lane = tid & 63;
+  const int tile = blockIdx.x;
+  if (tile >= T) return;
+  const int64_t r0 = max((int64_t)ranges[2 * (size_t)tile], (int64_t)0);
+  const int64_t r1 = min((int64_t)ranges[2 * (size_t)tile + 1], capacity);
+  if (r1 - r0 < 2) return;
+  const int n = (int)(r1 - r0);
+  uint32_t* wc = wcount[wave];
+  if (n <= TDS_CAP) {
+    const int chunk = ((n + 255) >> 8) << 6;
+    const int rounds = chunk >> 6;
+    const int ibase = wave * chunk + lane;
+    uint32_t key[TDS_IPT], val[TDS_IPT], rank[TDS_IPT];
+    {
+      const uint32_t* kb = tkeys + r0;
+      const uint32_t* vb = gsid + r0;
+#pragma unroll
+      for (int r = 0; r < TDS_IPT; ++r) {
+        const int i = min(ibase + r * 64, n - 1);
+        key[r] = kb[i];
+        val[r] = vb[i];
+      }
+    }
+    for (int shift = 0; shift < dbits; shift += width) {
+      const int nbits = min(width, dbits - shift);
+      const uint32_t dmask = (1u << nbits) - 1u;
+      const bool last = shift + width >= dbits;
+#pragma unroll
+      for (int w = 0; w < 4; ++w) wcount[w][tid] = 0;
+      __syncthreads();
+#pragma unroll
+      for (int r = 0; r < TDS_IPT; ++r)
+        if (r < rounds && wave * chunk + r * 64 < n) {
+          const uint32_t d = (key[r] >> shift) & dmask;
+          const bool valid = ibase + r * 64 < n;
+          EGS_WAVE_DIGIT_RANK(rank[r], d, valid, nbits, wc)
+        }
+      __syncthreads();
+      uint32_t cnt = 0;
+#pragma unroll
+      for (int w = 0; w < 4; ++w) {
+        const uint32_t c = wcount[w][tid];
+        wcount[w][tid] = cnt;
+        cnt += c;
+      }
+      const uint32_t ds = block256_exclusive_scan(cnt, sm, nullptr);
+      dstart[tid] = ds;
+      __syncthreads();
+#pragma unroll
+      for (int r = 0; r < TDS_IPT; ++r) {
+        if (r < rounds && ibase + r * 64 < n) {
+          const uint32_t d = (key[r] >> shift) & dmask;
+          const uint32_t slot = dstart[d] + wc[d] + rank[r];
+          if (!last) skey[slot] = key[r];
+          sval[slot] = val[r];
+        }
+      }
+      __syncthreads();
+      if (!last) {
+#pragma unroll
+        for (int r = 0; r < TDS_IPT; ++r) {
+          if (r < rounds && ibase + r * 64 < n) {
+            key[r] = skey[ibase + r * 64];
+            val[r] = sval[ibase + r * 64];
+          }
+        }
+      }
+    }
+    uint32_t* vo = gsid + r0;
+    for (int i = tid; i < n; i += 256) vo[i] = sval[i];
+    return;
+  }
+  uint32_t *ki = tkeys + r0, *vi = gsid + r0, *ko = tkeys_alt + r0, *vo = gsid_alt + r0;
+  uint32_t* gbase = skey;
+  for (int shift = 0; shift < dbits; shift += width) {
+    const int nbits = min(width, dbits - shift);
+    const uint32_t dmask = (1u << nbits) - 1u;
+    gbase[tid] = 0;
+    __syncthreads();
+    for (int i = tid; i < n; i += 256) atomicAdd(&gbase[(ki[i] >> shift) & dmask], 1u);
+    __syncthreads();
+    const uint32_t c = gbase[tid];
+    const uint32_t ex = block256_exclusive_scan(c, sm, nullptr);
+    gbase[tid] = ex;
+    for (int c0 = 0; c0 < n; c0 += TDS_CAP) {
+#pragma unroll
+      for (int w = 0; w < 4; ++w) wcount[w][tid] = 0;
+      __syncthreads();
+      const int ibase = c0 + wave * (TDS_IPT * 64) + lane;
+      uint32_t key[TDS_IPT], val[TDS_IPT], rank[TDS_IPT];
+#pragma unroll
+      for (int r = 0; r < TDS_IPT; ++r) {
+        const int i = min(ibase + r * 64, n - 1);
+        key[r] = ki[i];
+        val[r] = vi[i];
+      }
+#pragma unroll
+      for (int r = 0; r < TDS_IPT; ++r) {
+        const uint32_t d = (key[r] >> shift) & dmask;
+        const bool valid = ibase + r * 64 < n;
+        EGS_WAVE_DIGIT_RANK(rank[r], d, valid, nbits, wc)
+      }
+      __syncthreads();
+      uint32_t cnt = 0;
+#pragma unroll
+      for (int w = 0; w < 4; ++w) {
+        const uint32_t cw = wcount[w][tid];
+        wcount[w][tid] = cnt;
+        cnt += cw;
+      }
+      __syncthreads();
+#pragma unroll
+      for (int r = 0; r < TDS_IPT; ++r) {
+        if (ibase + r * 64 < n) {
+          const uint32_t d = (key[r] >> shift) & dmask;
+          const uint32_t pos = gbase[d] + wc[d] + rank[r];
+          ko[pos] = key[r];
+          vo[pos] = val[r];
+        }
+      }
+      __syncthreads();
+      gbase[tid] += cnt;
+    }
+    __syncthreads();
+    uint32_t* t = ki; ki = ko; ko = t;
+    t = vi; vi = vo; vo = t;
+  }
+  if (vi != gsid + r0)
+    for (int i = tid; i < n; i += 256) vo[i] = vi[i];
+}
+
+inline int tile_depth_sort_width(int dbits) {
+  const int passes = (dbits + 7) / 8;
+  return (dbits + passes - 1) / passes;
+}
+
+}
diff --git a/easygaussiansplatting_amd/csrc/egs_tilesort.hip b/easygaussiansplatting_amd/csrc/egs_tilesort.hip
--- /dev/null
+++ b/easygaussiansplatting_amd/csrc/egs_tilesort.hip
@@ -0,0 +1,23 @@
+#define EGS_SIDE_LIBRARY "egs_tilesort"
+#include "egs_side_error.h"
+
+#include "../../include/egs_tilesort.h"
+#include "egs_tile_depth_sort.h"
+
+static_assert(egs::TDS_CAP == EGS_TILE_DEPTH_SORT_CAP, "the header's capacity is the kernel's");
+
+extern "C" int egs_tilesort_abi_version(void) { return EGS_TILESORT_ABI_VERSION; }
+extern "C" const char* egs_tilesort_last_error_string(void) { return egs_side::g_err; }
+extern "C" int egs_tile_depth_sort_cap(void) { return egs::TDS_CAP; }
+
+extern "C" int egs_tile_depth_sort(int n_tiles, const int32_t* ranges, uint32_t* tkeys, uint32_t* gsid,
+                                   uint32_t* tkeys_alt, uint32_t* gsid_alt, int64_t capacity, int dbits,
+                                   void* stream) {
+  SIDE_CHECK_ARG(n_tiles >= 0 && capacity >= 0 && capacity < (int64_t)0x7FFFFFFF && dbits >= 0 && dbits <= 32);
+  if (n_tiles == 0 || capacity == 0 || dbits == 0) return 0;
+  SIDE_CHECK_ARG(ranges && tkeys && gsid && tkeys_alt && gsid_alt);
+  hipLaunchKernelGGL(egs::k_tile_depth_sort, dim3(n_tiles), dim3(256), 0, (hipStream_t)stream, n_tiles, ranges, tkeys,
+                     gsid, tkeys_alt, gsid_alt, capacity, dbits, egs::tile_depth_sort_width(dbits));
+  SIDE_HIP(hipGetLastError());
+  return 0;
+}
diff --git a/easygaussiansplatting_amd/fused.py b/easygaussiansplatting_amd/fused.py
--- a/easygaussiansplatting_amd/fused.py
+++ b/easygaussiansplatting_amd/fused.py
@@ -7,7 +7,7 @@
 
 import torch
 
-from . import _ahead, _lib
+from . import _ahead, _lib, _tilesortlib
 from ._ahead import (_ctx, _seg_decision, _settle, _tls, _walk_word,
                      commit, deferred, expect_long_walks, seg_hint)
 from ._host import _alphas, _chk, _lib_on, _pol, _ptr, _stream, _tiles
@@ -22,11 +22,14 @@
 TILE_WORK_CACHE = os.environ.get("EGS_TILE_WORK_CACHE", "1") != "0"
 SAVE_DCOLOR = os.environ.get("EGS_SAVE_DCOLOR", "1") != "0"
 CULL_LISTS = os.environ.get("EGS_CULL_LISTS", "1") != "0"
+TILE_DEPTH_SORT = int(os.environ.get("EGS_TILE_DEPTH_SORT", "1") or 0)
 SEGMENTS = os.environ.get("EGS_SEGMENTS", "auto")
 DRAW_CULLED_LISTS = 1
 DRAW_MASKED_LISTS = 2
 SEG_HISTORY = 4
 SEG_SPECULATE_FLAG = 8
+DRAW_TILE_DEPTH_SORT = 16
+DRAW_DEPTH_BITS_SHIFT = 8
 SEG_SPECULATE = os.environ.get("EGS_SEG_SPECULATE", "auto")
 ACCUMULATE = 64
 FACTORED_SH = 128
@@ -35,13 +38,14 @@
 CULLED_LISTS = 32
 ANTIALIASED = 256
 RAW = 512
+FUSED_TILE_DEPTH_SORT = 4096
 GSID_MASK = 0x0FFFFFFF
 
 
 class FusedState:
     __slots__ = ("us", "depths", "cinv2ds", "colors", "areas", "rec", "contrib", "final_tau", "ranges", "gsid",
                  "order", "order_by_work", "gpack", "dcw", "flags", "width", "height", "ticket", "_patches", "_keep",
-                 "seg", "extras")
+                 "seg", "extras", "depth_bits")
 
     @property
     def culled(self):
@@ -50,6 +54,7 @@
     @property
     def antialiased(self):
         return bool(self.flags & ANTIALIASED)
+
 
     def patch_count(self) -> int:
         if self.ticket is not None:
@@ -138,6 +143,7 @@
     S = FusedState()
     S.width, S.height = W, H
     S.ticket, S._patches, S._keep, S.seg, S.extras = None, None, None, None, None
+    S.depth_bits = 0
     S.us = S.cinv2ds = S.colors = S.areas = None
     pol_ = _pol()
     culled = CULL_LISTS and pol_.footprint == 0 and pol_.alpha_skip > 0 and n < (1 << 28)
@@ -147,11 +153,16 @@
     mask = torch.empty((n,), dtype=torch.bool, device=dev)
     ws_bin_bytes = lib.egs_splat_bin_ws_bytes(n)
     ws_bin = torch.empty(ws_bin_bytes, dtype=torch.uint8, device=dev)
-    enqueue_bin = lambda hint, total, host_slot: _lib.check(lib.egs_fused_forward(
-        n, K, _ptr(pws), _ptr(rots), _ptr(scales), _ptr(shs), _ptr(high_shs), _ptr(alphas), _ptr(Rcw), _ptr(tcw),
-        _ptr(twc), float(cam.fx), float(cam.fy), float(cam.cx), float(cam.cy), W, H, pol, _ptr(S.us), _ptr(S.depths),
-        _ptr(S.cinv2ds), _ptr(S.colors), _ptr(S.areas), _ptr(S.rec), _ptr(mask), _ptr(S.dcw), S.flags, hint,
-        _ptr(ws_bin), ws_bin_bytes, _ptr(total), host_slot, st))
+    def enqueue_bin(hint, total, host_slot):
+        S.depth_bits = _ahead.tile_depth_bits(TILE_DEPTH_SORT != 0 and n > 0, _tiles(W, H), hint,
+                                              None if TILE_DEPTH_SORT == 2 else longest_list(),
+                                              _tilesortlib.CAP)
+        _lib.check(lib.egs_fused_forward(
+            n, K, _ptr(pws), _ptr(rots), _ptr(scales), _ptr(shs), _ptr(high_shs), _ptr(alphas), _ptr(Rcw), _ptr(tcw),
+            _ptr(twc), float(cam.fx), float(cam.fy), float(cam.cx), float(cam.cy), W, H, pol, _ptr(S.us),
+            _ptr(S.depths), _ptr(S.cinv2ds), _ptr(S.colors), _ptr(S.areas), _ptr(S.rec), _ptr(mask), _ptr(S.dcw),
+            S.flags | (FUSED_TILE_DEPTH_SORT if S.depth_bits else 0), hint, _ptr(ws_bin), ws_bin_bytes, _ptr(total),
+            host_slot, st))
     image = torch.empty((3, H, W), dtype=f32, device=dev)
     depth_map = alpha_map = None
     ex = None
@@ -178,7 +189,8 @@
         _lib.check(lib.egs_splat_draw_rec_seg(
             n, rows, _ptr(total), W, H, _ptr(S.rec), pol, _ptr(ws_bin), _ptr(ws_draw), ws_draw.numel(), _ptr(image),
             _ptr(S.contrib), _ptr(S.final_tau), _ptr(S.ranges), _ptr(S.gsid), _ptr(S.order), _ptr(S.gpack), prev_work,
-            order_ready, draw_flags, _ptr(S.seg), S.seg.numel() if S.seg is not None else 0,
+            order_ready, draw_flags | _ahead.draw_depth_flags(S.depth_bits, DRAW_TILE_DEPTH_SORT, DRAW_DEPTH_BITS_SHIFT),
+            _ptr(S.seg), S.seg.numel() if S.seg is not None else 0,
             None if (redo and walk_word is not None) else seg_hint, _ptr(walk_word), None, st,
             None if ex is None else C.byref(ex)))
         remember_order()
@@ -193,6 +205,10 @@
     if extras is not None:
         use_seg = False
     walk_word = _walk_word(ctx, key, dev, st, seg_hint is not None)
+
+    def longest_list():
+        h = _ahead.seg_hint(dev, key) if seg_hint is not None else None
+        return None if h is None else h[0]
     walk_known = False
     if TILE_WORK_CACHE and n > 0:
         ck = (id(cam), int(st.value or 0))
diff --git a/include/egs_hip.h b/include/egs_hip.h
--- a/include/egs_hip.h
+++ b/include/egs_hip.h
@@ -98,6 +98,8 @@
 #define EGS_DRAW_MASKED_LISTS 2
 #define EGS_DRAW_SEG_HISTORY 4
 #define EGS_DRAW_SEG_SPECULATE 8
+#define EGS_DRAW_TILE_DEPTH_SORT 16
+#define EGS_DRAW_DEPTH_BITS_SHIFT 8
 size_t egs_tile_order_len(int width, int height);
 size_t egs_seg_ws_bytes(int64_t patch_capacity, int width, int height);
 int egs_seg_config(int segment_len, int split_min, int* out2);
@@ -145,6 +147,7 @@
 #define EGS_FUSED_CULLED_LISTS 32
 #define EGS_FUSED_ANTIALIASED 256
 #define EGS_FUSED_RAW 512
+#define EGS_FUSED_TILE_DEPTH_SORT 4096
 int egs_fused_forward(int n, int sh_dim, const float* pws, const float* rots, const float* scales,
                       const float* shs, const float* high_shs , const float* alphas,
                       const float* Rcw, const float* tcw, const float* twc, float fx, float fy, float cx, float cy,
diff --git a/include/egs_tilesort.h b/include/egs_tilesort.h
--- /dev/null
+++ b/include/egs_tilesort.h
@@ -0,0 +1,25 @@
+#ifndef EGS_TILESORT_H_
+#define EGS_TILESORT_H_
+
+#include <stddef.h>
+#include <stdint.h>
+
+#include "egs_hip.h"
+
+#ifdef __cplusplus
+extern "C" {
+#endif
+
+#define EGS_TILESORT_ABI_VERSION 1
+#define EGS_TILE_DEPTH_SORT_CAP 2048
+
+int egs_tilesort_abi_version(void);
+const char* egs_tilesort_last_error_string(void);
+int egs_tile_depth_sort_cap(void);
+int egs_tile_depth_sort(int n_tiles, const int32_t* ranges, uint32_t* tkeys, uint32_t* gsid, uint32_t* tkeys_alt,
+                        uint32_t* gsid_alt, int64_t capacity, int dbits, void* stream);
+
+#ifdef __cplusplus
+}
+#endif
+#endif
```

Result: slower. 2403 Mpix/s (-2.7%).
